# XunshanMan/Object-oriented-SLAM

Measured on AMD Instinct MI355X. Metric: LM iterations/sec (cams+ellipsoids), higher is better.
Workload: dtype f64

## Files before the change

### object-oriented-slam_amd/csrc/esl_capi.hip

```cpp
#include <algorithm>
#include <cfloat>
#include <cmath>
#include <cstdio>
#include <cstdlib>
#include <cstring>
#include <numeric>

#include "esl_graph_int.hpp"
#include "esl_graph_layout.hpp"
#include "esl_kernels_map.hpp"
#include "esl_kernels_chunk.hpp"
#include "esl_slam.hpp"
#include "esl_fixed.hpp"

namespace esl {
static thread_local std::string g_err;
void set_error(const std::string& s) { g_err = s; }
}

using namespace esl;

namespace esl {
ProfScope::ProfScope(esl_ctx* ctx, int kind) : c(ctx), slot(-1) {
  if (!c || !c->prof_on) return;
  if (c->prof_level < 2 && (kind != 0 || !c->prof_gate)) return;
  if (c->prof_used + 2 > c->prof_ev.size()) {
    if (c->prof_ev.size() >= 16384) { prof_drain(c); }
    else {
      for (int i = 0; i < 512; ++i) { hipEvent_t e; if (hipEventCreate(&e) != hipSuccess) return; c->prof_ev.push_back(e); }
      c->prof_kind.resize(c->prof_ev.size() / 2);
    }
  }
  slot = (int)c->prof_used;
  c->prof_kind[slot / 2] = kind;
  c->prof_used += 2;
  (void)hipEventRecord(c->prof_ev[slot], c->stream);
}
ProfScope::~ProfScope() {
  if (slot >= 0) (void)hipEventRecord(c->prof_ev[slot + 1], c->stream);
}
int prof_drain(esl_ctx* c) {
  if (hipStreamSynchronize(c->stream) != hipSuccess) return ESL_ERR_HIP;
  for (size_t s = 0; s + 1 < c->prof_used; s += 2) {
    float ms = 0;
    if (hipEventElapsedTime(&ms, c->prof_ev[s], c->prof_ev[s + 1]) == hipSuccess) {
      const int k = c->prof_kind[s / 2];
      c->prof_count[k]++;
      c->prof_ms[k] += ms;
    }
  }
  c->prof_used = 0;
  return ESL_OK;
}
}

struct WorkStage {
  struct Fix { void** dst; size_t off; };
  size_t total = 0;
  std::vector<Fix> fixes;
  template <class T>
  void add(T** dst, size_t n) {
    const size_t off = layout::align_up(total, 256);
    total = off + std::max<size_t>(n, 1) * sizeof(T);
    fixes.push_back({(void**)dst, off});
  }
  int commit(esl_ctx* c) {
    int rc = arena_reserve(&c->arena_work, &c->arena_work_cap, std::max<size_t>(total, 256));
    if (rc) return rc;
    for (const Fix& f : fixes) *f.dst = c->arena_work + f.off;
    return ESL_OK;
  }
};
int esl::work_buffers(esl_ctx* c, size_t cap_objs, size_t cap_cams, size_t cap_chunks) {
  WorkStage wk;
  wk.add(&c->chunk_out, cap_chunks * kChunkOut); wk.add(&c->chunk_out2, cap_chunks * kChunkOut);
  wk.add(&c->chunk_chi, cap_chunks);
  wk.add(&c->blk_part, ((cap_objs + kStepWaves - 1) / kStepWaves + 2) * 2);
  wk.add(&c->solve_part, ((cap_objs + kStepWaves - 1) / kStepWaves + (cap_objs + 63) / 64 + 2) * 4 * 2);
  wk.add(&c->blk_chi, cap_chunks + 2);
  wk.add(&c->cams, cap_cams * 7); wk.add(&c->cams_trial, cap_cams * 7);
  wk.add(&c->objs, cap_objs * 10); wk.add(&c->objs_trial, cap_objs * 10);
  wk.add(&c->Hoo, cap_objs * 45); wk.add(&c->bo, cap_objs * 9); wk.add(&c->xo, cap_objs * 9); wk.add(&c->obj_part, cap_objs * 4);
  int rc = wk.commit(c);
  if (rc) return rc;
  ESL_HIP_TRY(hipMemsetAsync(c->obj_part, 0, std::max<size_t>(cap_objs, 1) * 4 * sizeof(double), c->stream));
  return ESL_OK;
}

extern "C" {

int esl_abi_version(void) { return ESL_ABI_VERSION; }
const char* esl_last_error(void) { return g_err.c_str(); }

int esl_device_count(void) {
  int n = 0;
  if (hipGetDeviceCount(&n) != hipSuccess) return 0;
  return n;
}

void esl_lm_params_default(esl_lm_params* p) {
  p->max_iters = 10;
  p->max_trials = 10;
  p->tau = 1e-5;
  p->jacobian_mode = ESL_JAC_NUMERIC;
  p->numeric_delta = 1e-9;
  p->linear_solver = ESL_SOLVER_AUTO;
  p->drop_nan_bbox = 1;
  p->bbox_residual = ESL_BBOX_REPROJECTION;
  p->e3d_half_turn = 0;
}

int esl_ctx_create(int device_id, esl_ctx** out) {
  if (!out) return ESL_ERR_INVALID;
  *out = nullptr;
  int n = 0;
  if (hipGetDeviceCount(&n) != hipSuccess || n <= 0) {
    set_error("no HIP device visible: libesl_hip has no CPU fallback");
    return ESL_ERR_NO_DEVICE;
  }
  if (device_id < 0 || device_id >= n) { set_error("device id out of range"); return ESL_ERR_INVALID; }
  ESL_HIP_TRY(hipSetDevice(device_id));
  esl_ctx* c = new esl_ctx();
  c->device = device_id;
  { const char* ov = std::getenv("ESL_CF_OVERLAP"); c->sw_cf_overlap = (ov && ov[0] >= '0' && ov[0] <= '4') ? ov[0] - '0' : 4; }
  { const char* ok = std::getenv("ESL_CF_OS_KERNEL"); c->sw_cf_os_kernel = (ok && ok[0] == '0') ? 0 : 1; }
  { const char* ol = std::getenv("ESL_CF_OS_LIST"); c->sw_cf_os_list = (ol && ol[0] == '0') ? 0 : 1; }
  { const char* fp = std::getenv("ESL_CF_FWD_PARTS"); const int v = fp ? std::atoi(fp) : 0; if (v == 2 || v == 4 || v == 8) c->sw_cf_fwd_parts = v; }
  { const char* sd = std::getenv("ESL_CF_STRIDE"); const int v = sd ? std::atoi(sd) : 0; c->sw_cf_stride = (v == 16 || v == 32 || v == 48) ? v : 0; }
  auto init = [&]() -> int {
    ESL_HIP_TRY(hipStreamCreateWithFlags(&c->stream, hipStreamNonBlocking));
    ESL_HIP_TRY(hipHostMalloc((void**)&c->host_part, 16 * sizeof(double), hipHostMallocDefault));
    ESL_HIP_TRY(hipMalloc((void**)&c->dev_part, 16 * sizeof(double)));
    ESL_HIP_TRY(hipMalloc((void**)&c->chol_info, 4 * sizeof(int)));
    ESL_HIP_TRY(hipMemset(c->chol_info, 0, 4 * sizeof(int)));
    ESL_HIP_TRY(hipMalloc((void**)&c->tickets, 4 * sizeof(unsigned int)));
    ESL_HIP_TRY(hipMemset(c->tickets, 0, 4 * sizeof(unsigned int)));
    ESL_HIP_TRY(hipMalloc((void**)&c->dev_scal, 8 * sizeof(double)));
    ESL_HIP_TRY(hipEventCreateWithFlags(&c->ev_try, hipEventDisableTiming));
    ESL_HIP_TRY(hipHostMalloc(&c->host_scal, sizeof(LmScalars), hipHostMallocMapped));
    ESL_HIP_TRY(hipHostGetDevicePointer(&c->host_scal_dev, c->host_scal, 0));
    std::memset(c->host_scal, 0, sizeof(LmScalars));
    ESL_HIP_TRY(hipMalloc(&c->lm_dev, 2 * sizeof(LmCore)));
    ESL_HIP_TRY(hipMemset(c->lm_dev, 0, 2 * sizeof(LmCore)));
    ESL_HIP_TRY(hipHostMalloc(&c->lm_host, sizeof(LmHostView), hipHostMallocMapped));
    ESL_HIP_TRY(hipHostGetDevicePointer(&c->lm_host_dev, c->lm_host, 0));
    std::memset(c->lm_host, 0, sizeof(LmHostView));
    return ESL_OK;
  };
  const int rc = init();
  if (rc) { const std::string msg = g_err; esl_ctx_destroy(c); set_error(msg); return rc; }
  *out = c;
  return ESL_OK;
}

int esl_ctx_destroy(esl_ctx* c) {
  if (!c) return ESL_OK;
  (void)hipSetDevice(c->device);
  if (c->stream) (void)hipStreamSynchronize(c->stream);
  slam_sync_side(c);
  free_graph(c);
  slam_release(c);
  if (c->arena_graph) (void)hipFree(c->arena_graph);
  if (c->arena_work) (void)hipFree(c->arena_work);
  if (c->stage_host) (void)hipHostFree(c->stage_host);
  if (c->append_dev) (void)hipFree(c->append_dev);
  if (c->slam_tab_dev) (void)hipFree(c->slam_tab_dev);
  c->eq_buf.release();
  if (c->fx_blob) (void)hipFree(c->fx_blob);
  c->chain_ws.release();
  fit_release(c);
  plane_release(c);
  reloc_release(c);
  assoc_release(c);
  merge_release(c);
  render_release(c);
  dense_release(c);
  init_batch_release(c);
  for (hipEvent_t e : c->prof_ev) (void)hipEventDestroy(e);
  if (c->host_part) (void)hipHostFree(c->host_part);
  dev_free(&c->dev_part);
  dev_free(&c->chol_info);
  dev_free(&c->tickets); dev_free(&c->dev_scal);
  if (c->host_scal) (void)hipHostFree(c->host_scal);
  if (c->lm_host) (void)hipHostFree(c->lm_host);
  if (c->lm_dev) (void)hipFree(c->lm_dev);
  if (c->ev_try) (void)hipEventDestroy(c->ev_try);
  esl_comm_destroy(c);
  slam_release_runtime(c);
  if (c->stream) (void)hipStreamDestroy(c->stream);
  delete c;
  return ESL_OK;
}

int esl_ctx_trim(esl_ctx* c) {
  if (!c) return ESL_ERR_INVALID;
  ESL_HIP_TRY(hipSetDevice(c->device));
  ESL_HIP_TRY(hipStreamSynchronize(c->stream));
  slam_trim(c, c->graph_loaded && c->g.n_free_cams > 0);
  return ESL_OK;
}

int esl_debug_scratch_allocs(esl_ctx* c, int32_t owner, int64_t* allocs_out, int64_t* bytes_out) {
  if (!c || !allocs_out || !bytes_out || owner < ESL_SCRATCH_RELOC || owner > ESL_SCRATCH_INIT_ROBUST) {
    set_error("esl_debug_scratch_allocs: null pointer or unknown owner");
    return ESL_ERR_INVALID;
  }
  *allocs_out = 0; *bytes_out = 0;
  switch (owner) {
    case ESL_SCRATCH_RELOC: reloc_scratch_stats(c, allocs_out, bytes_out); break;
    case ESL_SCRATCH_ASSOC: assoc_scratch_stats(c, allocs_out, bytes_out); break;
    case ESL_SCRATCH_MERGE: merge_scratch_stats(c, allocs_out, bytes_out); break;
    case ESL_SCRATCH_RENDER: render_scratch_stats(c, allocs_out, bytes_out); break;
    default: init_scratch_stats(c, owner == ESL_SCRATCH_INIT_ROBUST, allocs_out, bytes_out);
  }
  return ESL_OK;
}

int esl_ctx_synchronize(esl_ctx* c) {
  if (!c) return ESL_ERR_INVALID;
  ESL_HIP_TRY(hipStreamSynchronize(c->stream));
  return ESL_OK;
}

static ChunkTable chunk_table(const esl_ctx* c) {
  ChunkTable t;
  t.n_chunks = c->n_chunks; t.obj = c->ck_obj; t.type = c->ck_type; t.begin = c->ck_begin; t.end = c->ck_end; t.ostart = c->ck_ostart;
  return t;
}
static int map_launch_linearize(esl_ctx* c, bool finalize, const double* src_objs = nullptr, double* dst_chunk = nullptr,
                                const LmCore* st = nullptr, bool validate = false) {
  const DevGraph& g = c->g;
  if (!src_objs) src_objs = c->objs;
  if (!dst_chunk) dst_chunk = c->chunk_out;
  const double* objs_b = st ? c->objs_trial : nullptr;
  double* chunk_b = st ? c->chunk_out2 : nullptr;
  if (st) { src_objs = c->objs; dst_chunk = c->chunk_out; }
  const ChunkTable ct = chunk_table(c);
  const bool an = c->lm.p.jacobian_mode == ESL_JAC_ANALYTIC;
  const int nb_e3 = (c->n_ids_e3 + 2 * kLinWaves - 1) / (2 * kLinWaves);
  const int nb_bb = (c->n_ids_bb + kLinWaves - 1) / kLinWaves;
  robust_dispatch(c->robust_on, [&](auto robust) {
    constexpr bool R = decltype(robust)::value;
    if (ct.n_chunks > 0) {
      ProfScope ps(c, 0);
      const dim3 block(64 * kLinWaves);
      int* cnt = c->chol_info + 2;
      if (an && g.bbox_mode) {
        if (validate && g.check_vis)
          hipLaunchKernelGGL((k_chunk_linearize_both<ESL_JAC_ANALYTIC, 2, true, R>), dim3(nb_e3 + nb_bb), block, 0, c->stream, g, ct, c->ck_ids_e3,
                             c->n_ids_e3, nb_e3, c->ck_ids_bb, c->n_ids_bb, c->cams, src_objs, objs_b, c->lm.p.numeric_delta, dst_chunk,
                             chunk_b, c->blk_chi, st, cnt);
        else if (validate)
          hipLaunchKernelGGL((k_chunk_linearize_both<ESL_JAC_ANALYTIC, 1, true, R>), dim3(nb_e3 + nb_bb), block, 0, c->stream, g, ct, c->ck_ids_e3,
                             c->n_ids_e3, nb_e3, c->ck_ids_bb, c->n_ids_bb, c->cams, src_objs, objs_b, c->lm.p.numeric_delta, dst_chunk,
                             chunk_b, c->blk_chi, st, cnt);
        else
          hipLaunchKernelGGL((k_chunk_linearize_both<ESL_JAC_ANALYTIC, 0, true, R>), dim3(nb_e3 + nb_bb), block, 0, c->stream, g, ct, c->ck_ids_e3,
                             c->n_ids_e3, nb_e3, c->ck_ids_bb, c->n_ids_bb, c->cams, src_objs, objs_b, c->lm.p.numeric_delta, dst_chunk,
                             chunk_b, c->blk_chi, st, cnt);
      } else if (an) {
        if (validate && g.check_vis)
          hipLaunchKernelGGL((k_chunk_linearize_both<ESL_JAC_ANALYTIC, 2, false, R>), dim3(nb_e3 + nb_bb), block, 0, c->stream, g, ct, c->ck_ids_e3,
                             c->n_ids_e3, nb_e3, c->ck_ids_bb, c->n_ids_bb, c->cams, src_objs, objs_b, c->lm.p.numeric_delta, dst_chunk,
                             chunk_b, c->blk_chi, st, cnt);
        else if (validate)
          hipLaunchKernelGGL((k_chunk_linearize_both<ESL_JAC_ANALYTIC, 1, false, R>), dim3(nb_e3 + nb_bb), block, 0, c->stream, g, ct, c->ck_ids_e3,
                             c->n_ids_e3, nb_e3, c->ck_ids_bb, c->n_ids_bb, c->cams, src_objs, objs_b, c->lm.p.numeric_delta, dst_chunk,
                             chunk_b, c->blk_chi, st, cnt);
        else
          hipLaunchKernelGGL((k_chunk_linearize_both<ESL_JAC_ANALYTIC, 0, false, R>), dim3(nb_e3 + nb_bb), block, 0, c->stream, g, ct, c->ck_ids_e3,
                             c->n_ids_e3, nb_e3, c->ck_ids_bb, c->n_ids_bb, c->cams, src_objs, objs_b, c->lm.p.numeric_delta, dst_chunk,
                             chunk_b, c->blk_chi, st, cnt);
      } else {
        if (nb_e3 > 0)
          hipLaunchKernelGGL((k_chunk_linearize<ESL_JAC_NUMERIC, 1, 0, false, R>), dim3(nb_e3), block, 0, c->stream, g, ct, c->ck_ids_e3,
                             c->n_ids_e3, c->cams, src_objs, objs_b, c->lm.p.numeric_delta, dst_chunk, chunk_b, c->blk_chi, 0, st, cnt);
        if (nb_bb > 0) {
          auto launch_bb = [&](auto kern) {
            hipLaunchKernelGGL(kern, dim3(nb_bb), block, 0, c->stream, g, ct, c->ck_ids_bb, c->n_ids_bb, c->cams, src_objs, objs_b,
// ... 643 lines not shown
```

### object-oriented-slam_amd/csrc/esl_cf.hpp

```cpp
#pragma once
#include "esl_cf_plan.hpp"
#include "esl_kernels_map.hpp"

namespace esl {

__device__ __forceinline__ double cf_readlane(double v, int src) {
  const int lo = __builtin_amdgcn_readlane(__double2loint(v), src), hi = __builtin_amdgcn_readlane(__double2hiint(v), src);
  return __hiloint2double(hi, lo);
}

static __global__ __launch_bounds__(256) void k_cf_gather_B(int nf, const double* __restrict__ Aod, const int* __restrict__ od_start,
                                                            const int* __restrict__ od_edge, double* __restrict__ B) {
  const long t = (long)blockIdx.x * 256 + threadIdx.x;
  const long i = t / 36;
  if (i >= nf) return;
  const int e = (int)(t - i * 36), r = e / 6, c = e - 6 * r;
  double s = 0;
  if (i + 1 < nf)
    for (int q = od_start[i]; q < od_start[i + 1]; ++q) {
      const int es = od_edge[q];
      const double* Hij = Aod + (size_t)(es >> 1) * 90 + 54;
      s += (es & 1) ? Hij[c * 6 + r] : Hij[r * 6 + c];
    }
  B[t] = s;
// ... 263 lines not shown
          for (int q = 0; q < CH * 6; ++q) sv[q * 64 + lane] = (q < hl * 6) ? svy[h0 * 6 + q] : 0.0;
        } else if (col) {
          const int ka = cst[ch], kb = cst[ch + 1];
          for (int k = ka; k < kb; k += 4) {
            int sl[4];
            double rec[4][6];
#pragma unroll
            for (int e = 0; e < 4; ++e) {
              const int kk = (k + e < kb) ? k + e : ka;
              sl[e] = oe_slot[kk];
              const double* src = V + ((size_t)kk * 9 + b) * 6;
#pragma unroll
              for (int a = 0; a < 6; ++a) rec[e][a] = src[a];
            }
#pragma unroll
            for (int e = 0; e < 4; ++e)
              if (k + e < kb && sl[e] - i0 >= h0 && sl[e] - i0 - h0 < hl) {
#pragma unroll
                for (int a = 0; a < 6; ++a) sv[((sl[e] - i0 - h0) * 6 + a) * 64 + lane] += rec[e][a];
              }
          }
        }
        __builtin_amdgcn_wave_barrier();
      }
      for (int ii = 0; ii < hl; ++ii) {
        const double* M = sM + (h0 + ii) * 36;
        double xn[6];
#pragma unroll
        for (int a = 0; a < 6; ++a) {
          double t = sv[(ii * 6 + a) * 64 + lane];
#pragma unroll
          for (int q = 0; q < 6; ++q) t -= M[a * 6 + q] * x[q];
          xn[a] = t;
        }
#pragma unroll
        for (int a = 0; a < 6; ++a) { x[a] = xn[a]; sv[(ii * 6 + a) * 64 + lane] = xn[a]; }
        if (use_z) {
          const double* Z = sZ + (h0 + ii) * 36;
#pragma unroll
          for (int a = 0; a < 6; ++a)
#pragma unroll
            for (int q = 0; q < 6; ++q) acc[a] += Z[q * 6 + a] * xn[q];
        }
      }
      if (on) {
#pragma unroll
        for (int q0 = 0; q0 < CH * 6; q0 += 8) {
          double t[8];
#pragma unroll
          for (int e = 0; e < 8; ++e) t[e] = sv[((q0 + e < hl * 6) ? q0 + e : 0) * 64 + lane];
#pragma unroll
          for (int e = 0; e < 8; ++e)
            if (q0 + e < hl * 6) {
              const int q = q0 + e;
              if (MODE == 2) {
                Xt[(size_t)sg.xoff[seg] + (size_t)(6 * (i0 - beg + h0) + q) * (size_t)sg.xld[seg] + (size_t)j] = t[e];
              } else {
                const size_t row = (SEP && sep_stride > 0) ? (size_t)(6 * ((i0 + q / 6) * sep_stride + sep_stride - 1) + q % 6) : (size_t)(6 * i0 + q);
                Xt[(size_t)j + row * (size_t)ldx] = t[e];
              }
            }
        }
      }
      __builtin_amdgcn_wave_barrier();
    }
  }
  if (use_z && on) {
#pragma unroll
    for (int a = 0; a < 6; ++a) R[(size_t)tcol + (size_t)(6 * (seg - 1) + a) * (size_t)ldx] = acc[a];
  }
}

static __global__ __launch_bounds__(64) void k_cf_zt(int nf, int stride, const double* __restrict__ Linv, const double* __restrict__ Mm,
                                                     const double* __restrict__ B, double* __restrict__ Zt) {
  __shared__ double sM[kCfMaxStride * 36];
  const int p = blockIdx.x + 1, lane = threadIdx.x;
  const int beg = p * stride, end = (beg + stride - 1 < nf) ? beg + stride - 1 : nf;
  if (beg >= end) return;
  const int len = end - beg;
  {
    constexpr int kQ = kCfMaxStride * 36 / 64;
    double t[kQ];
#pragma unroll
    for (int q = 0; q < kQ; ++q) { const int idx = q * 64 + lane; t[q] = Mm[(size_t)beg * 36 + (idx < len * 36 ? idx : 0)]; }
#pragma unroll
    for (int q = 0; q < kQ; ++q) sM[q * 64 + lane] = t[q];
  }
  __builtin_amdgcn_wave_barrier();
  const int c = lane < 6 ? lane : 5;
  double z[6];
  {
    const double* Li = Linv + (size_t)beg * 36;
    const double* Bs = B + (size_t)(beg - 1) * 36;
#pragma unroll
    for (int r = 0; r < 6; ++r) {
      double v = 0;
#pragma unroll
      for (int k = 0; k <= r; ++k) v += Li[r * 6 + k] * Bs[k * 6 + c];
      z[r] = v;
    }
  }
  for (int ii = 0; ii < len; ++ii) {
    if (ii > 0) {
      const double* M = sM + ii * 36;
      double zn[6];
#pragma unroll
      for (int r = 0; r < 6; ++r) {
        double v = 0;
#pragma unroll
        for (int k = 0; k < 6; ++k) v -= M[r * 6 + k] * z[k];
        zn[r] = v;
      }
#pragma unroll
      for (int r = 0; r < 6; ++r) z[r] = zn[r];
    }
    if (lane < 6) {
#pragma unroll
      for (int r = 0; r < 6; ++r) Zt[(size_t)(beg + ii) * 36 + r * 6 + lane] = z[r];
    }
  }
}

static __global__ __launch_bounds__(256) void k_cf_sep_assemble(int nf, int stride, int n_sep, const double* __restrict__ Hcc, double lambda,
                                                                const double* __restrict__ Gfac, const double* __restrict__ Zt,
                                                                double* __restrict__ Hs, double* __restrict__ Bs) {
  const int t = blockIdx.x * 256 + threadIdx.x;
  const int k = t / 36;
  if (k >= n_sep) return;
  const int e = t - k * 36, r = e / 6, c = e - 6 * r;
  const int s = k * stride + stride - 1, l = s - 1;
  double v = Hcc[(size_t)s * 36 + e] + ((r == c) ? lambda : 0.0);
#pragma unroll
  for (int q = 0; q < 6; ++q) v -= Gfac[(size_t)l * 36 + q * 6 + r] * Gfac[(size_t)l * 36 + q * 6 + c];
  const int beg = (k + 1) * stride, end = (beg + stride - 1 < nf) ? beg + stride - 1 : nf;
  for (int j = beg; j < end; ++j) {
#pragma unroll
    for (int q = 0; q < 6; ++q) v -= Zt[(size_t)j * 36 + q * 6 + r] * Zt[(size_t)j * 36 + q * 6 + c];
  }
  Hs[t] = v;
  double w = 0;
  if (k + 1 < n_sep) {
    const int le = end - 1;
#pragma unroll
    for (int q = 0; q < 6; ++q) w -= Gfac[(size_t)le * 36 + q * 6 + r] * Zt[(size_t)le * 36 + q * 6 + c];
  }
  Bs[t] = w;
}

static __global__ __launch_bounds__(64) void k_cf_sep_rhs(int nf, int n_o, int stride, int n_chunks, const int* __restrict__ oe_cst,
                                                          const int* __restrict__ oe_slot, const double* __restrict__ V,
                                                          const double* __restrict__ vy, const double* __restrict__ Gfac,
                                                          const double* __restrict__ LiS, const double* __restrict__ Xt, long ldx,
                                                          double* __restrict__ R, const int* __restrict__ cmap ,
                                                          CfSegs sg) {
  const int j = blockIdx.x * 64 + threadIdx.x, k = blockIdx.y;
  if (j > n_o) return;
  const bool rhs = j == n_o;
  const int N1 = n_o / 9 + 1;
  const int s = k * stride + stride - 1, l = s - 1;
  double vs[6] = {0, 0, 0, 0, 0, 0};
  if (rhs) {
#pragma unroll
    for (int a = 0; a < 6; ++a) vs[a] = vy[(size_t)s * 6 + a];
  } else {
    const int tb = j / 9, b = j - 9 * tb;
    const int o = sg.unrank ? sg.unrank[tb] : tb;
    const int* cst = oe_cst + (size_t)o * (n_chunks + 1);
    const int ch = s / kCfFwdCh;
    for (int q = cst[ch]; q < cst[ch + 1]; ++q)
      if (oe_slot[q] == s) {
        const double* src = V + ((size_t)q * 9 + b) * 6;
#pragma unroll
        for (int a = 0; a < 6; ++a) vs[a] += src[a];
      }
  }
  bool has_acc = (k + 1) * stride < nf;
  double xl[6] = {0, 0, 0, 0, 0, 0};
  if (cmap) {
    const int tb2 = j / 9, bb = rhs ? 0 : j - 9 * tb2;
    const int ob = rhs ? N1 - 1 : (sg.unrank ? sg.unrank[tb2] : tb2);
    has_acc = has_acc && cmap[(size_t)(k + 1) * N1 + ob] >= 0;
    const int e = cmap[(size_t)k * N1 + ob];
    if (e >= 0) {
      const double* src = Xt + (size_t)sg.xoff[k] + (size_t)(9 * (e & 0xFFFFFF) + bb);
      const size_t ld = (size_t)sg.xld[k];
#pragma unroll
      for (int r = 0; r < 6; ++r) xl[r] = src[(size_t)(6 * (stride - 2) + r) * ld];
    }
  } else {
#pragma unroll
    for (int r = 0; r < 6; ++r) xl[r] = Xt[(size_t)j + (size_t)(6 * l + r) * (size_t)ldx];
  }
  double t[6];
#pragma unroll
  for (int a = 0; a < 6; ++a) t[a] = has_acc ? R[(size_t)j + (size_t)(6 * k + a) * (size_t)ldx] : 0.0;
#pragma unroll
  for (int a = 0; a < 6; ++a)
#pragma unroll
    for (int r = 0; r < 6; ++r) t[a] += Gfac[(size_t)l * 36 + r * 6 + a] * xl[r];
#pragma unroll
  for (int a = 0; a < 6; ++a) {
    double v = vs[a];
#pragma unroll
    for (int q = 0; q <= a; ++q) v -= LiS[(size_t)k * 36 + a * 6 + q] * t[q];
    R[(size_t)j + (size_t)(6 * k + a) * (size_t)ldx] = v;
  }
}

static __global__ __launch_bounds__(256) void k_cf_back_prep(int nf, int stride, int n_sep, const double* __restrict__ Zt, const double* __restrict__ Gfac,
                                                             const double* __restrict__ xc, double* __restrict__ z) {
  const int t = blockIdx.x * 256 + threadIdx.x;
  const int i = t / 6, a = t - 6 * i;
  if (i >= nf) return;
  const int p = i / stride, pos = i - p * stride;
  if (pos == stride - 1) return;
  double v = 0;
  if (p >= 1) {
    const double* xs = xc + (size_t)(p * stride - 1) * 6;
#pragma unroll
    for (int q = 0; q < 6; ++q) v += Zt[(size_t)i * 36 + a * 6 + q] * xs[q];
  }
  if ((pos == stride - 2 || i == nf - 1) && p < n_sep) {
    const double* xs = xc + (size_t)(p * stride + stride - 1) * 6;
#pragma unroll
    for (int q = 0; q < 6; ++q) v += Gfac[(size_t)i * 36 + a * 6 + q] * xs[q];
  }
  z[t] -= v;
}

__device__ __forceinline__ void cf_T_init_full_one(const double* __restrict__ Hoo, const double* __restrict__ bo, double lambda,
                                                   double* __restrict__ T, long ldt, long n_o, long t) {
  const long col = t / ldt, row = t - col * ldt;
  if (col >= n_o) return;
  double v = 0;
  const long o = col / 9;
  const int c = (int)(col - 9 * o);
  if (row == n_o) v = bo[(size_t)o * 9 + c];
  else if (row < n_o && row / 9 == o && row >= col) {
    const int r = (int)(row - 9 * o);
    v = Hoo[(size_t)o * 45 + c * 9 - (c * (c - 1)) / 2 + (r - c)] + ((r == c) ? lambda : 0.0);
  }
  T[t] = v;
}
static __global__ __launch_bounds__(256) void k_cf_edge_scale_T(DevGraph g, int nb_es, int n_list, const int* __restrict__ oe_u, const int* __restrict__ oe_slot,
                                                                const double* __restrict__ W, const double* __restrict__ Linv,
                                                                const double* __restrict__ bc, double* __restrict__ V, double* __restrict__ vy,
                                                                const double* __restrict__ Hoo, const double* __restrict__ bo, double lambda,
                                                                double* __restrict__ T, long ldt, long n_o) {
  if ((int)blockIdx.x < nb_es) cf_edge_scale_one(g, n_list, oe_u, oe_slot, W, Linv, bc, V, vy, (long)blockIdx.x * 256 + threadIdx.x);
  else cf_T_init_full_one(Hoo, bo, lambda, T, ldt, n_o, (long)(blockIdx.x - nb_es) * 256 + threadIdx.x);
}

static __global__ __launch_bounds__(256) void k_cf_z(const double* __restrict__ Xt, long ldx, int n_o, const double* __restrict__ xo,
                                                     double* __restrict__ z) {
  __shared__ double red[4];
  const double* row = Xt + (size_t)blockIdx.x * (size_t)ldx;
  double s = 0;
  for (int o = threadIdx.x; o < n_o; o += 256) s += row[o] * xo[o];
  s = wave_sum(s);
  if ((threadIdx.x & 63) == 0) red[threadIdx.x >> 6] = s;
  __syncthreads();
  if (threadIdx.x == 0) z[blockIdx.x] = row[n_o] - (((red[0] + red[1]) + red[2]) + red[3]);
}

constexpr int kCfBackCh = 32;
static __global__ __launch_bounds__(64) void k_cf_tridiag_back(int nf_all, const double* __restrict__ Linv, const double* __restrict__ Nn,
                                                               const double* __restrict__ z, double* __restrict__ xc, int stride, int seglen,
                                                               int map_stride) {
  __shared__ double sLi[kCfBackCh * 36], sN[kCfBackCh * 36], sz[kCfBackCh * 6];
  const int lane = threadIdx.x;
  const int a = lane < 6 ? lane : 5;
  const int beg = (int)blockIdx.x * stride;
  const int nf = (beg + seglen < nf_all) ? beg + seglen : nf_all;
  if (beg >= nf) return;
  double xa = 0;
  for (int hi = nf; hi > beg; hi -= kCfBackCh) {
    const int i0 = (hi - kCfBackCh > beg) ? hi - kCfBackCh : beg, len = hi - i0;
    __builtin_amdgcn_wave_barrier();
    {
      constexpr int kQ = kCfBackCh * 36 / 64, kZ = (kCfBackCh * 6 + 63) / 64;
      double tl[kQ], tn[kQ], tz[kZ];
#pragma unroll
      for (int q = 0; q < kQ; ++q) {
        const int idx = q * 64 + lane, cl = idx < len * 36 ? idx : 0;
        tl[q] = Linv[(size_t)i0 * 36 + cl]; tn[q] = Nn[(size_t)i0 * 36 + cl];
      }
#pragma unroll
      for (int q = 0; q < kZ; ++q) {
        const int idx = q * 64 + lane, cl = idx < len * 6 ? idx : 0;
        const size_t src = map_stride > 0 ? (size_t)((i0 + cl / 6) * map_stride + map_stride - 1) * 6 + cl % 6 : (size_t)i0 * 6 + cl;
        tz[q] = z[src];
      }
#pragma unroll
      for (int q = 0; q < kQ; ++q) { sLi[q * 64 + lane] = tl[q]; sN[q * 64 + lane] = tn[q]; }
#pragma unroll
      for (int q = 0; q < kZ; ++q) if (q * 64 + lane < kCfBackCh * 6) sz[q * 64 + lane] = tz[q];
    }
    __builtin_amdgcn_wave_barrier();
    for (int ii = len - 1; ii >= 0; --ii) {
      double xn[6];
#pragma unroll
      for (int k = 0; k < 6; ++k) xn[k] = cf_readlane(xa, k);
      double s = 0;
#pragma unroll
      for (int k = 0; k < 6; ++k) s += sLi[ii * 36 + k * 6 + a] * sz[ii * 6 + k] - sN[ii * 36 + a * 6 + k] * xn[k];
      xa = s;
      const size_t dst = map_stride > 0 ? (size_t)((i0 + ii) * map_stride + map_stride - 1) * 6 : (size_t)(i0 + ii) * 6;
      if (lane < 6) xc[dst + lane] = s;
    }
  }
}

__device__ __forceinline__ void cf_obj_update_one(const DevGraph& g, double lambda, const double* __restrict__ objs, const double* __restrict__ bo,
                                                  const double* __restrict__ xo, double* __restrict__ objs_trial, double* __restrict__ part, int o) {
  if (o >= g.n_objs) return;
  const Ell e = ell_load(objs + 10 * o);
  const bool active = (g.bb_start[o + 1] > g.bb_start[o]) || (g.e3_start[o + 1] > g.e3_start[o]) || g.gr_cnt[o] > 0;
  part[o * 4 + 3] = 1;
  if (!active) {
    ell_store(e, objs_trial + 10 * o);
    part[o * 4 + 2] = 0;
    return;
  }
  double x[9], scale = 0;
#pragma unroll
  for (int i = 0; i < 9; ++i) { x[i] = xo[(size_t)o * 9 + i]; scale += x[i] * (lambda * x[i] + bo[(size_t)o * 9 + i]); }
  ell_store(ell_oplus(e, x), objs_trial + 10 * o);
  part[o * 4 + 2] = scale;
}

typedef double cf_d4 __attribute__((ext_vector_type(4)));
constexpr int kCfTPer = 16;
constexpr int kCfTBatch = 8;
static __global__ __launch_bounds__(256) void k_cf_T_sparse(int N, int nw, const unsigned long long* __restrict__ mask, const int* __restrict__ cmap,
                                                            const long long* __restrict__ xoff, const int* __restrict__ xld,
                                                            const double* __restrict__ Xc, const double* __restrict__ Hoo,
                                                            const double* __restrict__ bo, double lambda, double* __restrict__ T, long ldt,
                                                            int o2_begin, int o2_end, const int* __restrict__ unrank) {
  const int lane = threadIdx.x & 63, wave = __builtin_amdgcn_readfirstlane(threadIdx.x >> 6);
  const int t1 = blockIdx.x;
  const int o1 = (t1 == N || !unrank) ? t1 : unrank[t1];
  const int r = lane & 15, kq = lane >> 4;
  const int N1 = N + 1;
  const long n_o = 9L * N;
  for (int q = wave; q < kCfTPer; q += 4) {
    const int t2 = o2_begin + (int)blockIdx.y * kCfTPer + q;
    if (t2 >= o2_end || t2 > t1 || t2 >= N) continue;
    const int o2 = unrank ? unrank[t2] : t2;
    cf_d4 acc = {0, 0, 0, 0};
    for (int wd = 0; wd < nw; ++wd) {
      unsigned long long m = mask[(size_t)o1 * nw + wd] & mask[(size_t)o2 * nw + wd];
      if (!m) continue;
      const int pl = wd * 64 + lane;
      const bool mine = (m >> lane) & 1ull;
      const int e1l = mine ? cmap[(size_t)pl * N1 + o1] : 0, e2l = mine ? cmap[(size_t)pl * N1 + o2] : 0;
      const long long xol = mine ? xoff[pl] : 0;
      const int ldl = mine ? xld[pl] : 0;
      while (m) {
        const int bit = __builtin_ctzll(m);
        m &= m - 1;
        const int e1 = __builtin_amdgcn_readlane(e1l, bit), e2 = __builtin_amdgcn_readlane(e2l, bit);
        const int ld = __builtin_amdgcn_readlane(ldl, bit);
        const long long xo = ((long long)__builtin_amdgcn_readlane((int)(xol >> 32), bit) << 32) | (unsigned)__builtin_amdgcn_readlane((int)xol, bit);
        const int f1 = e1 >> 24, f2 = e2 >> 24, f = f1 > f2 ? f1 : f2;
        const double* pa = Xc + xo + 9 * (e1 & 0xFFFFFF) + r;
        const double* pb = Xc + xo + 9 * (e2 & 0xFFFFFF) + r;
        for (int k = (6 * f) & ~3; k < 6 * (kCfFwdCh - 1); k += 4 * kCfTBatch) {
          double av[kCfTBatch], bv[kCfTBatch];
#pragma unroll
          for (int u = 0; u < kCfTBatch; ++u) {
            int row = k + 4 * u + kq;
            row = row < kCfSegRows ? row : kCfSegRows - 1;
            av[u] = pa[(long)row * ld];
            bv[u] = pb[(long)row * ld];
          }
#pragma unroll
          for (int u = 0; u < kCfTBatch; ++u) acc = __builtin_amdgcn_mfma_f64_16x16x4f64(av[u], bv[u], acc, 0, 0, 0);
        }
      }
    }
    if (r < 9) {
#pragma unroll
      for (int g = 0; g < 4; ++g) {
        const int i = kq + 4 * g;
        if (o1 == N) {
          if (i == 0) T[n_o + (9L * t2 + r) * ldt] = bo[(size_t)o2 * 9 + r] - acc[g];
        } else if (i < 9) {
          double base = 0;
          if (o1 == o2) {
            const int lo = i < r ? i : r, hi = i < r ? r : i;
            base = Hoo[(size_t)o1 * 45 + lo * 9 - (lo * (lo - 1)) / 2 + (hi - lo)] + ((i == r) ? lambda : 0.0);
          }
          T[(9L * t1 + i) + (9L * t2 + r) * ldt] = base - acc[g];
        }
      }
    }
  }
}

static __global__ __launch_bounds__(256) void k_cf_z_sparse(int n_o, const double* __restrict__ Xs, long ldx, CfSegs sg, const double* __restrict__ Xc,
                                                            const double* __restrict__ xo, const double* __restrict__ xo_t, double* __restrict__ z,
                                                            int stride) {
  __shared__ double red[4];
  const int t = blockIdx.x, i = t / 6, a = t - 6 * i;
  const int p = i / stride, pos = i - p * stride;
  double s = 0, y;
  if (pos == stride - 1) {
    const double* row = Xs + (size_t)(6 * p + a) * (size_t)ldx;
    for (int o = threadIdx.x; o < n_o; o += 256) s += row[o] * xo_t[o];
    y = row[n_o];
  } else {
    const int ob = sg.seg_start[p], m = 9 * (sg.seg_start[p + 1] - ob);
    const double* row = Xc + (size_t)sg.xoff[p] + (size_t)(6 * pos + a) * (size_t)sg.xld[p];
    for (int cc = threadIdx.x; cc < m; cc += 256) {
      const int ci = cc / 9;
      s += row[cc] * xo[(size_t)9 * sg.seg_obj[ob + ci] + (cc - 9 * ci)];
    }
    y = row[m];
  }
  s = wave_sum(s);
  if ((threadIdx.x & 63) == 0) red[threadIdx.x >> 6] = s;
  __syncthreads();
  if (threadIdx.x == 0) z[t] = y - (((red[0] + red[1]) + red[2]) + red[3]);
}

static __global__ __launch_bounds__(256) void k_cf_seg_syrk(const int* __restrict__ twork, const int* __restrict__ seg_start,
                                                            const int* __restrict__ seg_first, const long long* __restrict__ xoff,
                                                            const int* __restrict__ xld, const double* __restrict__ Xc,
                                                            const long long* __restrict__ boff, double* __restrict__ P) {
  const int p = twork[3 * blockIdx.x], ti = twork[3 * blockIdx.x + 1], tj = twork[3 * blockIdx.x + 2];
  const int lane = threadIdx.x & 63, wave = __builtin_amdgcn_readfirstlane(threadIdx.x >> 6);
  const int r = lane & 15, kq = lane >> 4;
  const int ob = seg_start[p], m = 9 * (seg_start[p + 1] - ob);
  const int c1b = ti * kCfSyT + (wave >> 1) * 64, c2b = tj * kCfSyT + (wave & 1) * 64;
  if (c1b + 63 < c2b || c1b >= m || c2b >= m) return;
  const long ld = xld[p];
  const double* X = Xc + xoff[p];
  cf_d4 acc[4][4];
#pragma unroll
  for (int mi = 0; mi < 4; ++mi)
#pragma unroll
    for (int nj = 0; nj < 4; ++nj) acc[mi][nj] = cf_d4{0, 0, 0, 0};
  const double* pa = X + c1b + r;
  const double* pb = X + c2b + r;
  constexpr int kB = 3;
  constexpr int kNBatch = kCfSegRows / (4 * kB);
  static_assert(kNBatch * 4 * kB == kCfSegRows, "slab rows = whole batches");
  double a0[kB][4], b0[kB][4], a1[kB][4], b1[kB][4];
  auto load = [&](double (&a)[kB][4], double (&b)[kB][4], int it) {
    const int k = it * 4 * kB;
#pragma unroll
    for (int u = 0; u < kB; ++u)
#pragma unroll
      for (int q = 0; q < 4; ++q) {
        a[u][q] = pa[(long)(k + 4 * u + kq) * ld + 16 * q];
        b[u][q] = pb[(long)(k + 4 * u + kq) * ld + 16 * q];
      }
  };
  auto mac = [&](double (&a)[kB][4], double (&b)[kB][4]) {
#pragma unroll
    for (int u = 0; u < kB; ++u)
#pragma unroll
      for (int mi = 0; mi < 4; ++mi)
#pragma unroll
        for (int nj = 0; nj < 4; ++nj) acc[mi][nj] = __builtin_amdgcn_mfma_f64_16x16x4f64(b[u][nj], a[u][mi], acc[mi][nj], 0, 0, 0);
  };
  const int it0 = (6 * seg_first[ob + c1b / 9]) / (4 * kB);
  load(a0, b0, it0);
  for (int it = it0; it < kNBatch; it += 2) {
    if (it + 1 < kNBatch) load(a1, b1, it + 1);
    mac(a0, b0);
    if (it + 1 < kNBatch) {
      if (it + 2 < kNBatch) load(a0, b0, it + 2);
      mac(a1, b1);
    }
  }
  double* Pp = P + (size_t)boff[p] * 81;
#pragma unroll
  for (int mi = 0; mi < 4; ++mi) {
    const int c1 = c1b + 16 * mi + r;
    if (c1 >= m) continue;
    const int i1 = c1 / 9, i = c1 - 9 * i1;
    const size_t row_off = (size_t)i1 * (i1 + 1) / 2;
#pragma unroll
    for (int nj = 0; nj < 4; ++nj)
#pragma unroll
      for (int g = 0; g < 4; ++g) {
        const int c2 = c2b + 16 * nj + kq + 4 * g;
        if (c2 > c1) continue;
        const int i2 = c2 / 9, j = c2 - 9 * i2;
        Pp[(row_off + i2) * 81 + j * 9 + i] = acc[mi][nj][g];
      }
  }
}

static __global__ __launch_bounds__(64) void k_cf_seg_rhs(const int* __restrict__ fwork, const int* __restrict__ seg_start,
                                                          const long long* __restrict__ xoff, const int* __restrict__ xld,
                                                          const double* __restrict__ Xc, const long long* __restrict__ roff,
                                                          double* __restrict__ Prhs) {
  const int p = fwork[2 * blockIdx.x], c = fwork[2 * blockIdx.x + 1] * 64 + (int)threadIdx.x;
  const int m = 9 * (seg_start[p + 1] - seg_start[p]);
  const long ld = xld[p];
  const double* X = Xc + xoff[p];
  const int cc = c < m ? c : 0;
  double s = 0;
#pragma unroll 6
  for (int row = 0; row < 6 * (kCfFwdCh - 1); ++row) s += X[(long)row * ld + cc] * X[(long)row * ld + m];
  if (c < m) Prhs[roff[p] + c] = s;
}

static __global__ __launch_bounds__(256) void k_cf_T_gather(int N, int nw, const unsigned long long* __restrict__ mask, const int* __restrict__ cmap,
                                                            const long long* __restrict__ boff, const long long* __restrict__ roff,
                                                            const double* __restrict__ P, const double* __restrict__ Prhs,
                                                            const double* __restrict__ Hoo, const double* __restrict__ bo, double lambda,
                                                            double* __restrict__ T, long ldt, int o2_begin, int o2_end, const int* __restrict__ unrank,
                                                            int accumulate = 0) {
  const int lane = threadIdx.x & 63, wave = __builtin_amdgcn_readfirstlane(threadIdx.x >> 6);
  const int t1 = blockIdx.x;
  const int o1 = (t1 == N || !unrank) ? t1 : unrank[t1];
  const int N1 = N + 1;
  const long n_o = 9L * N;
  const bool rhs = o1 == N;
  for (int q = wave; q < kCfTPer; q += 4) {
    const int t2 = o2_begin + (int)blockIdx.y * kCfTPer + q;
    if (t2 >= o2_end || t2 > t1 || t2 >= N) continue;
    const int o2 = unrank ? unrank[t2] : t2;
    double s0 = 0, s1 = 0;
    const int eT0 = (lane % 9) * 9 + lane / 9, eT1 = lane < 17 ? ((64 + lane) % 9) * 9 + (64 + lane) / 9 : 0;
    for (int wd = 0; wd < nw; ++wd) {
      unsigned long long mk = mask[(size_t)o1 * nw + wd] & mask[(size_t)o2 * nw + wd];
      if (!mk) continue;
      const int pl = wd * 64 + lane;
      long long offl = 0;
      int swl = 0;
      if ((mk >> lane) & 1ull) {
        const long long i2 = cmap[(size_t)pl * N1 + o2] & 0xFFFFFF;
        if (rhs) offl = roff[pl] + 9 * i2;
        else {
          const long long i1 = cmap[(size_t)pl * N1 + o1] & 0xFFFFFF;
          swl = i2 > i1;
          offl = (boff[pl] + (swl ? i2 * (i2 + 1) / 2 + i1 : i1 * (i1 + 1) / 2 + i2)) * 81;
        }
      }
      while (mk) {
        long long off[4];
        bool have[4], sw[4];
#pragma unroll
        for (int u = 0; u < 4; ++u) {
          have[u] = mk != 0;
          const int bit = have[u] ? __builtin_ctzll(mk) : 0;
          if (have[u]) mk &= mk - 1;
          off[u] = ((long long)__builtin_amdgcn_readlane((int)(offl >> 32), bit) << 32) | (unsigned)__builtin_amdgcn_readlane((int)offl, bit);
          sw[u] = __builtin_amdgcn_readlane(swl, bit) != 0;
        }
        double v0[4], v1[4];
#pragma unroll
        for (int u = 0; u < 4; ++u) {
// ... 472 lines not shown
```

### object-oriented-slam_amd/csrc/esl_cf_plan.hpp

```cpp
#pragma once
#include <algorithm>
#include <array>
#include <cmath>
#include <cstddef>
#include <cstdint>
#include <utility>
#include <vector>

namespace esl {

constexpr int kCfFwdCh = 16;
constexpr int kCfSyT = 128;
constexpr int kCfSegRows = 96;
constexpr int kCfMaxStride = 128;
constexpr int kCfKC = 16;
constexpr int kCfSparseMinCams = 256;

constexpr double kCfUpdFlopsPerMs = 0.83 * 79.0e9;
constexpr double kCfPairMs = (7.82 - 4.21) / (77.35e6 - 31.05e6);
constexpr double kCfSlabMs = 1.30 / 1.35e8;
constexpr double kCfStrideMargin = 0.05;
inline double cf_stride_cost(double upd_flops, double pairs, double slab) {
  return upd_flops / kCfUpdFlopsPerMs + pairs * kCfPairMs + slab * kCfSlabMs;
}
inline int cf_stride_choose(long n_o, const double* upd_flops, const double* pairs, const double* slab) {
  if (n_o < 8192) return kCfFwdCh;
  const double base = cf_stride_cost(upd_flops[0], pairs[0], slab[0]);
  int best = 1;
  double best_ms = base * (1.0 - kCfStrideMargin);
  for (int m = 2; m <= 3; ++m) {
    const double ms = cf_stride_cost(upd_flops[m - 1], pairs[m - 1], slab[m - 1]);
    if (ms < best_ms) { best = m; best_ms = ms; }
  }
  return best * kCfFwdCh;
}

struct CfSwitches {
  int sparse = -1;
  bool tperm_off = false;
  bool no_nd = false;
  int nd_min = 48;
  int stride = 0;
  int os_kernel = 1;
  int os_list = 1;
};

struct CfSegTables {
  int S = kCfFwdCh, nseg = 0, nw = 0;
  std::vector<int> p, o, first;
  std::vector<int> seg_start, xld, fw_off;
  std::vector<long long> xoff, boff, roff, tw_off;
  int n_fwork = 0, n_twork = 0;
  size_t xc_len = 0, p_blocks = 0, prhs_len = 0;
  double sp_flops = 0;
};
struct CfPlan : CfSegTables {
  int n_list = 0, n_chunks = 0;
  int64_t ldx = 0, ldt = 0, kpad = 0, kpad_s = 0;
  bool nd = false;
  int stride = 0, n_sep = 0, n_seg = 1;
  bool sparse = false;
  int form = 0;
  std::vector<int> os, ou;
  size_t y_len = 0;
  size_t os_npairs = 0;
  bool os_offsets = false;
  double os_flops = 0;
  bool os_list = false;
  std::vector<int> os_run, os_heads;
  size_t osm_npairs = 0, osm_row_npairs = 0, os_list_npairs = 0;
  double osm_flops = 0;
  bool tperm = false;
  std::vector<int> rank, unrank, kfirst;
  double upd_flops = 0;
};

inline void cf_entry_lists(int N, int nf, const std::vector<int>& start, const int* cu_start, const int* cu_obj, const int* cu_id,
                           std::vector<int>& os, std::vector<int>& ou) {
  std::vector<int> cur(start.begin(), start.end() - 1);
  os.assign((size_t)start[(size_t)N], 0); ou.assign((size_t)start[(size_t)N], 0);
  for (int sl = 0; sl < nf; ++sl)
    for (int q = cu_start[sl]; q < cu_start[sl + 1]; ++q) { const int at = cur[cu_obj[q]]++; os[(size_t)at] = sl; ou[(size_t)at] = cu_id[q]; }
}
inline CfSegTables cf_walk(int S, int N, int nf, const int* cu_start, const int* cu_obj) {
  CfSegTables t;
  const int nseg = (nf + S - 1) / S;
  t.S = S; t.nseg = nseg; t.nw = (nseg + 63) / 64;
  std::vector<int> last_seg((size_t)N, -1);
  for (int sl = 0; sl < nf; ++sl) {
    const int p = sl / S, pos = sl - p * S;
    if (pos == S - 1) continue;
    for (int q = cu_start[sl]; q < cu_start[sl + 1]; ++q) {
      const int o = cu_obj[q];
      if (last_seg[(size_t)o] != p) { last_seg[(size_t)o] = p; t.p.push_back(p); t.o.push_back(o); t.first.push_back(pos); }
    }
  }
  const size_t n_inc = t.p.size();
  const long long rows = S == kCfFwdCh ? kCfSegRows : 6 * (S - 1);
  t.seg_start.assign((size_t)nseg + 1, 0); t.xld.assign((size_t)nseg, 0); t.fw_off.assign((size_t)nseg + 1, 0);
  t.xoff.assign((size_t)nseg + 1, 0); t.boff.assign((size_t)nseg + 1, 0); t.roff.assign((size_t)nseg + 1, 0); t.tw_off.assign((size_t)nseg + 1, 0);
  for (size_t q = 0; q < n_inc; ++q) ++t.seg_start[(size_t)t.p[q] + 1];
  for (int p = 0; p < nseg; ++p) t.seg_start[(size_t)p + 1] += t.seg_start[(size_t)p];
  for (size_t q = 0; q < n_inc; ++q)
    t.sp_flops += 81.0 * (double)(q - (size_t)t.seg_start[(size_t)t.p[q]] + 1) * (6.0 * (S - 1 - t.first[q]));
  for (int p = 0; p < nseg; ++p) {
    const int cnt = t.seg_start[(size_t)p + 1] - t.seg_start[(size_t)p];
    const int m = 9 * cnt + 1;
    t.xld[(size_t)p] = (m + 15) / 16 * 16 + 16;
    t.xoff[(size_t)p + 1] = t.xoff[(size_t)p] + rows * t.xld[(size_t)p];
    t.fw_off[(size_t)p + 1] = t.fw_off[(size_t)p] + (m + 63) / 64;
    t.boff[(size_t)p + 1] = t.boff[(size_t)p] + (long long)cnt * (cnt + 1) / 2;
    t.roff[(size_t)p + 1] = t.roff[(size_t)p] + 9LL * cnt;
    const long long nt = (9 * cnt + kCfSyT - 1) / kCfSyT;
    t.tw_off[(size_t)p + 1] = t.tw_off[(size_t)p] + nt * (nt + 1) / 2;
  }
  t.n_fwork = t.fw_off[(size_t)nseg]; t.n_twork = (int)t.tw_off[(size_t)nseg];
  t.xc_len = (size_t)t.xoff[(size_t)nseg] + 2 * kCfSyT;
  t.p_blocks = (size_t)t.boff[(size_t)nseg]; t.prhs_len = (size_t)t.roff[(size_t)nseg];
  return t;
}
inline double cf_staircase(int S, int N, int nf, const std::vector<int>& unrank, const std::vector<int>& first_cam, std::vector<int>& kfirst) {
  const size_t n_o = (size_t)9 * N;
  double upd_flops = 0;
  const int Ks = (int)((6 * ((size_t)nf / (size_t)S) + kCfKC - 1) / kCfKC * kCfKC);
  kfirst.assign((n_o + 1 + 256) / 64 + 8, Ks);
  for (size_t col = 0; col < n_o; ++col) {
    const int k0 = std::max(0, first_cam[(size_t)unrank[col / 9]] / S - 1);
    kfirst[col / 64] = std::min(kfirst[col / 64], std::min(6 * k0, Ks));
  }
  kfirst[n_o / 64] = 0;
  const long nti = ((long)n_o + 1 + 127) / 128;
  for (long ti = 0; ti < nti; ++ti) {
    const int ka = std::min(kfirst[(size_t)(ti * 2)], kfirst[(size_t)(ti * 2 + 1)]);
    for (long tj = 0; tj <= ti && tj * 128 < (long)n_o; ++tj) {
      const int kb = std::min(kfirst[(size_t)(tj * 2)], kfirst[(size_t)(tj * 2 + 1)]);
      int ks = std::min(std::max(ka, kb), Ks) & ~(kCfKC - 1);
      if (((Ks - ks) & kCfKC) != 0 && ks >= kCfKC) ks -= kCfKC;
      const double rows_t = (double)std::min<long>(128, (long)n_o + 1 - ti * 128), cols_t = (double)std::min<long>(128, (long)n_o - tj * 128);
      const double in_triangle = tj < ti ? 1.0 : 0.5 * (cols_t + 1.0) / cols_t;
      upd_flops += 2.0 * rows_t * cols_t * (double)(Ks - ks) * in_triangle;
    }
  }
  return upd_flops;
}
struct CfOsCounts { double prod = 0, rhs_entries = 0; };
inline CfOsCounts cf_os_counts(int S, int N, const std::vector<int>& start, const std::vector<int>& os, const std::vector<int>& rank) {
  std::vector<std::array<int, 3>> inc3;
  CfOsCounts n;
  for (int o = 0; o < N; ++o) {
    int last_p = -1;
    for (int k = start[(size_t)o]; k < start[(size_t)o + 1]; ++k) {
      const int sl = os[(size_t)k];
      if (sl % S == S - 1) continue;
      const int p = sl / S;
      if (p != last_p) { inc3.push_back({p, rank.empty() ? o : rank[(size_t)o], 0}); last_p = p; }
      ++inc3.back()[2]; n.rhs_entries += 1;
    }
  }
  std::sort(inc3.begin(), inc3.end());
  for (size_t q = 0, q0 = 0; q < inc3.size(); ++q) {
    if (inc3[q][0] != inc3[q0][0]) q0 = q;
    n.prod += (double)inc3[q][2] * (double)(q - q0 + 1);
  }
  return n;
}

inline void cf_os_sides(CfPlan& pl, const std::vector<int>& start) {
  const int S = pl.S;
  const size_t n_inc = pl.p.size();
  pl.os_run.assign(pl.os.size(), 0); pl.os_heads.assign(n_inc, 0);
  std::vector<int> cur(start.begin(), start.end() - 1);
  for (size_t q = 0; q < n_inc; ++q) {
    const int o = pl.o[q], p = pl.p[q], end = start[(size_t)o + 1];
    int k = cur[(size_t)o];
    while (k < end && pl.os[(size_t)k] / S < p) ++k;
    for (int head = -1; k < end && pl.os[(size_t)k] / S == p; ++k) {
      const int sl = pl.os[(size_t)k];
      if (sl % S == S - 1) continue;
      if (head < 0 || pl.os[(size_t)head] != sl) { head = k; ++pl.os_heads[q]; }
      ++pl.os_run[(size_t)head];
    }
    cur[(size_t)o] = k;
  }
  double both = 0, row = 0, brow = 0;
  std::vector<int> v;
  std::vector<std::pair<int, int>> byrank;
  for (int p = 0; p < pl.nseg; ++p) {
    const int q0 = pl.seg_start[(size_t)p], n = pl.seg_start[(size_t)p + 1] - q0;
    v.assign(pl.os_heads.begin() + q0, pl.os_heads.begin() + q0 + n);
    std::sort(v.begin(), v.end());
    for (int i = 0; i < n; ++i) { both += (double)v[(size_t)i] * (double)(n - i); brow += v[(size_t)i]; }
    byrank.clear();
    for (int i = 0; i < n; ++i) { const int o = pl.o[(size_t)(q0 + i)]; byrank.push_back({pl.rank.empty() ? o : pl.rank[(size_t)o], pl.os_heads[(size_t)(q0 + i)]}); }
    std::sort(byrank.begin(), byrank.end());
    for (int i = 0; i < n; ++i) row += (double)byrank[(size_t)i].second * (double)(i + 1);
  }
  pl.osm_npairs = (size_t)(both + brow); pl.osm_row_npairs = (size_t)(row + brow);
  pl.osm_flops = 2.0 * 6.0 * (81.0 * both + 9.0 * brow);
}

inline bool cf_plan_build(int N, int nf, size_t EU, const std::vector<int>& start, const int* cu_start, const int* cu_obj, const int* cu_id, bool chain_ok,
                          bool comm, size_t total_mem, const CfSwitches& sw, CfPlan& pl) {
  pl = CfPlan{};
  const size_t nfz = (size_t)nf, n_o = (size_t)9 * N;
  const int nch = (nf + kCfFwdCh - 1) / kCfFwdCh;
  pl.ldx = (int64_t)((n_o + 1 + 127) / 128 * 128);
  pl.kpad = (int64_t)((6 * nfz + kCfKC - 1) / kCfKC * kCfKC);
  pl.ldt = pl.ldx;
  pl.n_list = start[(size_t)N]; pl.n_chunks = nch;
  pl.nseg = nch; pl.nw = (nch + 63) / 64;
  if ((size_t)std::max(N, 1) * (size_t)(nch + 1) > ((size_t)1 << 28)) return false;
  cf_entry_lists(N, nf, start, cu_start, cu_obj, cu_id, pl.os, pl.ou);
  CfSegTables& seg = pl;
  if (chain_ok && nf >= kCfSparseMinCams && N > 0 && (size_t)nch * (size_t)(N + 1) <= ((size_t)1 << 28) && !sw.no_nd) {
    seg = cf_walk(kCfFwdCh, N, nf, cu_start, cu_obj);
    const double dense = (double)n_o * (double)n_o * 6.0 * (double)nfz;
    const double sparse = (double)n_o * (double)n_o * 6.0 * (double)(nfz / kCfFwdCh) + 24.0 * pl.sp_flops;
    pl.sparse = sw.sparse >= 0 ? sw.sparse != '0' : (n_o >= 2048 && sparse < 0.5 * dense);
    const double need = 8.0 * (81.0 * (double)pl.p_blocks + (double)pl.xc_len + 2.0 * (double)pl.ldt * (double)n_o +
                               2.0 * 6.0 * (double)(nfz / kCfFwdCh) * (double)pl.ldx  + 54.0 * (double)EU );
    pl.form = sw.sparse == '2' || need > 0.4 * (double)total_mem ? 2 : 1;
    if ((sw.sparse < 0 || sw.sparse == '3') && !comm) pl.form = 3;
  }
  const bool sp = pl.sparse;
  std::vector<int> first_cam;
  pl.tperm = sp && N > 0 && !sw.tperm_off;
  if (pl.tperm) {
    std::vector<int> cnt(nfz + 2, 0);
    first_cam.assign((size_t)N, nf);
    for (int o = 0; o < N; ++o) if (start[(size_t)o + 1] > start[(size_t)o]) first_cam[(size_t)o] = pl.os[(size_t)start[(size_t)o]];
    for (int o = 0; o < N; ++o) ++cnt[(size_t)first_cam[(size_t)o] + 1];
    for (int s = 0; s <= nf; ++s) cnt[(size_t)s + 1] += cnt[(size_t)s];
    pl.rank.assign((size_t)N, 0); pl.unrank.assign((size_t)N, 0);
    for (int o = 0; o < N; ++o) { const int t = cnt[(size_t)first_cam[(size_t)o]]++; pl.rank[(size_t)o] = t; pl.unrank[(size_t)t] = o; }
  }
  if (sp && pl.form == 3 && !comm) {
    int want = sw.stride;
    CfSegTables cand[3];
    if (!want && pl.tperm && n_o >= 8192) {
      double upd[3], pairs[3], slab[3];
      for (int m = 1; m <= 3; ++m) {
        const int S = m * kCfFwdCh;
        cand[m - 1] = cf_walk(S, N, nf, cu_start, cu_obj);
        const CfOsCounts n = cf_os_counts(S, N, start, pl.os, pl.rank);
        long long cols = 0;
        for (int x : cand[m - 1].xld) cols += x;
        upd[m - 1] = cf_staircase(S, N, nf, pl.unrank, first_cam, pl.kfirst); pairs[m - 1] = n.prod + n.rhs_entries; slab[m - 1] = 6.0 * (S - 1) * (double)cols;
      }
      want = cf_stride_choose((long)n_o, upd, pairs, slab);
      seg = std::move(cand[want / kCfFwdCh - 1]);
    }
    if (!want) want = kCfFwdCh;
    if (want != pl.S) seg = cf_walk(want, N, nf, cu_start, cu_obj);
  }
  pl.nd = nfz >= (size_t)std::max(sw.nd_min, 2 * kCfFwdCh) && !sw.no_nd;
  if (pl.nd) {
    int sd = 16 * (int)std::max(1.0, std::floor(std::sqrt((double)nfz) / 16.0 + 0.5));
    sd = std::min(sd, kCfMaxStride);
    if (sp) sd = pl.S;
    pl.stride = sd; pl.n_sep = nf / sd; pl.n_seg = (nf + sd - 1) / sd;
  }
  if (sp) pl.kpad_s = (int64_t)((6 * (size_t)pl.n_sep + kCfKC - 1) / kCfKC * kCfKC);
  if (pl.tperm) pl.upd_flops = cf_staircase(pl.S, N, nf, pl.unrank, first_cam, pl.kfirst);
  if (sp && pl.form == 3) {
    const CfOsCounts n = cf_os_counts(pl.S, N, start, pl.os, pl.rank);
    const size_t y_recs = std::max<size_t>(pl.p.size(), 1) * (size_t)(pl.S - 1);
    pl.os_flops = 2.0 * 6.0 * (81.0 * n.prod + 9.0 * n.rhs_entries);
    pl.os_npairs = (size_t)(n.prod + n.rhs_entries);
    pl.y_len = y_recs * 54 + std::max<size_t>(nfz, 1) * 6;
    pl.os_offsets = sw.os_kernel != 0 && 54 * std::max(EU, y_recs) <= (size_t)INT32_MAX;
    cf_os_sides(pl, start);
    pl.os_list = sw.os_list != 0;
    pl.os_list_npairs = pl.os_list ? pl.osm_npairs : pl.os_npairs;
  }
  return true;
}

}
```

### object-oriented-slam_amd/csrc/esl_chol.hpp

```cpp
#pragma once
#include <hip/hip_runtime.h>

#include <algorithm>
#include <cstdint>
#include <cstdio>
#include <cstdlib>
#include <vector>

#include "esl_chol_kernels.hpp"
#include "esl_chol_plan.hpp"
#include "esl_chol_persist.hpp"

namespace esl {

struct CholDist {
  int rank = 0, n_ranks = 1;
  void* user = nullptr;
  int (*bcast)(void* user, double* dev, size_t count, int root) = nullptr;
  double* pack = nullptr;
  double* pack2 = nullptr;
  int (*bcast_on)(void* user, double* dev, size_t count, int root, hipStream_t stream) = nullptr;
};
inline int chol_outer_panels(int n);
inline size_t chol_pack_len(int n) { const size_t w = (size_t)chol_outer_panels(n) * kNB; return ((size_t)n + 1) * w + w * kNB; }
inline int chol_outer_panels(int n) { return (n >= 8192) ? 4 : 2; }

struct CholSwitches {
  int persistent = 2;
  bool small = true;
  bool backsub_launches = false;
  bool upd_v = true;
  bool fuse = true;
  int merge = 0;
  bool strips = false;
  int special = 2;
  int W = 0;
  int filler = 128;
  int timeout_ms = 0;
  bool timing = false;
  bool debug = false;
  bool upd_v_cap = false;
};
inline CholSwitches chol_switches_from_env() {
  CholSwitches s;
  auto clamp = [](int v, int lo, int hi) { return v < lo ? lo : (v > hi ? hi : v); };
  if (const char* e = std::getenv("ESL_CHOL_PERSISTENT")) s.persistent = e[0] == '1' ? 1 : 0;
  if (const char* e = std::getenv("ESL_CHOL_SMALL")) s.small = e[0] != '0';
  if (const char* e = std::getenv("ESL_CHOL_BACKSUB_LAUNCHES")) s.backsub_launches = e[0] == '1';
  if (const char* e = std::getenv("ESL_UPD_V")) s.upd_v = std::atoi(e) != 0;
  if (const char* e = std::getenv("ESL_CHOL_FUSE")) s.fuse = e[0] != '0';
  if (const char* e = std::getenv("ESL_CHOL_MERGE")) s.merge = clamp(std::atoi(e), 1, 16);
  if (const char* e = std::getenv("ESL_CHOL_STRIPS")) s.strips = e[0] == '1';
  if (const char* e = std::getenv("ESL_CHOL_SPECIAL")) s.special = clamp(std::atoi(e), 1, 8);
  if (const char* e = std::getenv("ESL_CHOL_W")) s.W = std::max(1, std::atoi(e));
  if (const char* e = std::getenv("ESL_CHOL_FILLER")) s.filler = std::max(1, std::atoi(e));
  if (const char* e = std::getenv("ESL_CHOL_TIMEOUT_MS")) s.timeout_ms = std::max(1, std::atoi(e));
  s.timing = std::getenv("ESL_CHOL_TIMING") != nullptr;
  s.debug = std::getenv("ESL_CHOL_DEBUG") != nullptr;
  if (const char* e = std::getenv("ESL_UPD_V_CAP")) s.upd_v_cap = e[0] == '1';
  return s;
}

inline bool chol_update_v_applies(const CholSwitches& sw, long lda, long rows, long base, long col_limit, bool ext, long ldp) {
  const long nrows = rows - base, nc = col_limit - base;
  if (nrows <= 0 || nc <= 0) return false;
  const bool whole = (nc >= nrows - 1);
  const long big_tiles = ((nrows + 255) / 256) * ((nc + 127) / 128) / (whole ? 2 : 1);
  return big_tiles >= 1024 && sw.upd_v && (lda & 1) == 0 && (base & 1) == 0 && (!ext || (ldp & 1) == 0);
}
constexpr size_t kCholLdsVCap = 84 * 1024;
static_assert(2 * kCholLdsVCap > 160 * 1024 && kCholLdsVCap >= kCholLdsV, "one capped workgroup per CU");
inline void chol_launch_update(const CholSwitches& sw, double* M, long lda, long rows, hipStream_t stream, int kcol0, int K, long base, long col_limit,
                               const double* Pext = nullptr, long ldp = 0, double* part = nullptr, const int* kfirst = nullptr, bool assign = false,
                               bool cap = false) {
  const long nrows = rows - base, nc = col_limit - base;
  if (nrows <= 0 || nc <= 0) return;
  const bool whole = (nc >= nrows - 1);
  const long big_tiles = ((nrows + 255) / 256) * ((nc + 127) / 128) / (whole ? 2 : 1);
  if (big_tiles >= 1024) {
    const long ntI = (nrows + 255) / 256, ntJ = (nc + 127) / 128;
    const long nblk = whole ? ntI * (ntI + 1) : ntI * ntJ;
    if (chol_update_v_applies(sw, lda, rows, base, col_limit, Pext != nullptr, ldp)) {
      const long vI = (nrows + kVT - 1) / kVT, vJ = (nc + kVT - 1) / kVT;
      const long vblk = whole ? chol_v_grid(vI) : vI * vJ;
      hipLaunchKernelGGL(k_chol_update_v, dim3((unsigned)vblk), dim3(256), (cap || sw.upd_v_cap) ? kCholLdsVCap : kCholLdsV, stream, M, lda, rows, col_limit, kcol0, K, base, (int)vJ, whole ? 0 : 1, Pext, ldp,
                         Pext ? kfirst : nullptr, assign ? 1 : 0);
      return;
    }
    hipLaunchKernelGGL((k_chol_update_lds<256, 128>), dim3((unsigned)nblk), dim3(512), kCholLdsBig, stream, M, lda, rows, col_limit, kcol0, K,
                       base, (int)ntJ, whole ? 0 : 1, Pext, ldp, (double*)nullptr, 0, Pext ? kfirst : nullptr);
  } else {
    const long ntI = (nrows + 127) / 128, ntJ = (nc + 63) / 64;
    const long nblk = whole ? ntI * (ntI + 1) : ntI * ntJ;
    int nsplit = 1, kper = K;
    if (part && Pext && base == 0 && nblk < 128 && K >= 16 * kKC) {
      nsplit = (int)std::min<long>(kCholMaxSplit, std::max<long>(1, 512 / nblk));
      kper = ((K + nsplit - 1) / nsplit + kKC - 1) / kKC * kKC;
      nsplit = (K + kper - 1) / kper;
    }
    if (nsplit > 1) {
      hipLaunchKernelGGL((k_chol_update_lds<128, 64>), dim3((unsigned)nblk, (unsigned)nsplit), dim3(512), kCholLdsSmall, stream, M, lda, rows, col_limit,
                         kcol0, K, base, (int)ntJ, whole ? 0 : 1, Pext, ldp, part, kper);
      hipLaunchKernelGGL(k_chol_splitk_reduce, dim3((unsigned)((rows * col_limit + 255) / 256)), dim3(256), 0, stream, M, lda, rows, col_limit, part, nsplit);
    } else {
      hipLaunchKernelGGL((k_chol_update_lds<128, 64>), dim3((unsigned)nblk), dim3(512), kCholLdsSmall, stream, M, lda, rows, col_limit, kcol0, K,
                         base, (int)ntJ, whole ? 0 : 1, Pext, ldp, (double*)nullptr, 0, Pext ? kfirst : nullptr);
    }
  }
}

struct CholRuntime {
  hipStream_t side = nullptr;
  std::vector<hipEvent_t> ev_panel, ev_trail;
  hipStream_t comm = nullptr;
  hipEvent_t ev_begin = nullptr;
  std::vector<hipEvent_t> ev_packed, ev_recv, ev_unpacked;
  bool attr_set = false;
  int* bs_flags = nullptr; int bs_flags_cap = 0;
  CholPlan plan;
  CholTask* d_tasks = nullptr; int* d_ns = nullptr; int* d_sync = nullptr;
  size_t d_tasks_cap = 0, d_ns_cap = 0, d_sync_cap = 0;
  CholSwitches sw;
  int n_cu = 0;
  int fallbacks = 0;
  void (*prof_mark)(void* user, int begin) = nullptr;
  void* prof_user = nullptr;
  hipStream_t cf_side = nullptr;
  hipEvent_t cf_ev_x = nullptr, cf_ev_p = nullptr, cf_ev_a = nullptr, cf_ev_s = nullptr;
  hipError_t cf_overlap_init() {
    if (cf_side && cf_ev_x && cf_ev_p && cf_ev_a && cf_ev_s) return hipSuccess;
    if (cf_side) return hipErrorNotReady;
    hipError_t e = hipStreamCreateWithFlags(&cf_side, hipStreamNonBlocking); if (e != hipSuccess) return e;
    for (hipEvent_t* ev : {&cf_ev_x, &cf_ev_p, &cf_ev_a, &cf_ev_s}) {
      e = hipEventCreateWithFlags(ev, hipEventDisableTiming); if (e != hipSuccess) return e;
    }
    return hipSuccess;
  }
  void release() {
    if (cf_side) { (void)hipStreamSynchronize(cf_side); (void)hipStreamDestroy(cf_side); cf_side = nullptr; }
    for (hipEvent_t* ev : {&cf_ev_x, &cf_ev_p, &cf_ev_a, &cf_ev_s})
      if (*ev) { (void)hipEventDestroy(*ev); *ev = nullptr; }
    if (bs_flags) { (void)hipFree(bs_flags); bs_flags = nullptr; bs_flags_cap = 0; }
    if (d_tasks) { (void)hipFree(d_tasks); d_tasks = nullptr; d_tasks_cap = 0; }
    if (d_ns) { (void)hipFree(d_ns); d_ns = nullptr; d_ns_cap = 0; }
    if (d_sync) { (void)hipFree(d_sync); d_sync = nullptr; d_sync_cap = 0; }
    plan = CholPlan();
    for (std::vector<hipEvent_t>* v : {&ev_panel, &ev_trail, &ev_packed, &ev_recv, &ev_unpacked}) {
      for (hipEvent_t e : *v) (void)hipEventDestroy(e);
      v->clear();
    }
    if (side) { (void)hipStreamDestroy(side); side = nullptr; }
    if (comm) { (void)hipStreamDestroy(comm); comm = nullptr; }
    if (ev_begin) { (void)hipEventDestroy(ev_begin); ev_begin = nullptr; }
    attr_set = false;
  }
};

inline hipError_t chol_set_attributes(CholRuntime& rt) {
  if (rt.attr_set) return hipSuccess;
  rt.sw = chol_switches_from_env();
  hipError_t e = hipFuncSetAttribute((const void*)k_chol_potrf2, hipFuncAttributeMaxDynamicSharedMemorySize, (int)kP2Lds); if (e != hipSuccess) return e;
  e = hipFuncSetAttribute((const void*)k_chol_update_lds<256, 128>, hipFuncAttributeMaxDynamicSharedMemorySize, (int)kCholLdsBig); if (e != hipSuccess) return e;
  e = hipFuncSetAttribute((const void*)k_chol_update_v, hipFuncAttributeMaxDynamicSharedMemorySize, (int)kCholLdsVCap); if (e != hipSuccess) return e;
  e = hipFuncSetAttribute((const void*)k_chol_backsub, hipFuncAttributeMaxDynamicSharedMemorySize, (int)kBsLds); if (e != hipSuccess) return e;
  e = hipFuncSetAttribute((const void*)k_chol_persist, hipFuncAttributeMaxDynamicSharedMemorySize, (int)kPwLds); if (e != hipSuccess) return e;
  const int on = rt.sw.timing ? 1 : 0;
  e = hipMemcpyToSymbol(HIP_SYMBOL(g_chol_stats_on), &on, sizeof(on)); if (e != hipSuccess) return e;
  if (rt.sw.timeout_ms > 0) {
    const long long ticks = 100000LL * rt.sw.timeout_ms;
    e = hipMemcpyToSymbol(HIP_SYMBOL(g_chol_timeout_ticks), &ticks, sizeof(ticks)); if (e != hipSuccess) return e;
  }
  int dev = 0;
  hipDeviceProp_t prop;
  e = hipGetDevice(&dev); if (e != hipSuccess) return e;
  e = hipGetDeviceProperties(&prop, dev); if (e != hipSuccess) return e;
  rt.n_cu = prop.multiProcessorCount > 0 ? prop.multiProcessorCount : kPwGrid;
  rt.attr_set = true;
  return hipSuccess;
}

inline int chol_merge_for(const CholSwitches& sw, int n) { return sw.merge > 0 ? sw.merge : (n >= 16384 ? 3 : 2); }
inline void chol_plan_from_switches(const CholSwitches& sw, int n, int W, int filler, CholPlan& pl) {
  chol_plan_build(n, W, filler, pl, sw.fuse, chol_merge_for(sw, n), sw.strips, std::min(sw.special, W));
}
inline hipError_t chol_factor_persistent(double* M, long lda, int n, double* Linv_ws, int* info, hipStream_t st, CholRuntime& rt) {
  const CholSwitches& sw = rt.sw;
  const int W = sw.W > 0 ? sw.W : chol_outer_panels(n);
  const int merge = chol_merge_for(sw, n), spc = std::min(sw.special, W);
  if (rt.plan.n != n || rt.plan.W != W || rt.plan.fuse != (sw.fuse ? 1 : 0) || rt.plan.merge != merge || rt.plan.strip_merge != (sw.strips ? 1 : 0) || rt.plan.sp != spc) {
    { hipError_t e0 = hipStreamSynchronize(st); if (e0 != hipSuccess) return e0; }
    chol_plan_from_switches(sw, n, W, sw.filler, rt.plan);
    auto grow = [](void** p, size_t* cap, size_t need) -> hipError_t {
      if (*cap >= need) return hipSuccess;
      if (*p) { (void)hipFree(*p); *p = nullptr; *cap = 0; }
      hipError_t e = hipMalloc(p, need); if (e == hipSuccess) *cap = need;
      return e;
    };
    hipError_t e = grow((void**)&rt.d_tasks, &rt.d_tasks_cap, std::max<size_t>(rt.plan.tasks.size(), 1) * sizeof(CholTask)); if (e != hipSuccess) return e;
    e = grow((void**)&rt.d_ns, &rt.d_ns_cap, std::max<size_t>(rt.plan.ns.size(), 1) * sizeof(int)); if (e != hipSuccess) return e;
    {
      const size_t need = chol_sync_words(rt.plan.np, rt.plan.nR) * sizeof(int);
      if (rt.d_sync_cap < need) {
        if (rt.d_sync) { (void)hipFree(rt.d_sync); rt.d_sync = nullptr; rt.d_sync_cap = 0; }
        e = hipMalloc((void**)&rt.d_sync, need); if (e != hipSuccess) return e;
        rt.d_sync_cap = need;
      }
    }
    e = hipStreamSynchronize(st); if (e != hipSuccess) return e;
    if (!rt.plan.tasks.empty()) { e = hipMemcpyAsync(rt.d_tasks, rt.plan.tasks.data(), rt.plan.tasks.size() * sizeof(CholTask), hipMemcpyHostToDevice, st); if (e != hipSuccess) return e; }
    e = hipMemcpyAsync(rt.d_ns, rt.plan.ns.data(), rt.plan.ns.size() * sizeof(int), hipMemcpyHostToDevice, st); if (e != hipSuccess) return e;
  }
  const CholPlan& pl = rt.plan;
  hipError_t e = hipMemsetAsync(rt.d_sync, 0, chol_sync_words(pl.np, pl.nR) * sizeof(int), st); if (e != hipSuccess) return e;
  const int grid = std::max(2, std::min(rt.n_cu > 0 ? rt.n_cu : kPwGrid, kPwGrid));
  hipLaunchKernelGGL(k_chol_persist, dim3((unsigned)grid), dim3(kPwThreads), kPwLds, st, M, lda, n, pl.np, pl.W, pl.nR, Linv_ws, (const CholTask*)rt.d_tasks,
                     (int)pl.tasks.size(), (const int*)rt.d_ns, rt.d_sync, info, pl.fuse, pl.sp);
  return hipGetLastError();
}

struct CholOuter { int p0, p1, c_begin, c_end; long h, w; size_t n_inv; };
inline CholOuter chol_outer_geo(int n, int o) {
  const int W = chol_outer_panels(n), np = (n + kNB - 1) / kNB;
  CholOuter g;
  g.p0 = o * W; g.p1 = (g.p0 + W < np) ? g.p0 + W : np;
  g.c_begin = g.p0 * kNB; g.c_end = (g.p1 * kNB < n) ? g.p1 * kNB : n;
  g.h = (long)n + 1 - g.c_begin; g.w = g.c_end - g.c_begin; g.n_inv = (size_t)(g.p1 - g.p0) * kNB * kNB;
  return g;
}
inline int chol_n_outer(int n) { const int W = chol_outer_panels(n); return ((n + kNB - 1) / kNB + W - 1) / W; }
inline void chol_factor_outer(const CholSwitches& sw, double* M, long lda, int n, double* Linv_ws, int* info, hipStream_t st, const CholOuter& g) {
  const long rows = (long)n + 1;
  for (int p = g.p0; p < g.p1; ++p) {
    const int k0 = p * kNB, nb = (n - k0 < kNB) ? (n - k0) : kNB;
    double* Linv = Linv_ws + (size_t)p * kNB * kNB;
    hipLaunchKernelGGL(k_chol_potrf2, dim3(1), dim3(kP2Threads), kP2Lds, st, M, lda, k0, nb, Linv, info);
    const long below = rows - (k0 + nb);
    if (below > 0) hipLaunchKernelGGL(k_chol_panel, dim3((unsigned)((below + 63) / 64)), dim3(512), 0, st, M, lda, rows, k0, nb, Linv);
    if (p + 1 < g.p1) chol_launch_update(sw, M, lda, rows, st, k0, nb, (long)k0 + nb, (long)g.c_end);
  }
}
inline hipError_t chol_stage_panel(double* M, long lda, int n, double* Linv_ws, hipStream_t st, const CholOuter& g, double* buf) {
  hipLaunchKernelGGL(k_chol_pack, dim3((unsigned)((g.h + 255) / 256), (unsigned)g.w), dim3(256), 0, st, M, lda, (long)n + 1, (long)g.c_begin, (long)g.c_begin, buf, 0);
  return hipMemcpyAsync(buf + (size_t)g.h * g.w, Linv_ws + (size_t)g.p0 * kNB * kNB, g.n_inv * sizeof(double), hipMemcpyDeviceToDevice, st);
}
inline hipError_t chol_unpack_panel(double* M, long lda, int n, double* Linv_ws, hipStream_t st, const CholOuter& g, double* buf) {
  hipLaunchKernelGGL(k_chol_pack, dim3((unsigned)((g.h + 255) / 256), (unsigned)g.w), dim3(256), 0, st, M, lda, (long)n + 1, (long)g.c_begin, (long)g.c_begin, buf, 1);
  return hipMemcpyAsync(Linv_ws + (size_t)g.p0 * kNB * kNB, buf + (size_t)g.h * g.w, g.n_inv * sizeof(double), hipMemcpyDeviceToDevice, st);
}
inline hipError_t chol_grow_events(std::vector<hipEvent_t>& v, int count) {
  while ((int)v.size() < count) {
    hipEvent_t ev;
    hipError_t e = hipEventCreateWithFlags(&ev, hipEventDisableTiming); if (e != hipSuccess) return e;
    v.push_back(ev);
  }
  return hipSuccess;
}

inline hipError_t chol_solve_small(const double* M, long lda, int n, double* x, int* info, hipStream_t st) {
  hipLaunchKernelGGL(k_chol_small, dim3(1), dim3(kCsThreads), 0, st, M, lda, n, x, info);
  return hipGetLastError();
}

inline hipError_t chol_factor_dist_overlap(double* M, long lda, int n, double* Linv_ws, int* info, hipStream_t st, CholRuntime& rt, const CholDist& dist) {
  const long rows = (long)n + 1;
  const int n_outer = chol_n_outer(n), R = dist.n_ranks, me = dist.rank;
  if (!rt.comm) { hipError_t e = hipStreamCreateWithFlags(&rt.comm, hipStreamNonBlocking); if (e != hipSuccess) return e; }
  if (!rt.ev_begin) { hipError_t e = hipEventCreateWithFlags(&rt.ev_begin, hipEventDisableTiming); if (e != hipSuccess) return e; }
  {
    hipError_t e = hipEventRecord(rt.ev_begin, st); if (e != hipSuccess) return e;
    e = hipStreamWaitEvent(rt.comm, rt.ev_begin, 0); if (e != hipSuccess) return e;
  }
  for (std::vector<hipEvent_t>* v : {&rt.ev_packed, &rt.ev_recv, &rt.ev_unpacked}) { hipError_t e = chol_grow_events(*v, n_outer); if (e != hipSuccess) return e; }
  auto buf_of = [&](int o) { return (o & 1) ? dist.pack2 : dist.pack; };
  auto factor_and_stage = [&](int o) -> hipError_t {
    const CholOuter g = chol_outer_geo(n, o);
    chol_factor_outer(rt.sw, M, lda, n, Linv_ws, info, st, g);
    hipError_t e = chol_stage_panel(M, lda, n, Linv_ws, st, g, buf_of(o)); if (e != hipSuccess) return e;
    e = hipGetLastError(); if (e != hipSuccess) return e;
    return hipEventRecord(rt.ev_packed[o], st);
  };
  auto update_with = [&](int o, int o2) {
    const CholOuter g = chol_outer_geo(n, o), q = chol_outer_geo(n, o2);
    chol_launch_update(rt.sw, M, lda, rows, st, g.c_begin, g.c_end - g.c_begin, (long)q.c_begin, (long)q.c_end);
  };
  if (0 % R == me) { hipError_t e = factor_and_stage(0); if (e != hipSuccess) return e; }
  for (int o = 0; o < n_outer; ++o) {
    const int owner = o % R;
    const CholOuter g = chol_outer_geo(n, o);
    hipError_t e;
    if (owner == me) e = hipStreamWaitEvent(rt.comm, rt.ev_packed[o], 0);
    else e = (o >= 2) ? hipStreamWaitEvent(rt.comm, rt.ev_unpacked[o - 2], 0) : hipSuccess;
    if (e != hipSuccess) return e;
    if (dist.bcast_on(dist.user, buf_of(o), (size_t)g.h * g.w + g.n_inv, owner, rt.comm)) return hipErrorUnknown;
// ... 187 lines not shown
```

### object-oriented-slam_amd/csrc/esl_ctx.hpp

```cpp
#pragma once
#include <hip/hip_runtime.h>

#include <cstdint>
#include <string>
#include <type_traits>
#include <vector>

#include "../../include/esl.h"
#include "esl_cf_plan.hpp"
#include "esl_math.hpp"

namespace esl {

void set_error(const std::string& s);
#define ESL_HIP_TRY(expr)                                                                         \
  do {                                                                                            \
    hipError_t _e = (expr);                                                                       \
    if (_e != hipSuccess) {                                                                       \
      esl::set_error(std::string(#expr) + ": " + hipGetErrorString(_e));                          \
      return ESL_ERR_HIP;                                                                         \
    }                                                                                             \
  } while (0)

struct DevGraph {
// ... 70 lines not shown
  esl_lm_params p;
  bool slam = false;
  double lambda_used = 0;
  bool have_trial = false;
};

}

#include "esl_scratch.hpp"

struct BlobArena { char* dev = nullptr; size_t cap = 0; char* host = nullptr; size_t host_cap = 0; hipEvent_t ev = nullptr; };
struct esl_ctx;
namespace esl {
struct ProfScope {
  esl_ctx* c; int slot;
  ProfScope(esl_ctx* ctx, int kind);
  ~ProfScope();
};
int prof_drain(esl_ctx* c);
void fit_graphs_clear(esl_ctx* c);
void fit_release(esl_ctx* c);
void plane_release(esl_ctx* c);
void reloc_release(esl_ctx* c);
void assoc_release(esl_ctx* c);
void merge_release(esl_ctx* c);
void render_release(esl_ctx* c);
void dense_release(esl_ctx* c);
void init_batch_release(esl_ctx* c);
void reloc_scratch_stats(const esl_ctx* c, int64_t* allocs, int64_t* bytes);
void assoc_scratch_stats(const esl_ctx* c, int64_t* allocs, int64_t* bytes);
void merge_scratch_stats(const esl_ctx* c, int64_t* allocs, int64_t* bytes);
void render_scratch_stats(const esl_ctx* c, int64_t* allocs, int64_t* bytes);
void init_scratch_stats(const esl_ctx* c, bool robust, int64_t* allocs, int64_t* bytes);
void dense_scratch_stats(const esl_ctx* c, int64_t* allocs, int64_t* bytes);
int comm_gather_scalars_device(esl_ctx* c);
int comm_allreduce_sum(esl_ctx* c, double* dev_buf, size_t count, hipStream_t st = nullptr);
int comm_reduce_sum_root(esl_ctx* c, double* dev_buf, size_t count, int root);
int comm_bcast(esl_ctx* c, double* dev_buf, size_t count, int root, hipStream_t st = nullptr);
int comm_check_replicated(esl_ctx* c);
int comm_reduce4(esl_ctx* c, const double* dev_src4, double out[4]);
}

struct esl_ctx {
  int device = 0;
  hipStream_t stream = nullptr;
  esl::DevGraph g;
  bool graph_loaded = false;
  bool states_loaded = false;
  double* cams = nullptr; double* cams_trial = nullptr;
  double* objs = nullptr; double* objs_trial = nullptr;
  double* Hoo = nullptr;
  double* bo = nullptr;
  double* xo = nullptr;
  double* obj_part = nullptr;
  double* Hcc = nullptr;
  double* bc = nullptr;
  double* xc = nullptr;
  double* Wbb = nullptr;
  double* Abb = nullptr;
  double* Aod = nullptr;
  double* Dinv = nullptr;
  double* Yb = nullptr;
  double* Wt = nullptr;
  double* Tb = nullptr;
  double* S = nullptr;
  int64_t S_n = 0;
  double* cam_part = nullptr;
  double* od_part = nullptr;
  int* chol_info = nullptr;
  double* host_part = nullptr;
  double* dev_part = nullptr;
  esl::LmState lm;
  esl_robust_params robust = {{0, 0, 0, 0}, {1, 1, 1, 1}};
  bool robust_on = false;
  std::vector<int> h_bb_slot_of, h_e3_slot_of, h_grav_obj;
  esl::Scratch eq_buf;
  double* cams_snap = nullptr; double* objs_snap = nullptr;
  bool prof_on = false;
  int prof_level = 0;
  unsigned prof_runs = 0;
  bool prof_gate = true;
  std::vector<hipEvent_t> prof_ev;
  std::vector<int> prof_kind;
  size_t prof_used = 0;
  int64_t prof_count[ESL_PROF_KINDS] = {0};
  double prof_ms[ESL_PROF_KINDS] = {0};
  std::vector<int> h_bb_cam, h_bb_obj, h_e3_cam, h_e3_obj, h_cam_slot, h_od_i, h_od_j;
  int n_chunks = 0;
  int *ck_obj = nullptr, *ck_type = nullptr, *ck_begin = nullptr, *ck_end = nullptr, *ck_ostart = nullptr;
  int *ck_ids_bb = nullptr, *ck_ids_e3 = nullptr; int n_ids_bb = 0, n_ids_e3 = 0;
  double* chunk_out = nullptr;
  double* chunk_out2 = nullptr;
  hipEvent_t ev_try = nullptr;
  double* chunk_chi = nullptr;
  double* blk_part = nullptr;
  double* solve_part = nullptr;
  double* blk_chi = nullptr;
  unsigned int* tickets = nullptr;
  double* dev_scal = nullptr;
  esl::HostImage* append_img = nullptr;
  char* append_dev = nullptr; size_t append_dev_cap = 0;
  char* slam_tab_dev = nullptr; size_t slam_tab_cap = 0;
  char* arena_graph = nullptr; size_t arena_graph_cap = 0;
  char* arena_work = nullptr;  size_t arena_work_cap = 0;
  char* stage_host = nullptr;  size_t stage_host_cap = 0;
  BlobArena arena_slam, arena_solve, arena_S;
  const int *h_cu_start = nullptr, *h_cu_obj = nullptr, *h_cu_id = nullptr;
  std::vector<int> h_ue_start, h_ue_id, h_ue_slot;
  char* fit_slab = nullptr; size_t fit_slab_cap = 0;
  char* fit_in = nullptr;  size_t fit_in_cap = 0;
  char* fit_out = nullptr; size_t fit_out_cap = 0;
  esl::Scratch plane_slab;
  esl::RelocState* reloc = nullptr;
  esl::AssocState* assoc = nullptr;
  esl::MergeState* merge = nullptr;
  esl::RenderState* render = nullptr;
  esl::DenseState* dense = nullptr;
  esl::InitBatchState* init_batch = nullptr;
  void* fit_graph_cache = nullptr;
  bool parts_fresh = false;
  bool cams_match_snap = false;
  int n_grav_edges = 0;
  void* lm_dev = nullptr;
  void* lm_host = nullptr;
  void* lm_host_dev = nullptr;
  void* host_scal = nullptr;
  void* host_scal_dev = nullptr;
  bool sys_combined = false;
  void* comm = nullptr;
  int comm_ranks = 1, comm_rank = 0;
  bool comm_replicated = false;
  esl_host_allreduce_fn host_allreduce = nullptr;
  void* host_user = nullptr;
  double* host_stage = nullptr;
  double* dev_gather = nullptr;
  double* host_gather = nullptr;
  double* Linv_ws = nullptr;
  double* z_ws = nullptr;
  int64_t S_lda = 0;
  bool cf_chain_ok = false;
  bool cf_ready = false;
  bool cf_unavailable = false;
  esl::CfPlan cf_plan;
  int *cf_oe_start = nullptr, *cf_oe_u = nullptr, *cf_oe_slot = nullptr, *cf_od_start = nullptr, *cf_od_edge = nullptr, *cf_oe_cst = nullptr;
  double *cf_Linv = nullptr, *cf_M = nullptr, *cf_N = nullptr, *cf_V = nullptr, *cf_vy = nullptr, *cf_z = nullptr;
  double *cf_B = nullptr, *cf_Lfac = nullptr, *cf_G = nullptr;
  double *cf_Zt = nullptr, *cf_Hs = nullptr, *cf_Bs = nullptr, *cf_LfacS = nullptr, *cf_GS = nullptr, *cf_LiS = nullptr, *cf_MS = nullptr,
         *cf_NS = nullptr, *cf_R = nullptr;
  double *cf_Xt = nullptr, *cf_T = nullptr, *cf_Linv_ws = nullptr, *cf_part = nullptr;
  int *cf_seg_start = nullptr, *cf_seg_obj = nullptr, *cf_seg_first = nullptr, *cf_cmap = nullptr, *cf_xld = nullptr, *cf_fwork = nullptr, *cf_twork = nullptr;
  unsigned long long* cf_mask = nullptr;
  long long *cf_xoff = nullptr, *cf_boff = nullptr, *cf_roff = nullptr;
  double *cf_Xc = nullptr, *cf_Xs = nullptr, *cf_P = nullptr, *cf_Prhs = nullptr, *cf_Y = nullptr, *cf_Yr = nullptr;
  long long* cf_os_start = nullptr;
  int *cf_os_cnt = nullptr, *cf_os_pairs = nullptr;
  int *cf_os_run = nullptr, *cf_os_heads = nullptr;
  double* cf_Vm = nullptr;
  int *cf_rank = nullptr, *cf_unrank = nullptr, *cf_kfirst = nullptr;
  double* cf_xo_t = nullptr;
  int lm_solver_used = 0;
  bool fx_on = false;
  std::vector<uint8_t> fx_flags;
  esl::AnchGraph fx;
  char* fx_blob = nullptr; size_t fx_blob_cap = 0;
  double* fx_A = nullptr; double* fx_chi = nullptr;
  std::vector<int> fx_bb_map, fx_e3_map;
  std::vector<int> fx_grav_obj;
  bool chain_ok = false;
  esl::Scratch chain_ws;
  esl_pcg_params pcg = {1000, 8, 1e-10};
  esl_pcg_params pcg_run = {1000, 8, 1e-10};
  double* pcg_ws = nullptr; size_t pcg_ws_cap = 0;
  double* pcg_st = nullptr; double* pcg_M = nullptr;
  double* pcg_host = nullptr;
  bool pcg_ran = false;
  bool pcg_reset = true;
  void* chol_rt = nullptr;
  void* chol_prof_scope = nullptr;
  unsigned long long graph_fp = 0;
  bool repl_checked = false;
  double *chol_pack = nullptr, *chol_pack2 = nullptr;
  size_t chol_pack_len = 0;
  bool schur_attr_set = false;
  int sw_chol_dist = -1;
  bool sw_chol_overlap = true;
  int sw_cf_overlap = 4;
  int sw_cf_os_kernel = 1;
  int sw_cf_os_list = 1;
  int sw_cf_fwd_parts = 8;
  int sw_cf_stride = 0;
};
```

### object-oriented-slam_amd/csrc/esl_slam.hip

```cpp
#include "esl_slam.hpp"

#include <algorithm>
#include <array>
#include <chrono>
#include <cmath>
#include <cstdio>
#include <cstdlib>
#include <cstring>

#include "esl_cf.hpp"
#include "esl_chol.hpp"
#include "esl_fixed.hpp"
#include "esl_kernels_slam.hpp"
#include "esl_pcg.hpp"

namespace esl {

static __global__ __launch_bounds__(256) void k_cf_updates(DevGraph g, int nb_obj, double lambda, const double* __restrict__ objs, const double* __restrict__ bo,
                                                           const double* __restrict__ xo, double* __restrict__ objs_trial, double* __restrict__ obj_part,
                                                           const double* __restrict__ cams, const double* __restrict__ xc, const double* __restrict__ bc,
                                                           double* __restrict__ cams_trial, double* __restrict__ cam_part) {
  if ((int)blockIdx.x < nb_obj) cf_obj_update_one(g, lambda, objs, bo, xo, objs_trial, obj_part, blockIdx.x * 256 + threadIdx.x);
  else slam_cam_update_one(g, lambda, cams, xc, bc, cams_trial, cam_part, ((int)blockIdx.x - nb_obj) * 256 + threadIdx.x);
}

template <class T>
static int al(T** dst, size_t n) {
  if (*dst) { (void)hipFree(*dst); *dst = nullptr; }
  ESL_HIP_TRY(hipMalloc((void**)dst, std::max<size_t>(n, 1) * sizeof(T)));
  return ESL_OK;
}

namespace {
struct BlobStage {
  struct Item { void** dst; size_t bytes, off; bool upload; };
  std::vector<Item> items;
  size_t total = 0, up_end = 0;
  BlobArena* a = nullptr;
  template <class T> int up(T** dst, size_t n) { return add((void**)dst, n * sizeof(T), true); }
  template <class T> int work(T** dst, size_t n) { return add((void**)dst, n * sizeof(T), false); }
  int add(void** dst, size_t bytes, bool upload) {
    const size_t off = (total + 255) / 256 * 256;
    items.push_back({dst, bytes, off, upload});
    total = off + std::max<size_t>(bytes, 8);
    if (upload) up_end = total;
    return (int)items.size() - 1;
  }
  int reserve(BlobArena& arena) {
    a = &arena;
    if (a->ev) ESL_HIP_TRY(hipEventSynchronize(a->ev));
    else ESL_HIP_TRY(hipEventCreateWithFlags(&a->ev, hipEventDisableTiming));
    if (up_end > a->host_cap) {
      if (a->host) { (void)hipHostFree(a->host); a->host = nullptr; a->host_cap = 0; }
      const size_t want = up_end + up_end / 2 + 4096;
      ESL_HIP_TRY(hipHostMalloc((void**)&a->host, want, hipHostMallocDefault));
      a->host_cap = want;
    }
    if (total > a->cap) {
      if (a->dev) { (void)hipFree(a->dev); a->dev = nullptr; a->cap = 0; }
      const size_t want = total + (total < ((size_t)1 << 30) ? total / 8 : 0) + 4096;
      ESL_HIP_TRY(hipMalloc((void**)&a->dev, want));
      a->cap = want;
    }
    for (const Item& it : items) *it.dst = a->dev + it.off;
    return ESL_OK;
  }
  template <class T> T* host(int i) const { return (T*)(a->host + items[(size_t)i].off); }
  int ship(hipStream_t st) {
    if (up_end) ESL_HIP_TRY(hipMemcpyAsync(a->dev, a->host, up_end, hipMemcpyHostToDevice, st));
    ESL_HIP_TRY(hipEventRecord(a->ev, st));
    return ESL_OK;
  }
};
double now_us() { return std::chrono::duration<double, std::micro>(std::chrono::steady_clock::now().time_since_epoch()).count(); }
}

static void cf_forget(esl_ctx* c);
void slam_forget(esl_ctx* c) {
  DevGraph& g = c->g;
  g.ue_start = g.ue_id = g.ue_slot = g.cu_start = g.cu_obj = g.cu_id = nullptr;
  c->Hcc = c->bc = c->xc = c->Wbb = c->Abb = c->Aod = c->Dinv = c->Yb = c->Wt = c->Tb = c->cam_part = c->od_part = c->z_ws = nullptr;
  c->cf_od_start = c->cf_od_edge = nullptr;
  c->S = c->Linv_ws = nullptr;
  c->pcg_M = nullptr;
  cf_forget(c);
  c->cf_chain_ok = false; c->cf_unavailable = false; c->chain_ok = false;
  c->h_ue_start.clear(); c->h_ue_id.clear(); c->h_ue_slot.clear();
  c->h_cu_start = c->h_cu_obj = c->h_cu_id = nullptr;
}
static void blob_release(BlobArena& a) {
  if (a.dev) (void)hipFree(a.dev);
  if (a.host) (void)hipHostFree(a.host);
  if (a.ev) (void)hipEventDestroy(a.ev);
  a = BlobArena{};
}
static void pcg_release(esl_ctx* c) {
  if (c->pcg_ws) (void)hipFree(c->pcg_ws);
  if (c->pcg_host) (void)hipHostFree(c->pcg_host);
  c->pcg_ws = c->pcg_st = c->pcg_M = c->pcg_host = nullptr; c->pcg_ws_cap = 0; c->pcg_ran = false;
}
void slam_release(esl_ctx* c) { slam_forget(c); blob_release(c->arena_slam); blob_release(c->arena_solve); blob_release(c->arena_S); pcg_release(c); }
void slam_trim(esl_ctx* c, bool keep_lists) {
  slam_sync_side(c);
  cf_forget(c);
  c->S = c->Linv_ws = nullptr;
  c->cf_unavailable = false;
  blob_release(c->arena_solve); blob_release(c->arena_S);
  if (!keep_lists) { slam_forget(c); blob_release(c->arena_slam); }
}

int slam_alloc(esl_ctx* c) {
  DevGraph& g = c->g;
  const int N = g.n_objs, F = g.n_cams, nf = g.n_free_cams;
  const bool timing = std::getenv("ESL_UPLOAD_HOST_TIMING") != nullptr;
  const double t0 = timing ? now_us() : 0;
  std::vector<int>& start = c->h_ue_start;
  std::vector<int>& id = c->h_ue_id;
  std::vector<int>& slot = c->h_ue_slot;
  start.assign((size_t)N + 1, 0);
  for (int i = 0; i < g.n_bbox; ++i) if (c->h_bb_obj[i] >= 0 && c->h_cam_slot[c->h_bb_cam[i]] >= 0) ++start[(size_t)c->h_bb_obj[i] + 1];
  for (int i = 0; i < g.n_e3d; ++i) if (c->h_e3_obj[i] >= 0 && c->h_cam_slot[c->h_e3_cam[i]] >= 0) ++start[(size_t)c->h_e3_obj[i] + 1];
  for (int o = 0; o < N; ++o) start[(size_t)o + 1] += start[o];
  const size_t nue = (size_t)start[N];
  id.resize(nue); slot.resize(nue);
  {
    std::vector<int> cur(start.begin(), start.end() - 1);
    for (int i = 0; i < g.n_bbox; ++i) {
      if (c->h_bb_obj[i] < 0) continue;
      const int s = c->h_cam_slot[c->h_bb_cam[i]];
      if (s >= 0) { const int at = cur[c->h_bb_obj[i]]++; id[at] = i; slot[at] = s; }
    }
    for (int i = 0; i < g.n_e3d; ++i) {
      if (c->h_e3_obj[i] < 0) continue;
      const int s = c->h_cam_slot[c->h_e3_cam[i]];
      if (s >= 0) { const int at = cur[c->h_e3_obj[i]]++; id[at] = g.n_bbox + i; slot[at] = s; }
    }
  }
  g.n_ue = (int)nue;
  std::vector<int> ods((size_t)std::max(nf, 1) + 1, 0), ode;
  bool chain = true;
  {
    std::vector<std::pair<int, int>> pe;
    for (int e = 0; e < g.n_odom; ++e) {
      const int si = c->h_cam_slot[c->h_od_i[e]], sj = c->h_cam_slot[c->h_od_j[e]];
      if (si < 0 || sj < 0) continue;
      if (si == sj + 1) pe.push_back({sj, e * 2});
      else if (sj == si + 1) pe.push_back({si, e * 2 + 1});
      else chain = false;
    }
    for (auto& p : pe) ++ods[(size_t)p.first + 1];
    for (int k = 0; k < nf; ++k) ods[(size_t)k + 1] += ods[k];
    ode.resize(pe.size());
    std::vector<int> cur(ods.begin(), ods.end() - 1);
    for (auto& p : pe) ode[(size_t)cur[p.first]++] = p.second;
  }
  c->cf_chain_ok = chain && nf > 0 && N > 0;
  c->chain_ok = chain && nf > 0;
  const double t1 = timing ? now_us() : 0;
  const size_t EU = (size_t)g.n_bbox + g.n_e3d;
  const int64_t n = 6 * (int64_t)nf;
  c->S_n = n;
  c->S_lda = ((n + 1 + 127) / 128) * 128;
  BlobStage st;
  const int i_ust = st.up(&g.ue_start, start.size()), i_uid = st.up(&g.ue_id, nue), i_usl = st.up(&g.ue_slot, nue);
  const int i_cst = st.up(&g.cu_start, (size_t)nf + 1), i_cob = st.up(&g.cu_obj, nue), i_cid = st.up(&g.cu_id, nue);
  const int i_ods = st.up(&c->cf_od_start, ods.size()), i_ode = st.up(&c->cf_od_edge, ode.size());
  st.work(&c->Hcc, (size_t)nf * 36); st.work(&c->bc, (size_t)nf * 6);
  st.work(&c->Wbb, EU * 54);
  st.work(&c->Abb, EU * 27);
  st.work(&c->Yb, EU * 54);
  st.work(&c->Wt, EU * 54);
  st.work(&c->Tb, EU * 6);
  st.work(&c->Aod, (size_t)g.n_odom * 90); st.work(&c->Dinv, (size_t)N * 81);
  st.work(&c->cam_part, (size_t)F * 4); st.work(&c->od_part, (size_t)g.n_odom);
  st.work(&c->xc, (size_t)n); st.work(&c->z_ws, (size_t)kNB);
  if (int rc = st.reserve(c->arena_slam)) return rc;
  std::memcpy(st.host<int>(i_ust), start.data(), start.size() * sizeof(int));
  if (nue) { std::memcpy(st.host<int>(i_uid), id.data(), nue * sizeof(int)); std::memcpy(st.host<int>(i_usl), slot.data(), nue * sizeof(int)); }
  std::memcpy(st.host<int>(i_ods), ods.data(), ods.size() * sizeof(int));
  if (!ode.empty()) std::memcpy(st.host<int>(i_ode), ode.data(), ode.size() * sizeof(int));
  {
    int* cstart = st.host<int>(i_cst); int* cobj = st.host<int>(i_cob); int* cid = st.host<int>(i_cid);
    c->h_cu_start = cstart; c->h_cu_obj = cobj; c->h_cu_id = cid;
    std::fill(cstart, cstart + nf + 1, 0);
    for (size_t k = 0; k < nue; ++k) ++cstart[(size_t)slot[k] + 1];
    g.cu_max = 0;
    for (int s = 0; s < nf; ++s) { g.cu_max = std::max(g.cu_max, cstart[(size_t)s + 1]); cstart[(size_t)s + 1] += cstart[s]; }
    std::vector<int> cur(cstart, cstart + nf);
    for (int o = 0; o < N; ++o)
      for (int k = start[o]; k < start[(size_t)o + 1]; ++k) { const int at = cur[slot[k]]++; cobj[at] = o; cid[at] = id[k]; }
  }
  if (int rc = st.ship(c->stream)) return rc;
  ESL_HIP_TRY(hipMemsetAsync(c->Abb, 0, std::max<size_t>(EU, 1) * 27 * sizeof(double), c->stream));
  ESL_HIP_TRY(hipMemsetAsync(c->Wbb, 0, std::max<size_t>(EU, 1) * 54 * sizeof(double), c->stream));
  if (timing) {
    const double t2 = now_us();
    ESL_HIP_TRY(hipStreamSynchronize(c->stream));
    fprintf(stderr, "[slam_alloc host, us] lists %.0f  layout + per-camera lists + enqueue %.0f  wait %.0f  (blob %.1f MB uploaded, %.1f MB in all)\n",
            t1 - t0, t2 - t1, now_us() - t2, st.up_end / 1e6, st.total / 1e6);
  }
  return ESL_OK;
}

static CholRuntime& chol_rt(esl_ctx* c);
static __global__ void k_info_to_double(const int* __restrict__ info, double* __restrict__ d) { d[0] = info[0] ? 1.0 : 0.0; }
static __global__ void k_double_to_info(const double* __restrict__ d, int* __restrict__ info) { if (d[0] > 0.5) info[0] |= 1; }
static int slam_ensure_S(esl_ctx* c) {
  if (c->S) return ESL_OK;
  const size_t n = (size_t)c->S_n, np = (n + kNB - 1) / kNB;
  BlobStage st;
  st.work(&c->S, (size_t)c->S_lda * n); st.work(&c->Linv_ws, np * kNB * kNB);
  const int rc = st.reserve(c->arena_S);
  if (rc) { c->S = c->Linv_ws = nullptr; return rc; }
  return st.ship(c->stream);
}

static int chol_pack_ensure(esl_ctx* c, int n) {
  const size_t need = chol_pack_len(n);
  if (c->chol_pack && c->chol_pack2 && c->chol_pack_len >= need) return ESL_OK;
  int rc = al(&c->chol_pack, need);
  if (rc) return rc;
  if ((rc = al(&c->chol_pack2, need))) return rc;
  c->chol_pack_len = need;
  return ESL_OK;
}
static int chol_dist_fill(esl_ctx* c, int n, CholDist& d) {
  d.rank = c->comm_rank; d.n_ranks = c->comm_ranks; d.user = c;
  d.bcast = [](void* u, double* dev, size_t count, int root) { return comm_bcast((esl_ctx*)u, dev, count, root); };
  const int rc = chol_pack_ensure(c, n);
  if (rc) return rc;
  d.pack = c->chol_pack;
  if (c->sw_chol_overlap) {
    d.pack2 = c->chol_pack2;
    d.bcast_on = [](void* u, double* dev, size_t count, int root, hipStream_t st) { return comm_bcast((esl_ctx*)u, dev, count, root, st); };
  }
  return ESL_OK;
}
static bool cf_applicable(const esl_ctx* c) { return c->cf_chain_ok && (!c->comm || c->comm_replicated); }
static bool cf_dist(const esl_ctx* c) {
  if (!c->comm || !c->comm_replicated || c->comm_ranks < 2) return false;
  if (c->sw_chol_dist >= 0) return c->sw_chol_dist == 1;
  return 9L * c->g.n_objs >= 8192;
}
static bool chain_applicable(const esl_ctx* c) { return c->chain_ok && c->g.n_ue == 0 && !c->comm; }
static int slam_pick_solver(const esl_ctx* c) {
  const int want = c->lm.p.linear_solver;
  if (want == ESL_SOLVER_PCG) return c->comm ? -3 : ESL_SOLVER_PCG;
  if (want == ESL_SOLVER_CAMERA_CHAIN) return chain_applicable(c) ? ESL_SOLVER_CAMERA_CHAIN : -2;
  if (want == ESL_SOLVER_AUTO && c->fx_on && chain_applicable(c)) return ESL_SOLVER_CAMERA_CHAIN;
  if (want == ESL_SOLVER_REDUCED_CAMERA) return ESL_SOLVER_REDUCED_CAMERA;
  if (want == ESL_SOLVER_REDUCED_ELLIPSOID) return cf_applicable(c) ? ESL_SOLVER_REDUCED_ELLIPSOID : -1;
  if (!cf_applicable(c) || c->cf_unavailable) return ESL_SOLVER_REDUCED_CAMERA;
  const double nc = (double)c->S_n, no = 9.0 * c->g.n_objs;
  return (no * no * nc + no * no * no / 3.0 < nc * nc * nc / 3.0) ? ESL_SOLVER_REDUCED_ELLIPSOID : ESL_SOLVER_REDUCED_CAMERA;
}
static void cf_forget(esl_ctx* c) {
  c->cf_oe_start = c->cf_oe_u = c->cf_oe_slot = c->cf_oe_cst = nullptr;
  c->cf_seg_start = c->cf_seg_obj = c->cf_seg_first = c->cf_cmap = c->cf_xld = c->cf_fwork = c->cf_twork = nullptr;
  c->cf_mask = nullptr; c->cf_xoff = c->cf_boff = c->cf_roff = nullptr;
  c->cf_Linv = c->cf_M = c->cf_N = c->cf_V = c->cf_B = c->cf_Lfac = c->cf_G = c->cf_vy = c->cf_z = nullptr;
  c->cf_T = c->cf_Linv_ws = c->cf_part = nullptr;
  c->cf_Zt = c->cf_Hs = c->cf_Bs = c->cf_LfacS = c->cf_GS = c->cf_LiS = c->cf_MS = c->cf_NS = c->cf_R = nullptr;
  c->cf_Xc = c->cf_Xs = c->cf_P = c->cf_Prhs = c->cf_Xt = c->cf_Y = c->cf_Yr = nullptr;
  c->cf_os_start = nullptr; c->cf_os_cnt = c->cf_os_pairs = c->cf_os_run = c->cf_os_heads = nullptr; c->cf_Vm = nullptr;
  c->cf_rank = c->cf_unrank = c->cf_kfirst = nullptr; c->cf_xo_t = nullptr;
  c->cf_plan = CfPlan{};
  c->cf_ready = false;
}
static int cf_ensure_impl(esl_ctx* c);
static int cf_ensure(esl_ctx* c) {
  if (c->cf_ready) return ESL_OK;
  const int rc = cf_ensure_impl(c);
  if (rc) { cf_forget(c); (void)hipGetLastError(); return rc; }
  c->cf_ready = true;
  return ESL_OK;
}
static_assert(kCfKC == kKC, "esl_cf_plan.hpp pads K to the rank-K update's chunk");
static int cf_ensure_impl(esl_ctx* c) {
  const DevGraph& g = c->g;
  const int N = g.n_objs, nfi = g.n_free_cams;
  const size_t nf = (size_t)nfi, EU = (size_t)g.n_bbox + g.n_e3d, n_o = (size_t)9 * N;
  const bool timing = std::getenv("ESL_UPLOAD_HOST_TIMING") != nullptr;
  const double t0 = timing ? now_us() : 0;
  CfSwitches sw;
  { const char* e = std::getenv("ESL_CF_SPARSE"); sw.sparse = e ? (int)(unsigned char)e[0] : -1; }
  { const char* e = std::getenv("ESL_CF_TPERM"); sw.tperm_off = e && e[0] == '0'; }
  sw.no_nd = std::getenv("ESL_CF_NO_ND") != nullptr;
  static const int nd_min = [] { const char* e = std::getenv("ESL_CF_ND_MIN"); return e ? std::atoi(e) : 48; }();
  sw.nd_min = nd_min; sw.stride = c->sw_cf_stride; sw.os_kernel = c->sw_cf_os_kernel; sw.os_list = c->sw_cf_os_list;
  size_t free_b = 0, total_b = 0;
  if (nfi >= kCfSparseMinCams) ESL_HIP_TRY(hipMemGetInfo(&free_b, &total_b));
  CfPlan& pl = c->cf_plan;
  if (!cf_plan_build(N, nfi, EU, c->h_ue_start, c->h_cu_start, c->h_cu_obj, c->h_cu_id, c->cf_chain_ok, c->comm != nullptr, total_b, sw, pl)) {
    set_error("camera-first elimination: the (ellipsoid, camera chunk) range table of this graph exceeds 1 GB");
    return ESL_ERR_ALLOC;
  }
  const bool sp = pl.sparse, os3 = sp && pl.form == 3, osm = os3 && pl.os_list;
  const int nch = pl.n_chunks, nseg = pl.nseg, nw = pl.nw, N1 = N + 1;
  const size_t n_inc = pl.p.size();
  const size_t y_recs = std::max<size_t>(n_inc, 1) * (size_t)(pl.S - 1), nb = (size_t)N * (N + 1) / 2 + N;
  const double t1 = timing ? now_us() : 0;
  BlobStage st;
  struct Up { int item; const void* src; size_t bytes; };
  std::vector<Up> ups;
  auto ship = [&](auto** dst, const auto& v) { ups.push_back({st.up(dst, v.size()), v.data(), v.size() * sizeof(v[0])}); };
  ship(&c->cf_oe_start, c->h_ue_start); ship(&c->cf_oe_u, pl.ou); ship(&c->cf_oe_slot, pl.os);
  int* d_inc = nullptr; int* d_fw_off = nullptr; long long* d_tw_off = nullptr;
  int i_inc = -1;
  if (pl.tperm) { ship(&c->cf_rank, pl.rank); ship(&c->cf_unrank, pl.unrank); ship(&c->cf_kfirst, pl.kfirst); }
  if (sp) {
    i_inc = st.up(&d_inc, 4 * n_inc); ship(&c->cf_seg_start, pl.seg_start); ship(&c->cf_xld, pl.xld);
    ship(&c->cf_xoff, pl.xoff); ship(&c->cf_boff, pl.boff); ship(&c->cf_roff, pl.roff); ship(&d_fw_off, pl.fw_off); ship(&d_tw_off, pl.tw_off);
  }
  if (osm) { ship(&c->cf_os_run, pl.os_run); ship(&c->cf_os_heads, pl.os_heads); }
  st.work(&c->cf_oe_cst, (size_t)std::max(N, 1) * (nch + 1));
  if (sp) {
    st.work(&c->cf_cmap, (size_t)nseg * N1); st.work(&c->cf_mask, (size_t)N1 * nw); st.work(&c->cf_seg_obj, n_inc); st.work(&c->cf_seg_first, n_inc);
    st.work(&c->cf_fwork, 2 * (size_t)pl.n_fwork); st.work(&c->cf_twork, 3 * (size_t)pl.n_twork);
  }
  st.work(&c->cf_Linv, nf * 36); st.work(&c->cf_M, nf * 36); st.work(&c->cf_N, nf * 36); st.work(&c->cf_V, EU * 54);
  st.work(&c->cf_B, nf * 36); st.work(&c->cf_Lfac, nf * 21); st.work(&c->cf_G, nf * 36); st.work(&c->cf_vy, nf * 6); st.work(&c->cf_z, nf * 6);
  st.work(&c->cf_T, (size_t)pl.ldt * n_o); st.work(&c->cf_Linv_ws, ((n_o + kNB - 1) / kNB) * kNB * kNB);
  if (pl.tperm) st.work(&c->cf_xo_t, n_o);
  if (n_o <= 1024) st.work(&c->cf_part, (size_t)kCholMaxSplit * (size_t)pl.ldt * n_o);
  if (pl.nd) {
    const size_t ns = (size_t)std::max(pl.n_sep, 1);
    st.work(&c->cf_Zt, nf * 36); st.work(&c->cf_Hs, ns * 36); st.work(&c->cf_Bs, ns * 36); st.work(&c->cf_LfacS, ns * 21);
    st.work(&c->cf_GS, ns * 36); st.work(&c->cf_LiS, ns * 36); st.work(&c->cf_MS, ns * 36); st.work(&c->cf_NS, ns * 36);
    st.work(&c->cf_R, ns * 6 * (size_t)pl.ldx);
  }
  if (sp) {
    st.work(&c->cf_Xc, pl.xc_len); st.work(&c->cf_Xs, (size_t)pl.ldx * (size_t)pl.kpad_s);
    if (pl.form == 1) { st.work(&c->cf_P, pl.p_blocks * 81); st.work(&c->cf_Prhs, pl.prhs_len); }
    if (pl.form == 3) {
      st.work(&c->cf_Y, y_recs * 54); st.work(&c->cf_Yr, std::max<size_t>(nf, 1) * 6);
      st.work(&c->cf_os_start, nb + 1); st.work(&c->cf_os_cnt, nb); st.work(&c->cf_os_pairs, 2 * std::max<size_t>(pl.os_list_npairs, 1));
      if (osm) st.work(&c->cf_Vm, EU * 54);
    }
  } else {
    st.work(&c->cf_Xt, (size_t)pl.ldx * (size_t)pl.kpad);
  }
  if (int rc = st.reserve(c->arena_solve)) return rc;
  for (const Up& u : ups) if (u.bytes) std::memcpy(st.host<char>(u.item), u.src, u.bytes);
  if (sp && n_inc) {
    int* inc = st.host<int>(i_inc);
    std::memcpy(inc, pl.p.data(), n_inc * sizeof(int)); std::memcpy(inc + n_inc, pl.o.data(), n_inc * sizeof(int));
    std::memcpy(inc + 2 * n_inc, pl.first.data(), n_inc * sizeof(int));
    for (size_t q = 0; q < n_inc; ++q) inc[3 * n_inc + q] = (int)q;
  }
  if (int rc = st.ship(c->stream)) return rc;
  if (N > 0) {
    const long nt = (long)N * (nch + 1);
    hipLaunchKernelGGL(k_cf_make_cst, dim3((unsigned)((nt + 255) / 256)), dim3(256), 0, c->stream, N, nch, c->cf_oe_start, c->cf_oe_slot, c->cf_oe_cst);
  }
  if (sp) {
    ESL_HIP_TRY(hipMemsetAsync(c->cf_cmap, 0xFF, (size_t)nseg * N1 * sizeof(int), c->stream));
    ESL_HIP_TRY(hipMemsetAsync(c->cf_mask, 0, (size_t)N1 * nw * sizeof(unsigned long long), c->stream));
    if (n_inc)
      hipLaunchKernelGGL(k_cf_make_cmap, dim3((unsigned)((n_inc + 255) / 256)), dim3(256), 0, c->stream, (int)n_inc, d_inc, N1, nw, c->cf_seg_start, c->cf_cmap,
                         c->cf_mask, c->cf_seg_obj, c->cf_seg_first);
    hipLaunchKernelGGL(k_cf_make_work, dim3((unsigned)nseg), dim3(64), 0, c->stream, nseg, N, nw, c->cf_seg_start, d_fw_off, d_tw_off, c->cf_cmap, c->cf_mask,
                       c->cf_fwork, c->cf_twork);
  }
  if (os3) {
    const dim3 grid((unsigned)(N + 1), (unsigned)((N + kCfTPer - 1) / kCfTPer));
    ESL_HIP_TRY(hipMemsetAsync(c->cf_os_cnt, 0, nb * sizeof(int), c->stream));
    hipLaunchKernelGGL(k_cf_os_list<false>, grid, dim3(256), 0, c->stream, N, nw, nch, pl.S / kCfFwdCh, c->cf_mask, c->cf_cmap, c->cf_seg_start, c->cf_oe_cst, c->cf_oe_slot,
                       (const int*)c->cf_unrank, (const long long*)nullptr, c->cf_os_cnt, (int2*)nullptr, 0, (const int*)c->cf_os_run, (const int*)c->cf_os_heads);
    std::vector<int> h_cnt(nb);
    std::vector<long long> h_start(nb + 1);
    ESL_HIP_TRY(hipMemcpyAsync(h_cnt.data(), c->cf_os_cnt, nb * sizeof(int), hipMemcpyDeviceToHost, c->stream));
    ESL_HIP_TRY(hipStreamSynchronize(c->stream));
    h_start[0] = 0;
    for (size_t b = 0; b < nb; ++b) h_start[b + 1] = h_start[b] + h_cnt[b];
    if ((size_t)h_start[nb] != pl.os_list_npairs) {
      set_error("camera-first elimination: the one-sided assembly's pair list does not have the length the host counted");
      return ESL_ERR_STATE;
    }
    ESL_HIP_TRY(hipMemcpyAsync(c->cf_os_start, h_start.data(), (nb + 1) * sizeof(long long), hipMemcpyHostToDevice, c->stream));
    hipLaunchKernelGGL(k_cf_os_list<true>, grid, dim3(256), 0, c->stream, N, nw, nch, pl.S / kCfFwdCh, c->cf_mask, c->cf_cmap, c->cf_seg_start, c->cf_oe_cst, c->cf_oe_slot,
                       (const int*)c->cf_unrank, (const long long*)c->cf_os_start, c->cf_os_cnt, (int2*)c->cf_os_pairs, pl.os_offsets ? 1 : 0,
                       (const int*)c->cf_os_run, (const int*)c->cf_os_heads);
    ESL_HIP_TRY(hipStreamSynchronize(c->stream));
  }
  if (pl.nd) ESL_HIP_TRY(hipMemsetAsync(c->cf_Zt, 0, nf * 36 * sizeof(double), c->stream));
  if (sp) {
    ESL_HIP_TRY(hipMemsetAsync(c->cf_Xc, 0, std::max<size_t>(pl.xc_len, 1) * sizeof(double), c->stream));
    ESL_HIP_TRY(hipMemsetAsync(c->cf_Xs, 0, (size_t)pl.ldx * (size_t)pl.kpad_s * sizeof(double), c->stream));
    ESL_HIP_TRY(hipMemsetAsync(c->cf_T, 0, (size_t)pl.ldt * n_o * sizeof(double), c->stream));
    if (pl.form == 3) {
      ESL_HIP_TRY(hipMemsetAsync(c->cf_Y, 0, y_recs * 54 * sizeof(double), c->stream));
      ESL_HIP_TRY(hipMemsetAsync(c->cf_Yr, 0, std::max<size_t>(nf, 1) * 6 * sizeof(double), c->stream));
    }
  } else {
    ESL_HIP_TRY(hipMemsetAsync(c->cf_Xt, 0, (size_t)pl.ldx * (size_t)pl.kpad * sizeof(double), c->stream));
  }
  ESL_HIP_TRY(hipMemsetAsync(c->cf_V, 0, std::max<size_t>(EU, 1) * 54 * sizeof(double), c->stream));
  if (timing)
    fprintf(stderr, "[cf_ensure host, us] sorts + structure %.0f  layout + tables + enqueue %.0f  (blob %.1f MB uploaded, %.1f MB in all; sparse %d form %d)\n",
            t1 - t0, now_us() - t1, st.up_end / 1e6, st.total / 1e6, (int)sp, pl.form);
  return ESL_OK;
}

namespace {
struct CfSideJoin {
  CholRuntime& rt; hipStream_t main; bool armed;
  hipError_t wait(hipEvent_t ev) { const hipError_t e = hipStreamWaitEvent(main, ev, 0); armed = e != hipSuccess; return e; }
  ~CfSideJoin() {
    if (!armed) return;
    if (hipEventRecord(rt.cf_ev_p, rt.cf_side) != hipSuccess || hipStreamWaitEvent(main, rt.cf_ev_p, 0) != hipSuccess) (void)hipStreamSynchronize(rt.cf_side);
  }
};
struct CfTrial {
  esl_ctx* c; CholRuntime& rt; const CfPlan& pl; const DevGraph& g; const double lambda;
  const int N, nf, n_o; const long ldx, ldt;
  const int st, ns, nseg;
  const bool nd, dist;
  const unsigned cg;
  const hipStream_t main;
  CfSideJoin join;
  CfTrial(esl_ctx* c_, CholRuntime& rt_, double lambda_)
      : c(c_), rt(rt_), pl(c_->cf_plan), g(c_->g), lambda(lambda_), N(g.n_objs), nf(g.n_free_cams), n_o(9 * N), ldx((long)pl.ldx), ldt((long)pl.ldt),
        st(pl.stride), ns(pl.n_sep), nseg(pl.n_seg), nd(st > 0 && ns > 0), dist(cf_dist(c_)), cg((unsigned)((n_o + 1 + 63) / 64)), main(c_->stream),
        join{rt_, c_->stream, false} {}
  CfSegs segs() const { return CfSegs{c->cf_fwork, c->cf_seg_start, c->cf_seg_obj, c->cf_xoff, c->cf_xld, c->cf_rank, c->cf_unrank}; }
  int edge_blocks() const { return (int)(((long)pl.n_list * 9 + nf + 255) / 256); }
  template <class F> void my_columns(F f) const {
    if (!dist) { f(0L, (long)n_o); return; }
    const int Wp = chol_outer_panels(n_o), n_outer = ((n_o + kNB - 1) / kNB + Wp - 1) / Wp;
    for (int op = c->comm_rank; op < n_outer; op += c->comm_ranks) f((long)op * Wp * kNB, std::min<long>((long)(op + 1) * Wp * kNB, (long)n_o));
  }
  dim3 block_grid(long c_begin, long c_end, int& o2b, int& o2e) const {
    o2b = (int)(c_begin / 9); o2e = (int)((c_end + 8) / 9);
    return dim3((unsigned)(N + 1), (unsigned)((o2e - o2b + kCfTPer - 1) / kCfTPer));
  }
  void edge_scale(int cls, hipStream_t s) const {
    hipLaunchKernelGGL(k_cf_edge_scale, dim3((unsigned)edge_blocks()), dim3(256), 0, s, g, pl.n_list, c->cf_oe_u, c->cf_oe_slot, c->Wbb, c->cf_Linv, c->bc,
                       c->cf_V, c->cf_vy, cls, st);
  }
  void segment_chains() const {
    hipLaunchKernelGGL(k_cf_chain, dim3((unsigned)nseg), dim3(64), 0, main, nf, c->Hcc, c->cf_B, lambda, c->cf_Lfac, c->cf_G, c->chol_info, st, st - 1);
    hipLaunchKernelGGL(k_cf_factor_blocks, dim3((unsigned)((nf + 63) / 64)), dim3(64), 0, main, nf, c->cf_Lfac, c->cf_G, c->cf_Linv, c->cf_M, c->cf_N, st);
    if (nseg > 1) hipLaunchKernelGGL(k_cf_zt, dim3((unsigned)(nseg - 1)), dim3(64), 0, main, nf, st, c->cf_Linv, c->cf_M, c->cf_B, c->cf_Zt);
    hipLaunchKernelGGL(k_cf_sep_assemble, dim3((unsigned)((ns * 36 + 255) / 256)), dim3(256), 0, main, nf, st, ns, c->Hcc, lambda, c->cf_G, c->cf_Zt,
                       c->cf_Hs, c->cf_Bs);
  }
  void sep_chain(hipStream_t s) const {
    hipLaunchKernelGGL(k_cf_chain, dim3(1), dim3(64), 0, s, ns, c->cf_Hs, c->cf_Bs, 0.0, c->cf_LfacS, c->cf_GS, c->chol_info, ns, ns);
    hipLaunchKernelGGL(k_cf_factor_blocks, dim3((unsigned)((ns + 63) / 64)), dim3(64), 0, s, ns, c->cf_LfacS, c->cf_GS, c->cf_LiS, c->cf_MS, c->cf_NS, 0,
                       c->cf_Linv, st);
  }
  int slabs(bool beside) {
    segment_chains();
    if (beside) {
      ESL_HIP_TRY(hipEventRecord(rt.cf_ev_a, main));
      ESL_HIP_TRY(hipStreamWaitEvent(rt.cf_side, rt.cf_ev_a, 0));
      join.armed = true;
    }
    sep_chain(beside ? rt.cf_side : main);
    if (beside) ESL_HIP_TRY(hipEventRecord(rt.cf_ev_s, rt.cf_side));
    edge_scale(beside ? 1 : 0, main);
    auto forward = [&](auto parts) {
      hipLaunchKernelGGL((k_cf_forward<2, decltype(parts)::value>), dim3((unsigned)pl.n_fwork), dim3(64), 0, main, nf, n_o, pl.n_chunks, c->cf_oe_cst, c->cf_oe_slot,
                         c->cf_V, c->cf_vy, c->cf_M, c->cf_Xc, ldx, st, st - 1, (const double*)c->cf_Zt, c->cf_R, st, segs());
    };
    if (c->sw_cf_fwd_parts == 8) forward(std::integral_constant<int, 8>{});
    else if (c->sw_cf_fwd_parts == 4) forward(std::integral_constant<int, 4>{});
    else forward(std::integral_constant<int, 2>{});
    return ESL_OK;
  }
  void sep_rhs(hipStream_t s, bool sp = true) const {
    hipLaunchKernelGGL(k_cf_sep_rhs, dim3(cg, (unsigned)ns), dim3(64), 0, s, nf, n_o, st, pl.n_chunks, c->cf_oe_cst, c->cf_oe_slot, c->cf_V, c->cf_vy,
                       c->cf_G, c->cf_LiS, sp ? c->cf_Xc : c->cf_Xt, ldx, c->cf_R, sp ? (const int*)c->cf_cmap : nullptr, sp ? segs() : CfSegs{});
  }
  void sep_forward(hipStream_t s, bool sp = true) const {
    hipLaunchKernelGGL(k_cf_forward<1>, dim3(cg), dim3(64), 0, s, ns, n_o, pl.n_chunks, c->cf_oe_cst, c->cf_oe_slot, c->cf_V, c->cf_vy,
                       c->cf_MS, sp ? c->cf_Xs : c->cf_Xt, ldx, ns, ns, (const double*)nullptr, c->cf_R, sp ? 0 : st, CfSegs{});
  }
  void products(hipStream_t s) const {
    hipLaunchKernelGGL(k_cf_seg_syrk, dim3((unsigned)pl.n_twork), dim3(256), 0, s, c->cf_twork, c->cf_seg_start, c->cf_seg_first, c->cf_xoff,
                       c->cf_xld, c->cf_Xc, c->cf_boff, c->cf_P);
    hipLaunchKernelGGL(k_cf_seg_rhs, dim3((unsigned)pl.n_fwork), dim3(64), 0, s, c->cf_fwork, c->cf_seg_start, c->cf_xoff, c->cf_xld, c->cf_Xc,
                       c->cf_roff, c->cf_Prhs);
  }
  void gather_products(long c_begin, long c_end, int accumulate) const {
    int o2b, o2e;
    const dim3 grid = block_grid(c_begin, c_end, o2b, o2e);
    hipLaunchKernelGGL(k_cf_T_gather, grid, dim3(256), 0, main, N, pl.nw, c->cf_mask, c->cf_cmap, c->cf_boff, c->cf_roff, c->cf_P, c->cf_Prhs,
                       c->Hoo, c->bo, lambda, c->cf_T, ldt, o2b, o2e, (const int*)c->cf_unrank, accumulate);
  }
  void update() const {
    ProfScope pk(c, 7);
    const double* Xf = pl.sparse ? c->cf_Xs : c->cf_Xt;
    const int K = (int)(pl.sparse ? pl.kpad_s : pl.kpad);
    if (!dist && K <= 0) return;
    my_columns([&](long c_begin, long c_end) {
      chol_launch_update(rt.sw, c->cf_T, ldt, (long)n_o + 1, main, 0, K, c_begin, c_end, Xf, ldx, dist ? nullptr : c->cf_part, pl.sparse ? c->cf_kfirst : nullptr);
    });
  }

  int build_dense() {
    auto edge_scale_T = [&] {
      const int nb_es = edge_blocks();
      hipLaunchKernelGGL(k_cf_edge_scale_T, dim3((unsigned)(nb_es + (int)((ldt * (long)n_o + 255) / 256))), dim3(256), 0, main, g, nb_es, pl.n_list, c->cf_oe_u,
                         c->cf_oe_slot, c->Wbb, c->cf_Linv, c->bc, c->cf_V, c->cf_vy, c->Hoo, c->bo, lambda, c->cf_T, ldt, (long)n_o);
    };
    if (!nd) {
      hipLaunchKernelGGL(k_cf_chain, dim3(1), dim3(64), 0, main, nf, c->Hcc, c->cf_B, lambda, c->cf_Lfac, c->cf_G, c->chol_info, nf, nf);
      hipLaunchKernelGGL(k_cf_factor_blocks, dim3((unsigned)((nf + 63) / 64)), dim3(64), 0, main, nf, c->cf_Lfac, c->cf_G, c->cf_Linv, c->cf_M, c->cf_N, 0);
      edge_scale_T();
      hipLaunchKernelGGL(k_cf_forward<0>, dim3(cg), dim3(64), 0, main, nf, n_o, pl.n_chunks, c->cf_oe_cst, c->cf_oe_slot, c->cf_V, c->cf_vy,
                         c->cf_M, c->cf_Xt, ldx, nf, nf, (const double*)nullptr, (double*)nullptr, 0, CfSegs{});
    } else {
      segment_chains();
      sep_chain(main);
      edge_scale_T();
      hipLaunchKernelGGL(k_cf_forward<0>, dim3(cg, (unsigned)nseg), dim3(64), 0, main, nf, n_o, pl.n_chunks, c->cf_oe_cst, c->cf_oe_slot, c->cf_V,
                         c->cf_vy, c->cf_M, c->cf_Xt, ldx, st, st - 1, (const double*)c->cf_Zt, c->cf_R, st, CfSegs{});
      sep_rhs(main, false);
      sep_forward(main, false);
    }
    ESL_HIP_TRY(hipGetLastError());
    update();
    return ESL_OK;
  }

  int build_stored_serial() {
    if (int rc = slabs(false)) return rc;
    sep_rhs(main);
    sep_forward(main);
    {
      ProfScope pk(c, 8);
      if (pl.form == 1) products(main);
      my_columns([&](long c_begin, long c_end) {
        if (pl.form == 1) { gather_products(c_begin, c_end, 0); return; }
        int o2b, o2e;
        const dim3 grid = block_grid(c_begin, c_end, o2b, o2e);
        hipLaunchKernelGGL(k_cf_T_sparse, grid, dim3(256), 0, main, N, pl.nw, c->cf_mask, c->cf_cmap, c->cf_xoff, c->cf_xld, c->cf_Xc, c->Hoo, c->bo,
                           lambda, c->cf_T, ldt, o2b, o2e, (const int*)c->cf_unrank);
      });
    }
    ESL_HIP_TRY(hipGetLastError());
    update();
    return ESL_OK;
  }

  int build_stored_side(int ov) {
    const bool side_chain = ov != 3, early_products = ov != 2;
    if (int rc = slabs(side_chain)) return rc;
    if (side_chain) {
      ESL_HIP_TRY(join.wait(rt.cf_ev_s));
      edge_scale(2, main);
    }
    sep_rhs(main);
    if (early_products) ESL_HIP_TRY(hipEventRecord(rt.cf_ev_x, main));
    sep_forward(main);
    if (!early_products) ESL_HIP_TRY(hipEventRecord(rt.cf_ev_x, main));
    ESL_HIP_TRY(hipStreamWaitEvent(rt.cf_side, rt.cf_ev_x, 0));
    join.armed = true;
    products(rt.cf_side);
    ESL_HIP_TRY(hipEventRecord(rt.cf_ev_p, rt.cf_side));
    if (chol_update_v_applies(rt.sw, ldt, (long)n_o + 1, 0, (long)n_o, true, ldx)) {
      {
        ProfScope pk(c, 7);
        chol_launch_update(rt.sw, c->cf_T, ldt, (long)n_o + 1, main, 0, (int)pl.kpad_s, 0, (long)n_o, c->cf_Xs, ldx, nullptr, c->cf_kfirst, true, ov == 4);
      }
      ESL_HIP_TRY(join.wait(rt.cf_ev_p));
      ProfScope pk(c, 8);
      gather_products(0, (long)n_o, 1);
    } else {
      ESL_HIP_TRY(join.wait(rt.cf_ev_p));
      {
        ProfScope pk(c, 8);
        gather_products(0, (long)n_o, 0);
      }
      ESL_HIP_TRY(hipGetLastError());
      update();
    }
    return ESL_OK;
  }

  int build_onesided(bool beside) {
    const hipStream_t sst = beside ? rt.cf_side : main;
    if (int rc = slabs(beside)) return rc;
    if (beside) {
      ESL_HIP_TRY(hipEventRecord(rt.cf_ev_x, main));
      ESL_HIP_TRY(hipStreamWaitEvent(rt.cf_side, rt.cf_ev_x, 0));
      edge_scale(2, rt.cf_side);
    }
    sep_rhs(sst);
    sep_forward(sst);
    if (beside) ESL_HIP_TRY(hipEventRecord(rt.cf_ev_p, rt.cf_side));
    {
      ProfScope pk(c, 8);
      auto seg_back = [&](auto mch) {
        hipLaunchKernelGGL(k_cf_seg_back<decltype(mch)::value>, dim3((unsigned)pl.n_fwork), dim3(64), 0, main, nf, c->cf_fwork, c->cf_seg_start, c->cf_xoff,
                           c->cf_xld, c->cf_Xc, c->cf_Linv, c->cf_G, c->cf_Y, c->cf_Yr);
      };
      if (st == 3 * kCfFwdCh) seg_back(std::integral_constant<int, 3>{});
      else if (st == 2 * kCfFwdCh) seg_back(std::integral_constant<int, 2>{});
      else seg_back(std::integral_constant<int, 1>{});
      if (pl.os_list && pl.n_list > 0)
        hipLaunchKernelGGL(k_cf_v_merge, dim3((unsigned)(((long)pl.n_list * 9 + 255) / 256)), dim3(256), 0, main, pl.n_list, (const int*)c->cf_os_run, c->cf_V, c->cf_Vm);
      const dim3 grid((unsigned)(N + 1), (unsigned)((N + kCfTPer - 1) / kCfTPer));
      hipLaunchKernelGGL(pl.os_offsets ? k_cf_T_onesided_lds : k_cf_T_onesided, grid, dim3(256), 0, main, N, (const int2*)c->cf_os_pairs,
                         (const long long*)c->cf_os_start, (const int*)c->cf_os_cnt, pl.os_list ? c->cf_Vm : c->cf_V, c->cf_Y, c->cf_Yr, c->Hoo, c->bo, lambda, c->cf_T, ldt, 0, N,
                         (const int*)c->cf_unrank, 0);
    }
    ESL_HIP_TRY(hipGetLastError());
    if (beside) ESL_HIP_TRY(join.wait(rt.cf_ev_p));
    update();
    return ESL_OK;
  }

  int back_substitute() const {
    {
      ProfScope ps(c, 3);
      double* xsol = (pl.sparse && pl.tperm) ? c->cf_xo_t : c->xo;
      if (dist) {
        CholDist d;
        if (int rc = chol_dist_fill(c, n_o, d)) return rc;
        ESL_HIP_TRY(chol_factor_solve(c->cf_T, ldt, n_o, c->cf_Linv_ws, c->z_ws, xsol, c->chol_info, main, rt, &d));
      } else {
        ESL_HIP_TRY(chol_factor_solve(c->cf_T, ldt, n_o, c->cf_Linv_ws, c->z_ws, xsol, c->chol_info, main, rt));
      }
      if (xsol != c->xo) hipLaunchKernelGGL(k_cf_xo_unpermute, dim3((unsigned)((n_o + 255) / 256)), dim3(256), 0, main, N, c->cf_rank, xsol, c->xo);
      if (pl.sparse)
        hipLaunchKernelGGL(k_cf_z_sparse, dim3((unsigned)(6 * nf)), dim3(256), 0, main, n_o, c->cf_Xs, ldx, segs(), c->cf_Xc, c->xo, xsol, c->cf_z, st);
      else
        hipLaunchKernelGGL(k_cf_z, dim3((unsigned)(6 * nf)), dim3(256), 0, main, c->cf_Xt, ldx, n_o, c->xo, c->cf_z);
      if (nd) {
        hipLaunchKernelGGL(k_cf_tridiag_back, dim3(1), dim3(64), 0, main, ns, c->cf_LiS, c->cf_NS, c->cf_z, c->xc, ns, ns, st);
        hipLaunchKernelGGL(k_cf_back_prep, dim3((unsigned)((6 * nf + 255) / 256)), dim3(256), 0, main, nf, st, ns, c->cf_Zt, c->cf_G, c->xc, c->cf_z);
        hipLaunchKernelGGL(k_cf_tridiag_back, dim3((unsigned)nseg), dim3(64), 0, main, nf, c->cf_Linv, c->cf_N, c->cf_z, c->xc, st, st - 1, 0);
      } else {
        hipLaunchKernelGGL(k_cf_tridiag_back, dim3(1), dim3(64), 0, main, nf, c->cf_Linv, c->cf_N, c->cf_z, c->xc, nf, nf, 0);
      }
      ESL_HIP_TRY(hipGetLastError());
    }
    ProfScope ps(c, 1);
    const int F = g.n_cams, nb_obj = (N + 255) / 256, nb_cam = (F + 255) / 256;
    hipLaunchKernelGGL(k_cf_updates, dim3((unsigned)(nb_obj + nb_cam)), dim3(256), 0, main, g, nb_obj, lambda, c->objs, c->bo, c->xo, c->objs_trial, c->obj_part,
                       c->cams, c->xc, c->bc, c->cams_trial, c->cam_part);
    const int nb_co = (N + kWavesPerBlock - 1) / kWavesPerBlock, nb_od = (g.n_odom + kWave * kWavesPerBlock - 1) / (kWave * kWavesPerBlock);
    robust_dispatch(c->robust_on, [&](auto robust) {
      hipLaunchKernelGGL(k_slam_chi2_all<decltype(robust)::value>, dim3((unsigned)(nb_co + nb_od)), dim3(kWave * kWavesPerBlock), 0, main, g, nb_co,
                         c->cams_trial, c->objs_trial, c->obj_part, c->od_part);
    });
    ESL_HIP_TRY(hipGetLastError());
    return ESL_OK;
  }
};
}
static int slam_try_step_cf(esl_ctx* c, double lambda) {
  int rc = cf_ensure(c);
  if (rc) return rc;
  const CfPlan& pl = c->cf_plan;
  CfTrial t(c, chol_rt(c), lambda);
  {
    ProfScope ps(c, 2);
    ESL_HIP_TRY(hipMemsetAsync(c->chol_info, 0, sizeof(int), c->stream));
    hipLaunchKernelGGL(k_cf_gather_B, dim3((unsigned)(((long)t.nf * 36 + 255) / 256)), dim3(256), 0, c->stream, t.nf, c->Aod, c->cf_od_start, c->cf_od_edge, c->cf_B);
    ESL_HIP_TRY(chol_set_attributes(t.rt));
    if (!pl.sparse) rc = t.build_dense();
    else if (!t.nd) {
      set_error("camera-first elimination: sparse X needs the dissected camera chain");
      rc = ESL_ERR_STATE;
    }
    else {
      const bool side = c->sw_cf_overlap != 0 && (pl.form == 1 || pl.form == 3) && !t.dist && pl.kpad_s > 0 && t.rt.cf_overlap_init() == hipSuccess;
      rc = pl.form == 3 ? t.build_onesided(side) : side ? t.build_stored_side(c->sw_cf_overlap) : t.build_stored_serial();
    }
    if (rc) return rc;
    ESL_HIP_TRY(hipGetLastError());
  }
  return t.back_substitute();
}

static bool slam_dist_chol(esl_ctx* c) {
  if (!c->comm || c->comm_ranks < 2) return false;
  if (c->sw_chol_dist >= 0) return c->sw_chol_dist == 1;
  return c->S_n >= 8192;
}
static void chol_prof_mark(void* user, int begin) {
  esl_ctx* c = (esl_ctx*)user;
  if (begin) { if (!c->chol_prof_scope) c->chol_prof_scope = new ProfScope(c, 9); }
  else if (c->chol_prof_scope) { delete (ProfScope*)c->chol_prof_scope; c->chol_prof_scope = nullptr; }
}
static CholRuntime& chol_rt(esl_ctx* c) {
  if (!c->chol_rt) {
    CholRuntime* rt = new CholRuntime();
    rt->prof_mark = chol_prof_mark; rt->prof_user = c;
    c->chol_rt = rt;
  }
  return *(CholRuntime*)c->chol_rt;
}
void slam_sync_side(esl_ctx* c) {
  if (c->chol_rt && ((CholRuntime*)c->chol_rt)->cf_side) (void)hipStreamSynchronize(((CholRuntime*)c->chol_rt)->cf_side);
}
void slam_release_runtime(esl_ctx* c) {
  if (c->chol_prof_scope) { delete (ProfScope*)c->chol_prof_scope; c->chol_prof_scope = nullptr; }
  if (!c->chol_rt) return;
  ((CholRuntime*)c->chol_rt)->release();
  delete (CholRuntime*)c->chol_rt;
  c->chol_rt = nullptr;
  c->schur_attr_set = false;
}

static int reduce_all(esl_ctx* c, const int* info = nullptr) {
  const DevGraph& g = c->g;
  hipLaunchKernelGGL(k_slam_reduce_all, dim3(1), dim3(256), 0, c->stream, c->obj_part, g.n_objs, c->cam_part, g.n_cams, c->od_part,
                     (g.n_odom && g.shard_rank == 0) ? g.n_odom : 0, c->dev_part, info);
  ESL_HIP_TRY(hipGetLastError());
  return ESL_OK;
}

int slam_linearize(esl_ctx* c) {
  c->parts_fresh = false;
  const DevGraph& g = c->g;
  const int N = g.n_objs, F = g.n_cams;
  const bool an = c->lm.p.jacobian_mode == ESL_JAC_ANALYTIC;
  const double delta = c->lm.p.numeric_delta;
  {
    ProfScope ps(c, 0);
    if (N > 0) {
      ChunkTable ct;
      ct.n_chunks = c->n_chunks; ct.obj = c->ck_obj; ct.type = c->ck_type; ct.begin = c->ck_begin; ct.end = c->ck_end; ct.ostart = c->ck_ostart;
      const dim3 block(64 * kLinWaves);
      const int nb_e3 = (c->n_ids_e3 + kLinWaves - 1) / kLinWaves, nb_bb = (c->n_ids_bb + kLinWaves - 1) / kLinWaves;
      robust_dispatch(c->robust_on, [&](auto robust) {
        constexpr bool R = decltype(robust)::value;
        if (an) {
          if (nb_e3) hipLaunchKernelGGL((k_slam_linearize_chunks<ESL_JAC_ANALYTIC, 1, R>), dim3(nb_e3), block, 0, c->stream, g, ct, c->ck_ids_e3, c->n_ids_e3, c->cams,
                                        c->objs, delta, c->chunk_out, c->Wbb, c->Abb);
          if (nb_bb) hipLaunchKernelGGL((k_slam_linearize_chunks<ESL_JAC_ANALYTIC, 0, R>), dim3(nb_bb), block, 0, c->stream, g, ct, c->ck_ids_bb, c->n_ids_bb, c->cams,
                                        c->objs, delta, c->chunk_out, c->Wbb, c->Abb);
          hipLaunchKernelGGL((k_slam_combine<ESL_JAC_ANALYTIC, R>), dim3((N + kWavesPerBlock - 1) / kWavesPerBlock), dim3(kWave * kWavesPerBlock), 0, c->stream, g, ct,
                             c->chunk_out, c->objs, delta, c->Hoo, c->bo, c->obj_part);
        } else {
          if (nb_e3) hipLaunchKernelGGL((k_slam_linearize_chunks<ESL_JAC_NUMERIC, 1, R>), dim3(nb_e3), block, 0, c->stream, g, ct, c->ck_ids_e3, c->n_ids_e3, c->cams,
                                        c->objs, delta, c->chunk_out, c->Wbb, c->Abb);
          if (nb_bb) hipLaunchKernelGGL((k_slam_linearize_chunks<ESL_JAC_NUMERIC, 0, R>), dim3(nb_bb), block, 0, c->stream, g, ct, c->ck_ids_bb, c->n_ids_bb, c->cams,
                                        c->objs, delta, c->chunk_out, c->Wbb, c->Abb);
          hipLaunchKernelGGL((k_slam_combine<ESL_JAC_NUMERIC, R>), dim3((N + kWavesPerBlock - 1) / kWavesPerBlock), dim3(kWave * kWavesPerBlock), 0, c->stream, g, ct,
                             c->chunk_out, c->objs, delta, c->Hoo, c->bo, c->obj_part);
        }
      });
    }
    if (g.n_odom) {
      const dim3 grid((g.n_odom + 127) / 128), block(128);
      robust_dispatch(c->robust_on, [&](auto robust) {
        constexpr bool R = decltype(robust)::value;
        if (an) hipLaunchKernelGGL((k_slam_odom<ESL_JAC_ANALYTIC, R>), grid, block, 0, c->stream, g, c->cams, delta, c->Aod, c->od_part);
        else hipLaunchKernelGGL((k_slam_odom<ESL_JAC_NUMERIC, R>), grid, block, 0, c->stream, g, c->cams, delta, c->Aod, c->od_part);
      });
    }
    hipLaunchKernelGGL(k_slam_cam_gather, dim3((F + kWavesPerBlock - 1) / kWavesPerBlock), dim3(kWave * kWavesPerBlock), 0, c->stream, g, c->Abb, c->Aod,
                       c->Hcc, c->bc, c->cam_part);
    if (c->fx_on && c->fx.n_bb + c->fx.n_e3 > 0) {
      const AnchGraph& a = c->fx;
      robust_dispatch(c->robust_on, [&](auto robust) {
        constexpr bool R = decltype(robust)::value;
        const dim3 gb((a.n_bb + 63) / 64), ge((a.n_e3 + 63) / 64);
        if (an) {
          if (a.n_bb) hipLaunchKernelGGL((k_anch_linearize<ESL_JAC_ANALYTIC, 0, R>), gb, dim3(64), 0, c->stream, g, a, c->cams, c->objs, delta, c->fx_A, c->fx_chi);
          if (a.n_e3) hipLaunchKernelGGL((k_anch_linearize<ESL_JAC_ANALYTIC, 1, R>), ge, dim3(64), 0, c->stream, g, a, c->cams, c->objs, delta, c->fx_A, c->fx_chi);
        } else {
          if (a.n_bb) hipLaunchKernelGGL((k_anch_linearize<ESL_JAC_NUMERIC, 0, R>), gb, dim3(64), 0, c->stream, g, a, c->cams, c->objs, delta, c->fx_A, c->fx_chi);
          if (a.n_e3) hipLaunchKernelGGL((k_anch_linearize<ESL_JAC_NUMERIC, 1, R>), ge, dim3(64), 0, c->stream, g, a, c->cams, c->objs, delta, c->fx_A, c->fx_chi);
        }
      });
      hipLaunchKernelGGL(k_anch_gather, dim3((F + kWavesPerBlock - 1) / kWavesPerBlock), dim3(kWave * kWavesPerBlock), 0, c->stream, g, a, c->fx_A, c->fx_chi,
                         c->Hcc, c->bc, c->cam_part);
    }
    if (c->comm && !c->comm_replicated) {
      int rc2 = comm_allreduce_sum(c, c->Hcc, (size_t)g.n_free_cams * 36);
      if (!rc2) rc2 = comm_allreduce_sum(c, c->bc, (size_t)g.n_free_cams * 6);
      if (rc2) return rc2;
      hipLaunchKernelGGL(k_slam_cam_maxdiag, dim3((F + 127) / 128), dim3(128), 0, c->stream, g, c->Hcc, c->cam_part);
    }
// ... 495 lines not shown
```

Baseline: 19.19.

## Fuse segment forward and back substitution into a twisted-factorization sweep

Adds a twisted-factorization kernel that precomputes per-frame P/Q matrices from the chain factors, run on a side stream. A single sweep kernel then replaces the forward plus segment-back passes, writing only a compact last-row XL buffer instead of the full Xc. After the object solve, camera back-substitution is recomputed from V, vy and xo, and the sparse z kernel runs only on separator rows. This is meant to drop the seg_back pass and the Xc memset and traffic, at the cost of extra 6x6 algebra per frame and more numerical steps.

```diff
diff --git a/object-oriented-slam_amd/csrc/esl_capi.hip b/object-oriented-slam_amd/csrc/esl_capi.hip
--- a/object-oriented-slam_amd/csrc/esl_capi.hip
+++ b/object-oriented-slam_amd/csrc/esl_capi.hip
@@ -125,6 +125,7 @@
   { const char* ov = std::getenv("ESL_CF_OVERLAP"); c->sw_cf_overlap = (ov && ov[0] >= '0' && ov[0] <= '4') ? ov[0] - '0' : 4; }
   { const char* ok = std::getenv("ESL_CF_OS_KERNEL"); c->sw_cf_os_kernel = (ok && ok[0] == '0') ? 0 : 1; }
   { const char* ol = std::getenv("ESL_CF_OS_LIST"); c->sw_cf_os_list = (ol && ol[0] == '0') ? 0 : 1; }
+  { const char* sp = std::getenv("ESL_CF_SWEEP"); c->sw_cf_sweep = (sp && sp[0] == '0') ? 0 : 1; }
   { const char* fp = std::getenv("ESL_CF_FWD_PARTS"); const int v = fp ? std::atoi(fp) : 0; if (v == 2 || v == 4 || v == 8) c->sw_cf_fwd_parts = v; }
   { const char* sd = std::getenv("ESL_CF_STRIDE"); const int v = sd ? std::atoi(sd) : 0; c->sw_cf_stride = (v == 16 || v == 32 || v == 48) ? v : 0; }
   auto init = [&]() -> int {
diff --git a/object-oriented-slam_amd/csrc/esl_cf.hpp b/object-oriented-slam_amd/csrc/esl_cf.hpp
--- a/object-oriented-slam_amd/csrc/esl_cf.hpp
+++ b/object-oriented-slam_amd/csrc/esl_cf.hpp
@@ -439,7 +439,7 @@
                                                           const double* __restrict__ vy, const double* __restrict__ Gfac,
                                                           const double* __restrict__ LiS, const double* __restrict__ Xt, long ldx,
                                                           double* __restrict__ R, const int* __restrict__ cmap ,
-                                                          CfSegs sg) {
+                                                          CfSegs sg, const double* __restrict__ XL = nullptr, long long xl_rows = 1) {
   const int j = blockIdx.x * 64 + threadIdx.x, k = blockIdx.y;
   if (j > n_o) return;
   const bool rhs = j == n_o;
@@ -468,7 +468,12 @@
     const int ob = rhs ? N1 - 1 : (sg.unrank ? sg.unrank[tb2] : tb2);
     has_acc = has_acc && cmap[(size_t)(k + 1) * N1 + ob] >= 0;
     const int e = cmap[(size_t)k * N1 + ob];
-    if (e >= 0) {
+    if (e >= 0 && XL) {
+      const double* src = XL + (size_t)(sg.xoff[k] / xl_rows) * 6 + (size_t)(9 * (e & 0xFFFFFF) + bb);
+      const size_t ld = (size_t)sg.xld[k];
+#pragma unroll
+      for (int r = 0; r < 6; ++r) xl[r] = src[(size_t)r * ld];
+    } else if (e >= 0) {
       const double* src = Xt + (size_t)sg.xoff[k] + (size_t)(9 * (e & 0xFFFFFF) + bb);
       const size_t ld = (size_t)sg.xld[k];
 #pragma unroll
@@ -687,9 +692,9 @@
 
 static __global__ __launch_bounds__(256) void k_cf_z_sparse(int n_o, const double* __restrict__ Xs, long ldx, CfSegs sg, const double* __restrict__ Xc,
                                                             const double* __restrict__ xo, const double* __restrict__ xo_t, double* __restrict__ z,
-                                                            int stride) {
+                                                            int stride, int sep_only = 0) {
   __shared__ double red[4];
-  const int t = blockIdx.x, i = t / 6, a = t - 6 * i;
+  const int t = sep_only ? 6 * (((int)blockIdx.x / 6) * stride + stride - 1) + (int)blockIdx.x % 6 : (int)blockIdx.x, i = t / 6, a = t - 6 * i;
   const int p = i / stride, pos = i - p * stride;
   double s = 0, y;
   if (pos == stride - 1) {
diff --git a/object-oriented-slam_amd/csrc/esl_cf_plan.hpp b/object-oriented-slam_amd/csrc/esl_cf_plan.hpp
--- a/object-oriented-slam_amd/csrc/esl_cf_plan.hpp
+++ b/object-oriented-slam_amd/csrc/esl_cf_plan.hpp
@@ -43,6 +43,7 @@
   int stride = 0;
   int os_kernel = 1;
   int os_list = 1;
+  int sweep = 1;
 };
 
 struct CfSegTables {
@@ -70,6 +71,9 @@
   std::vector<int> os_run, os_heads;
   size_t osm_npairs = 0, osm_row_npairs = 0, os_list_npairs = 0;
   double osm_flops = 0;
+  bool sweep = false;
+  std::vector<int> sl_ent;
+  size_t xl_len = 0;
   bool tperm = false;
   std::vector<int> rank, unrank, kfirst;
   double upd_flops = 0;
@@ -272,6 +276,16 @@
     cf_os_sides(pl, start);
     pl.os_list = sw.os_list != 0;
     pl.os_list_npairs = pl.os_list ? pl.osm_npairs : pl.os_npairs;
+    pl.sweep = sw.sweep != 0;
+    if (pl.sweep) {
+      std::vector<int> cur(start.begin(), start.end() - 1);
+      pl.sl_ent.assign((size_t)cu_start[nf], 0);
+      for (int sl = 0; sl < nf; ++sl)
+        for (int q = cu_start[sl]; q < cu_start[sl + 1]; ++q) pl.sl_ent[(size_t)q] = cur[cu_obj[q]]++;
+      long long cols = 0;
+      for (int x : pl.xld) cols += x;
+      pl.xl_len = 6 * (size_t)cols;
+    }
   }
   return true;
 }
diff --git a/object-oriented-slam_amd/csrc/esl_cf_sweep.hpp b/object-oriented-slam_amd/csrc/esl_cf_sweep.hpp
--- /dev/null
+++ b/object-oriented-slam_amd/csrc/esl_cf_sweep.hpp
@@ -0,0 +1,502 @@
+#pragma once
+#include "esl_cf.hpp"
+
+namespace esl {
+
+constexpr int kCfSweepSI = 3 * kCfFwdCh - 1;
+
+#define CF_LT(r, c) ((r) * ((r) + 1) / 2 + (c))
+__device__ __forceinline__ void cf_chol6(double (&d)[21], double (&is)[6], bool& ok) {
+#pragma unroll
+  for (int j = 0; j < 6; ++j) {
+    const double p = d[CF_LT(j, j)];
+    ok = ok && (p > 0);
+    double q = __builtin_amdgcn_rsq(p);
+    q = q * (1.5 - 0.5 * p * q * q);
+    q = q * (1.5 - 0.5 * p * q * q);
+    is[j] = q;
+    d[CF_LT(j, j)] = p * q;
+#pragma unroll
+    for (int r = j + 1; r < 6; ++r) d[CF_LT(r, j)] *= q;
+#pragma unroll
+    for (int r = j + 1; r < 6; ++r)
+#pragma unroll
+      for (int c = j + 1; c <= r; ++c) d[CF_LT(r, c)] -= d[CF_LT(r, j)] * d[CF_LT(c, j)];
+  }
+}
+
+static __global__ __launch_bounds__(64) void k_cf_twist(int nf_all, int stride, const double* __restrict__ Hcc, double lambda,
+                                                        const double* __restrict__ Lfac, const double* __restrict__ Gfac,
+                                                        double* __restrict__ Pm, double* __restrict__ Qm, int* __restrict__ info) {
+  __shared__ double sH[kCfSweepSI * 36], sG[kCfSweepSI * 36], sL[kCfSweepSI * 21];
+  const int lane = threadIdx.x;
+  const int beg = (int)blockIdx.x * stride;
+  const int len = ((beg + stride - 1 < nf_all) ? beg + stride - 1 : nf_all) - beg;
+  if (len <= 0) return;
+  {
+    constexpr int kQ = (kCfSweepSI * 36 + 63) / 64, kL = (kCfSweepSI * 21 + 63) / 64;
+    double th[kQ], tg[kQ], tl[kL];
+#pragma unroll
+    for (int q = 0; q < kQ; ++q) {
+      const int idx = q * 64 + lane, cl = idx < len * 36 ? idx : 0;
+      th[q] = Hcc[(size_t)beg * 36 + cl]; tg[q] = Gfac[(size_t)beg * 36 + cl];
+    }
+#pragma unroll
+    for (int q = 0; q < kL; ++q) { const int idx = q * 64 + lane; tl[q] = Lfac[(size_t)beg * 21 + (idx < len * 21 ? idx : 0)]; }
+#pragma unroll
+    for (int q = 0; q < kQ; ++q) if (q * 64 + lane < kCfSweepSI * 36) { sH[q * 64 + lane] = th[q]; sG[q * 64 + lane] = tg[q]; }
+#pragma unroll
+    for (int q = 0; q < kL; ++q) if (q * 64 + lane < kCfSweepSI * 21) sL[q * 64 + lane] = tl[q];
+  }
+  __builtin_amdgcn_wave_barrier();
+  bool ok = true;
+  double K[21], isk[6];
+#pragma unroll
+  for (int k = 0; k < 21; ++k) K[k] = 0;
+#pragma unroll
+  for (int k = 0; k < 6; ++k) isk[k] = 0;
+  for (int i = len - 1; i >= 0; --i) {
+    double dm[21], P[36], Q[36];
+    if (i == len - 1) {
+#pragma unroll
+      for (int r = 0; r < 6; ++r)
+#pragma unroll
+        for (int c = 0; c < 6; ++c) { P[r * 6 + c] = r == c ? 1.0 : 0.0; Q[r * 6 + c] = 0.0; }
+#pragma unroll
+      for (int r = 0; r < 6; ++r)
+#pragma unroll
+        for (int c = 0; c <= r; ++c) dm[CF_LT(r, c)] = sH[i * 36 + r * 6 + c] + ((r == c) ? lambda : 0.0);
+    } else {
+      double g[36], h[36], L[21], Ln[21];
+#pragma unroll
+      for (int k = 0; k < 36; ++k) g[k] = sG[i * 36 + k];
+#pragma unroll
+      for (int k = 0; k < 21; ++k) { L[k] = sL[i * 21 + k]; Ln[k] = sL[(i + 1) * 21 + k]; }
+#pragma unroll
+      for (int c = 0; c < 6; ++c)
+#pragma unroll
+        for (int r = 0; r < 6; ++r) {
+          double v = g[c * 6 + r];
+#pragma unroll
+          for (int k = 0; k < r; ++k) v -= K[CF_LT(r, k)] * h[k * 6 + c];
+          h[r * 6 + c] = v * isk[r];
+        }
+      double S[36];
+#pragma unroll
+      for (int a = 0; a < 6; ++a)
+#pragma unroll
+        for (int b = 0; b <= a; ++b) {
+          double v = 0;
+#pragma unroll
+          for (int r = 0; r < 6; ++r) v += h[r * 6 + a] * h[r * 6 + b];
+          S[a * 6 + b] = v; S[b * 6 + a] = v;
+        }
+      double C[21], ic[6], Ci[36];
+#pragma unroll
+      for (int a = 0; a < 6; ++a)
+#pragma unroll
+        for (int b = 0; b <= a; ++b) C[CF_LT(a, b)] = ((a == b) ? 1.0 : 0.0) - S[a * 6 + b];
+      cf_chol6(C, ic, ok);
+#pragma unroll
+      for (int c = 0; c < 6; ++c)
+#pragma unroll
+        for (int r = 0; r < 6; ++r) {
+          if (r < c) { Ci[r * 6 + c] = 0; continue; }
+          double v = (r == c) ? 1.0 : 0.0;
+#pragma unroll
+          for (int k = c; k < r; ++k) v -= C[CF_LT(r, k)] * Ci[k * 6 + c];
+          Ci[r * 6 + c] = v * ic[r];
+        }
+#pragma unroll
+      for (int a = 0; a < 6; ++a)
+#pragma unroll
+        for (int b = 0; b <= a; ++b) {
+          double v = 0;
+#pragma unroll
+          for (int k = a; k < 6; ++k) v += Ci[k * 6 + a] * Ci[k * 6 + b];
+          P[a * 6 + b] = v; P[b * 6 + a] = v;
+        }
+      double t1[36];
+#pragma unroll
+      for (int c = 0; c < 6; ++c)
+#pragma unroll
+        for (int r = 0; r < 6; ++r) {
+          if (r < c) { t1[r * 6 + c] = 0; continue; }
+          double v = Ln[CF_LT(r, c)];
+#pragma unroll
+          for (int k = c; k < r; ++k) v -= K[CF_LT(r, k)] * t1[k * 6 + c];
+          t1[r * 6 + c] = v * isk[r];
+        }
+#pragma unroll
+      for (int a = 0; a < 6; ++a)
+#pragma unroll
+        for (int b = 0; b < 6; ++b) {
+          double v = 0;
+#pragma unroll
+          for (int r = b; r < 6; ++r) v += h[r * 6 + a] * t1[r * 6 + b];
+          Q[a * 6 + b] = v;
+        }
+      double U[36];
+#pragma unroll
+      for (int r = 0; r < 6; ++r)
+#pragma unroll
+        for (int c = 0; c < 6; ++c) {
+          double v = 0;
+#pragma unroll
+          for (int k = 0; k <= r; ++k) v += L[CF_LT(r, k)] * S[k * 6 + c];
+          U[r * 6 + c] = v;
+        }
+#pragma unroll
+      for (int r = 0; r < 6; ++r)
+#pragma unroll
+        for (int c = 0; c <= r; ++c) {
+          double v = sH[i * 36 + r * 6 + c] + ((r == c) ? lambda : 0.0);
+#pragma unroll
+          for (int k = 0; k <= c; ++k) v -= U[r * 6 + k] * L[CF_LT(c, k)];
+          dm[CF_LT(r, c)] = v;
+        }
+    }
+    cf_chol6(dm, isk, ok);
+#pragma unroll
+    for (int k = 0; k < 21; ++k) K[k] = dm[k];
+    if (lane == 0) {
+#pragma unroll
+      for (int k = 0; k < 36; ++k) { sH[i * 36 + k] = P[k]; sG[i * 36 + k] = Q[k]; }
+    }
+  }
+  __builtin_amdgcn_wave_barrier();
+  for (int idx = lane; idx < len * 36; idx += 64) { Pm[(size_t)beg * 36 + idx] = sH[idx]; Qm[(size_t)beg * 36 + idx] = sG[idx]; }
+  if (!ok && lane == 0) atomicOr(info, 1);
+}
+#undef CF_LT
+
+template <int PARTS>
+static __global__ __launch_bounds__(64) void k_cf_sweep(int nf_all, int n_o, int n_chunks, const int* __restrict__ oe_cst, const int* __restrict__ oe_slot,
+                                                        const double* __restrict__ V, const double* __restrict__ vy, const double* __restrict__ Mm,
+                                                        const double* __restrict__ Zt, const double* __restrict__ Pm, const double* __restrict__ Qm,
+                                                        double* __restrict__ R, long ldx, int stride, CfSegs sg, double* __restrict__ Y,
+                                                        double* __restrict__ Yr, double* __restrict__ XL, long long xl_rows) {
+  static_assert(PARTS == 2 || PARTS == 4 || PARTS == 8, "halves, quarters or eighths of a chunk");
+  constexpr int CH = kCfFwdCh / PARTS;
+  constexpr int kQ = kCfFwdCh * 36 / 64;
+  __shared__ double sA[kCfFwdCh * 36], sB[kCfFwdCh * 36], sP[kCfFwdCh * 36];
+  __shared__ double sv[CH * 6 * 64];
+  __shared__ double svy[kCfFwdCh * 6];
+  const int lane = threadIdx.x;
+  const int seg = sg.fwork[2 * blockIdx.x];
+  const int j = sg.fwork[2 * blockIdx.x + 1] * 64 + lane;
+  const int ob = sg.seg_start[seg];
+  const int jr = 9 * (sg.seg_start[seg + 1] - ob);
+  const bool on = j <= jr, rhs = j == jr, col = on && !rhs;
+  const int oi = col ? j / 9 : 0, b = j - 9 * oi;
+  const int o = col ? sg.seg_obj[ob + oi] : 0;
+  const long tcol = rhs ? (long)n_o : 9L * (sg.rank ? sg.rank[o] : o) + b;
+  const int SI = stride - 1;
+  const int beg = seg * stride;
+  const int nf = (beg + SI < nf_all) ? beg + SI : nf_all;
+  if (beg >= nf) return;
+  const int len = nf - beg;
+  const bool use_z = Zt != nullptr && seg >= 1;
+  const int* cst = oe_cst + (size_t)o * (n_chunks + 1);
+  constexpr int kE = 4;
+  int s_first = len, s_last = -1, ecnt = 0;
+  int eslot[kE];
+  double erec[kE][6];
+#pragma unroll
+  for (int e = 0; e < kE; ++e) {
+    eslot[e] = -1;
+#pragma unroll
+    for (int a = 0; a < 6; ++a) erec[e][a] = 0.0;
+  }
+  if (rhs) { s_first = 0; s_last = len - 1; }
+  else if (col) {
+    const int c0 = beg / kCfFwdCh, c1 = (c0 + stride / kCfFwdCh < n_chunks) ? c0 + stride / kCfFwdCh : n_chunks;
+    const int ka = cst[c0], kb = cst[c1];
+    if (ka < kb) {
+      const int f = oe_slot[ka] - beg;
+      int k = kb - 1, l = oe_slot[k] - beg;
+      while (l >= len && k > ka) { --k; l = oe_slot[k] - beg; }
+      if (f < len) {
+        s_first = f; s_last = l; ecnt = k - ka + 1;
+#pragma unroll
+        for (int e = 0; e < kE; ++e) {
+          const int kk = e < ecnt ? ka + e : ka;
+          eslot[e] = oe_slot[kk] - beg;
+          const double* src = V + ((size_t)kk * 9 + b) * 6;
+#pragma unroll
+          for (int a = 0; a < 6; ++a) erec[e][a] = src[a];
+        }
+      }
+    }
+  }
+  const bool fast = !__any(ecnt > kE);
+  double* dst = rhs ? Yr + (size_t)beg * 6 : Y + ((size_t)(ob + oi) * SI) * 54 + b * 6;
+  const int dstep = rhs ? 6 : 54;
+  auto gather = [&](int ch, int h0, int p0, int hl) {
+#pragma unroll
+    for (int q = 0; q < CH * 6; ++q) sv[q * 64 + lane] = 0.0;
+    __builtin_amdgcn_wave_barrier();
+    if (rhs) {
+#pragma unroll
+      for (int q = 0; q < CH * 6; ++q) sv[q * 64 + lane] = (q < hl * 6) ? svy[h0 * 6 + q] : 0.0;
+    } else if (col && fast) {
+#pragma unroll
+      for (int e = 0; e < kE; ++e) {
+        const int at = eslot[e] - p0;
+        if (e < ecnt && at >= 0 && at < hl) {
+#pragma unroll
+          for (int a = 0; a < 6; ++a) sv[(at * 6 + a) * 64 + lane] += erec[e][a];
+        }
+      }
+    } else if (col) {
+      const int ka = cst[ch], kb = cst[ch + 1];
+      for (int k = ka; k < kb; k += 4) {
+        int sl[4];
+        double rec[4][6];
+#pragma unroll
+        for (int e = 0; e < 4; ++e) {
+          const int kk = (k + e < kb) ? k + e : ka;
+          sl[e] = oe_slot[kk];
+          const double* src = V + ((size_t)kk * 9 + b) * 6;
+#pragma unroll
+          for (int a = 0; a < 6; ++a) rec[e][a] = src[a];
+        }
+#pragma unroll
+        for (int e = 0; e < 4; ++e) {
+          const int at = sl[e] - beg - p0;
+          if (k + e < kb && at >= 0 && at < hl) {
+#pragma unroll
+            for (int a = 0; a < 6; ++a) sv[(at * 6 + a) * 64 + lane] += rec[e][a];
+          }
+        }
+      }
+    }
+    __builtin_amdgcn_wave_barrier();
+  };
+  double x[6] = {0, 0, 0, 0, 0, 0}, acc[6] = {0, 0, 0, 0, 0, 0};
+  for (int i0 = beg; i0 < nf; i0 += kCfFwdCh) {
+    const int ch = i0 / kCfFwdCh;
+    const int clen = (nf - i0 < kCfFwdCh) ? nf - i0 : kCfFwdCh;
+    if (!__any(on && s_first < i0 - beg + clen)) continue;
+    __builtin_amdgcn_wave_barrier();
+    {
+      double tm[kQ], tz[kQ], tp[kQ], ty[2];
+#pragma unroll
+      for (int q = 0; q < kQ; ++q) {
+        const int idx = q * 64 + lane, cl = idx < clen * 36 ? idx : 0;
+        tm[q] = Mm[(size_t)i0 * 36 + cl];
+        tz[q] = use_z ? Zt[(size_t)i0 * 36 + cl] : 0.0;
+        tp[q] = Pm[(size_t)i0 * 36 + cl];
+      }
+#pragma unroll
+      for (int q = 0; q < 2; ++q) { const int idx = q * 64 + lane; ty[q] = vy[(size_t)i0 * 6 + (idx < clen * 6 ? idx : 0)]; }
+#pragma unroll
+      for (int q = 0; q < kQ; ++q) { sA[q * 64 + lane] = tm[q]; sB[q * 64 + lane] = tz[q]; sP[q * 64 + lane] = tp[q]; }
+#pragma unroll
+      for (int q = 0; q < 2; ++q) if (q * 64 + lane < kCfFwdCh * 6) svy[q * 64 + lane] = ty[q];
+    }
+    __builtin_amdgcn_wave_barrier();
+    for (int h0 = 0; h0 < clen; h0 += CH) {
+      const int hl = (clen - h0 < CH) ? clen - h0 : CH;
+      const int p0 = i0 - beg + h0;
+      if (!__any(on && s_first < p0 + hl)) continue;
+      gather(ch, h0, p0, hl);
+      for (int ii = 0; ii < hl; ++ii) {
+        const double* M = sA + (h0 + ii) * 36;
+        double xn[6];
+#pragma unroll
+        for (int a = 0; a < 6; ++a) {
+          double t = sv[(ii * 6 + a) * 64 + lane];
+#pragma unroll
+          for (int q = 0; q < 6; ++q) t -= M[a * 6 + q] * x[q];
+          xn[a] = t;
+        }
+#pragma unroll
+        for (int a = 0; a < 6; ++a) x[a] = xn[a];
+        if (use_z) {
+          const double* Z = sB + (h0 + ii) * 36;
+#pragma unroll
+          for (int a = 0; a < 6; ++a)
+#pragma unroll
+            for (int q = 0; q < 6; ++q) acc[a] += Z[q * 6 + a] * xn[q];
+        }
+        const double* P = sP + (h0 + ii) * 36;
+#pragma unroll
+        for (int a = 0; a < 6; ++a) {
+          double t = 0;
+#pragma unroll
+          for (int q = 0; q < 6; ++q) t += P[a * 6 + q] * xn[q];
+          sv[(ii * 6 + a) * 64 + lane] = t;
+        }
+      }
+      if (on) {
+#pragma unroll
+        for (int q0 = 0; q0 < CH * 6; q0 += 8) {
+          double t[8];
+#pragma unroll
+          for (int e = 0; e < 8; ++e) t[e] = sv[((q0 + e < hl * 6) ? q0 + e : 0) * 64 + lane];
+#pragma unroll
+          for (int e = 0; e < 8; ++e) {
+            const int q = q0 + e, pos = p0 + q / 6;
+            if (q < hl * 6 && pos >= s_first) dst[(size_t)pos * dstep + q % 6] = t[e];
+          }
+        }
+      }
+      __builtin_amdgcn_wave_barrier();
+    }
+  }
+  if (use_z && on) {
+#pragma unroll
+    for (int a = 0; a < 6; ++a) R[(size_t)tcol + (size_t)(6 * (seg - 1) + a) * (size_t)ldx] = acc[a];
+  }
+  if (on && len == SI) {
+    double* xl = XL + (size_t)(sg.xoff[seg] / xl_rows) * 6 + (size_t)j;
+    const size_t ld = (size_t)sg.xld[seg];
+#pragma unroll
+    for (int a = 0; a < 6; ++a) xl[(size_t)a * ld] = x[a];
+  }
+  double u[6] = {0, 0, 0, 0, 0, 0};
+  for (int i0 = beg + ((len - 1) / kCfFwdCh) * kCfFwdCh; i0 >= beg; i0 -= kCfFwdCh) {
+    const int ch = i0 / kCfFwdCh;
+    const int clen = (nf - i0 < kCfFwdCh) ? nf - i0 : kCfFwdCh;
+    if (!__any(on && s_last >= i0 - beg)) continue;
+    __builtin_amdgcn_wave_barrier();
+    {
+      double tq[kQ], tp[kQ], ty[2];
+#pragma unroll
+      for (int q = 0; q < kQ; ++q) {
+        const int idx = q * 64 + lane, cl = idx < clen * 36 ? idx : 0;
+        tq[q] = Qm[(size_t)i0 * 36 + cl];
+        tp[q] = Pm[(size_t)i0 * 36 + cl];
+      }
+#pragma unroll
+      for (int q = 0; q < 2; ++q) { const int idx = q * 64 + lane; ty[q] = vy[(size_t)i0 * 6 + (idx < clen * 6 ? idx : 0)]; }
+#pragma unroll
+      for (int q = 0; q < kQ; ++q) { sA[q * 64 + lane] = tq[q]; sP[q * 64 + lane] = tp[q]; }
+#pragma unroll
+      for (int q = 0; q < 2; ++q) if (q * 64 + lane < kCfFwdCh * 6) svy[q * 64 + lane] = ty[q];
+    }
+    __builtin_amdgcn_wave_barrier();
+    for (int h0 = ((clen - 1) / CH) * CH; h0 >= 0; h0 -= CH) {
+      const int hl = (clen - h0 < CH) ? clen - h0 : CH;
+      const int p0 = i0 - beg + h0;
+      if (!__any(on && s_last >= p0)) continue;
+      gather(ch, h0, p0, hl);
+      for (int ii = hl - 1; ii >= 0; --ii) {
+        const double* Qi = sA + (h0 + ii) * 36;
+        const bool both = p0 + ii >= s_first;
+        double un[6], d[6];
+#pragma unroll
+        for (int a = 0; a < 6; ++a) {
+          const double v = sv[(ii * 6 + a) * 64 + lane];
+          double t = v;
+#pragma unroll
+          for (int q = 0; q < 6; ++q) t -= Qi[a * 6 + q] * u[q];
+          un[a] = t;
+          d[a] = both ? t - v : t;
+        }
+#pragma unroll
+        for (int a = 0; a < 6; ++a) u[a] = un[a];
+        const double* P = sP + (h0 + ii) * 36;
+#pragma unroll
+        for (int a = 0; a < 6; ++a) {
+          double t = 0;
+#pragma unroll
+          for (int q = 0; q < 6; ++q) t += P[a * 6 + q] * d[q];
+          sv[(ii * 6 + a) * 64 + lane] = t;
+        }
+      }
+      if (on) {
+        const bool rmw = __any(s_first < s_last && s_first < p0 + hl && p0 < s_last) != 0;
+#pragma unroll
+        for (int q0 = 0; q0 < CH * 6; q0 += 8) {
+          double t[8], old[8];
+#pragma unroll
+          for (int e = 0; e < 8; ++e) t[e] = sv[((q0 + e < hl * 6) ? q0 + e : 0) * 64 + lane];
+          if (rmw) {
+#pragma unroll
+            for (int e = 0; e < 8; ++e) {
+              const int q = q0 + e, pos = p0 + q / 6;
+              old[e] = (q < hl * 6 && pos >= s_first && pos < s_last) ? dst[(size_t)pos * dstep + q % 6] : 0.0;
+            }
+          } else {
+#pragma unroll
+            for (int e = 0; e < 8; ++e) old[e] = 0.0;
+          }
+#pragma unroll
+          for (int e = 0; e < 8; ++e) {
+            const int q = q0 + e, pos = p0 + q / 6;
+            if (q < hl * 6 && pos < s_last) dst[(size_t)pos * dstep + q % 6] = (pos >= s_first) ? old[e] + t[e] : t[e];
+          }
+        }
+      }
+      __builtin_amdgcn_wave_barrier();
+    }
+  }
+}
+
+static __global__ __launch_bounds__(64) void k_cf_wxo(int stride, const int* __restrict__ sl_start, const int* __restrict__ sl_ent,
+                                                      const int* __restrict__ sl_obj, const double* __restrict__ V, const double* __restrict__ vy,
+                                                      const double* __restrict__ xo, double* __restrict__ z) {
+  __shared__ double red[64];
+  const int i = blockIdx.x, lane = threadIdx.x;
+  if (i % stride == stride - 1) return;
+  const int l = lane < 54 ? lane : 0, b = l / 6;
+  const int qa = sl_start[i], qb = sl_start[i + 1];
+  double s = 0;
+  for (int q = qa; q < qb; q += 4) {
+    double v[4], w[4];
+#pragma unroll
+    for (int e = 0; e < 4; ++e) {
+      const int qq = (q + e < qb) ? q + e : qa;
+      v[e] = V[(size_t)sl_ent[qq] * 54 + l];
+      w[e] = xo[(size_t)9 * sl_obj[qq] + b];
+    }
+#pragma unroll
+    for (int e = 0; e < 4; ++e) if (q + e < qb) s += v[e] * w[e];
+  }
+  red[lane] = s;
+  __builtin_amdgcn_wave_barrier();
+  if (lane < 6) {
+    double t = 0;
+#pragma unroll
+    for (int bb = 0; bb < 9; ++bb) t += red[6 * bb + lane];
+    z[(size_t)i * 6 + lane] = vy[(size_t)i * 6 + lane] - t;
+  }
+}
+static __global__ __launch_bounds__(64) void k_cf_z_fwd(int nf_all, int stride, const double* __restrict__ Mm, double* __restrict__ z) {
+  __shared__ double sM[kCfSweepSI * 36], sz[kCfSweepSI * 6];
+  const int lane = threadIdx.x;
+  const int beg = (int)blockIdx.x * stride;
+  const int len = ((beg + stride - 1 < nf_all) ? beg + stride - 1 : nf_all) - beg;
+  if (len <= 0) return;
+  {
+    constexpr int kQ = (kCfSweepSI * 36 + 63) / 64, kZ = (kCfSweepSI * 6 + 63) / 64;
+    double tm[kQ], tz[kZ];
+#pragma unroll
+    for (int q = 0; q < kQ; ++q) { const int idx = q * 64 + lane; tm[q] = Mm[(size_t)beg * 36 + (idx < len * 36 ? idx : 0)]; }
+#pragma unroll
+    for (int q = 0; q < kZ; ++q) { const int idx = q * 64 + lane; tz[q] = z[(size_t)beg * 6 + (idx < len * 6 ? idx : 0)]; }
+#pragma unroll
+    for (int q = 0; q < kQ; ++q) if (q * 64 + lane < kCfSweepSI * 36) sM[q * 64 + lane] = tm[q];
+#pragma unroll
+    for (int q = 0; q < kZ; ++q) if (q * 64 + lane < kCfSweepSI * 6) sz[q * 64 + lane] = tz[q];
+  }
+  __builtin_amdgcn_wave_barrier();
+  const int a = lane < 6 ? lane : 5;
+  double za = 0;
+  for (int ii = 0; ii < len; ++ii) {
+    double zp[6];
+#pragma unroll
+    for (int k = 0; k < 6; ++k) zp[k] = cf_readlane(za, k);
+    double t = sz[ii * 6 + a];
+#pragma unroll
+    for (int k = 0; k < 6; ++k) t -= sM[ii * 36 + a * 6 + k] * zp[k];
+    za = t;
+    if (lane < 6) sz[ii * 6 + lane] = t;
+  }
+  __builtin_amdgcn_wave_barrier();
+  for (int idx = lane; idx < len * 6; idx += 64) z[(size_t)beg * 6 + idx] = sz[idx];
+}
+
+}
diff --git a/object-oriented-slam_amd/csrc/esl_chol.hpp b/object-oriented-slam_amd/csrc/esl_chol.hpp
--- a/object-oriented-slam_amd/csrc/esl_chol.hpp
+++ b/object-oriented-slam_amd/csrc/esl_chol.hpp
@@ -126,19 +126,19 @@
   void (*prof_mark)(void* user, int begin) = nullptr;
   void* prof_user = nullptr;
   hipStream_t cf_side = nullptr;
-  hipEvent_t cf_ev_x = nullptr, cf_ev_p = nullptr, cf_ev_a = nullptr, cf_ev_s = nullptr;
+  hipEvent_t cf_ev_x = nullptr, cf_ev_p = nullptr, cf_ev_a = nullptr, cf_ev_s = nullptr, cf_ev_c = nullptr, cf_ev_t = nullptr;
   hipError_t cf_overlap_init() {
-    if (cf_side && cf_ev_x && cf_ev_p && cf_ev_a && cf_ev_s) return hipSuccess;
+    if (cf_side && cf_ev_x && cf_ev_p && cf_ev_a && cf_ev_s && cf_ev_c && cf_ev_t) return hipSuccess;
     if (cf_side) return hipErrorNotReady;
     hipError_t e = hipStreamCreateWithFlags(&cf_side, hipStreamNonBlocking); if (e != hipSuccess) return e;
-    for (hipEvent_t* ev : {&cf_ev_x, &cf_ev_p, &cf_ev_a, &cf_ev_s}) {
+    for (hipEvent_t* ev : {&cf_ev_x, &cf_ev_p, &cf_ev_a, &cf_ev_s, &cf_ev_c, &cf_ev_t}) {
       e = hipEventCreateWithFlags(ev, hipEventDisableTiming); if (e != hipSuccess) return e;
     }
     return hipSuccess;
   }
   void release() {
     if (cf_side) { (void)hipStreamSynchronize(cf_side); (void)hipStreamDestroy(cf_side); cf_side = nullptr; }
-    for (hipEvent_t* ev : {&cf_ev_x, &cf_ev_p, &cf_ev_a, &cf_ev_s})
+    for (hipEvent_t* ev : {&cf_ev_x, &cf_ev_p, &cf_ev_a, &cf_ev_s, &cf_ev_c, &cf_ev_t})
       if (*ev) { (void)hipEventDestroy(*ev); *ev = nullptr; }
     if (bs_flags) { (void)hipFree(bs_flags); bs_flags = nullptr; bs_flags_cap = 0; }
     if (d_tasks) { (void)hipFree(d_tasks); d_tasks = nullptr; d_tasks_cap = 0; }
diff --git a/object-oriented-slam_amd/csrc/esl_ctx.hpp b/object-oriented-slam_amd/csrc/esl_ctx.hpp
--- a/object-oriented-slam_amd/csrc/esl_ctx.hpp
+++ b/object-oriented-slam_amd/csrc/esl_ctx.hpp
@@ -246,6 +246,8 @@
   unsigned long long* cf_mask = nullptr;
   long long *cf_xoff = nullptr, *cf_boff = nullptr, *cf_roff = nullptr;
   double *cf_Xc = nullptr, *cf_Xs = nullptr, *cf_P = nullptr, *cf_Prhs = nullptr, *cf_Y = nullptr, *cf_Yr = nullptr;
+  double *cf_Pm = nullptr, *cf_Qm = nullptr, *cf_XL = nullptr;
+  int* cf_sl_ent = nullptr;
   long long* cf_os_start = nullptr;
   int *cf_os_cnt = nullptr, *cf_os_pairs = nullptr;
   int *cf_os_run = nullptr, *cf_os_heads = nullptr;
@@ -282,5 +284,6 @@
   int sw_cf_os_kernel = 1;
   int sw_cf_os_list = 1;
   int sw_cf_fwd_parts = 8;
+  int sw_cf_sweep = 1;
   int sw_cf_stride = 0;
 };
diff --git a/object-oriented-slam_amd/csrc/esl_slam.hip b/object-oriented-slam_amd/csrc/esl_slam.hip
--- a/object-oriented-slam_amd/csrc/esl_slam.hip
+++ b/object-oriented-slam_amd/csrc/esl_slam.hip
@@ -9,6 +9,7 @@
 #include <cstring>
 
 #include "esl_cf.hpp"
+#include "esl_cf_sweep.hpp"
 #include "esl_chol.hpp"
 #include "esl_fixed.hpp"
 #include "esl_kernels_slam.hpp"
@@ -263,6 +264,7 @@
   c->cf_Zt = c->cf_Hs = c->cf_Bs = c->cf_LfacS = c->cf_GS = c->cf_LiS = c->cf_MS = c->cf_NS = c->cf_R = nullptr;
   c->cf_Xc = c->cf_Xs = c->cf_P = c->cf_Prhs = c->cf_Xt = c->cf_Y = c->cf_Yr = nullptr;
   c->cf_os_start = nullptr; c->cf_os_cnt = c->cf_os_pairs = c->cf_os_run = c->cf_os_heads = nullptr; c->cf_Vm = nullptr;
+  c->cf_Pm = c->cf_Qm = c->cf_XL = nullptr; c->cf_sl_ent = nullptr;
   c->cf_rank = c->cf_unrank = c->cf_kfirst = nullptr; c->cf_xo_t = nullptr;
   c->cf_plan = CfPlan{};
   c->cf_ready = false;
@@ -288,6 +290,7 @@
   sw.no_nd = std::getenv("ESL_CF_NO_ND") != nullptr;
   static const int nd_min = [] { const char* e = std::getenv("ESL_CF_ND_MIN"); return e ? std::atoi(e) : 48; }();
   sw.nd_min = nd_min; sw.stride = c->sw_cf_stride; sw.os_kernel = c->sw_cf_os_kernel; sw.os_list = c->sw_cf_os_list;
+  sw.sweep = c->sw_cf_sweep;
   size_t free_b = 0, total_b = 0;
   if (nfi >= kCfSparseMinCams) ESL_HIP_TRY(hipMemGetInfo(&free_b, &total_b));
   CfPlan& pl = c->cf_plan;
@@ -296,6 +299,7 @@
     return ESL_ERR_ALLOC;
   }
   const bool sp = pl.sparse, os3 = sp && pl.form == 3, osm = os3 && pl.os_list;
+  const bool swp = os3 && pl.sweep;
   const int nch = pl.n_chunks, nseg = pl.nseg, nw = pl.nw, N1 = N + 1;
   const size_t n_inc = pl.p.size();
   const size_t y_recs = std::max<size_t>(n_inc, 1) * (size_t)(pl.S - 1), nb = (size_t)N * (N + 1) / 2 + N;
@@ -313,6 +317,7 @@
     ship(&c->cf_xoff, pl.xoff); ship(&c->cf_boff, pl.boff); ship(&c->cf_roff, pl.roff); ship(&d_fw_off, pl.fw_off); ship(&d_tw_off, pl.tw_off);
   }
   if (osm) { ship(&c->cf_os_run, pl.os_run); ship(&c->cf_os_heads, pl.os_heads); }
+  if (swp) ship(&c->cf_sl_ent, pl.sl_ent);
   st.work(&c->cf_oe_cst, (size_t)std::max(N, 1) * (nch + 1));
   if (sp) {
     st.work(&c->cf_cmap, (size_t)nseg * N1); st.work(&c->cf_mask, (size_t)N1 * nw); st.work(&c->cf_seg_obj, n_inc); st.work(&c->cf_seg_first, n_inc);
@@ -330,12 +335,14 @@
     st.work(&c->cf_R, ns * 6 * (size_t)pl.ldx);
   }
   if (sp) {
-    st.work(&c->cf_Xc, pl.xc_len); st.work(&c->cf_Xs, (size_t)pl.ldx * (size_t)pl.kpad_s);
+    if (!swp) st.work(&c->cf_Xc, pl.xc_len);
+    st.work(&c->cf_Xs, (size_t)pl.ldx * (size_t)pl.kpad_s);
     if (pl.form == 1) { st.work(&c->cf_P, pl.p_blocks * 81); st.work(&c->cf_Prhs, pl.prhs_len); }
     if (pl.form == 3) {
       st.work(&c->cf_Y, y_recs * 54); st.work(&c->cf_Yr, std::max<size_t>(nf, 1) * 6);
       st.work(&c->cf_os_start, nb + 1); st.work(&c->cf_os_cnt, nb); st.work(&c->cf_os_pairs, 2 * std::max<size_t>(pl.os_list_npairs, 1));
       if (osm) st.work(&c->cf_Vm, EU * 54);
+      if (swp) { st.work(&c->cf_Pm, nf * 36); st.work(&c->cf_Qm, nf * 36); st.work(&c->cf_XL, std::max<size_t>(pl.xl_len, 1)); }
     }
   } else {
     st.work(&c->cf_Xt, (size_t)pl.ldx * (size_t)pl.kpad);
@@ -385,7 +392,7 @@
   }
   if (pl.nd) ESL_HIP_TRY(hipMemsetAsync(c->cf_Zt, 0, nf * 36 * sizeof(double), c->stream));
   if (sp) {
-    ESL_HIP_TRY(hipMemsetAsync(c->cf_Xc, 0, std::max<size_t>(pl.xc_len, 1) * sizeof(double), c->stream));
+    if (!swp) ESL_HIP_TRY(hipMemsetAsync(c->cf_Xc, 0, std::max<size_t>(pl.xc_len, 1) * sizeof(double), c->stream));
     ESL_HIP_TRY(hipMemsetAsync(c->cf_Xs, 0, (size_t)pl.ldx * (size_t)pl.kpad_s * sizeof(double), c->stream));
     ESL_HIP_TRY(hipMemsetAsync(c->cf_T, 0, (size_t)pl.ldt * n_o * sizeof(double), c->stream));
     if (pl.form == 3) {
@@ -417,11 +424,12 @@
   const int st, ns, nseg;
   const bool nd, dist;
   const unsigned cg;
+  const bool swp;
   const hipStream_t main;
   CfSideJoin join;
   CfTrial(esl_ctx* c_, CholRuntime& rt_, double lambda_)
       : c(c_), rt(rt_), pl(c_->cf_plan), g(c_->g), lambda(lambda_), N(g.n_objs), nf(g.n_free_cams), n_o(9 * N), ldx((long)pl.ldx), ldt((long)pl.ldt),
-        st(pl.stride), ns(pl.n_sep), nseg(pl.n_seg), nd(st > 0 && ns > 0), dist(cf_dist(c_)), cg((unsigned)((n_o + 1 + 63) / 64)), main(c_->stream),
+        st(pl.stride), ns(pl.n_sep), nseg(pl.n_seg), nd(st > 0 && ns > 0), dist(cf_dist(c_)), cg((unsigned)((n_o + 1 + 63) / 64)), swp(pl.sparse && pl.form == 3 && pl.sweep), main(c_->stream),
         join{rt_, c_->stream, false} {}
   CfSegs segs() const { return CfSegs{c->cf_fwork, c->cf_seg_start, c->cf_seg_obj, c->cf_xoff, c->cf_xld, c->cf_rank, c->cf_unrank}; }
   int edge_blocks() const { return (int)(((long)pl.n_list * 9 + nf + 255) / 256); }
@@ -438,8 +446,9 @@
     hipLaunchKernelGGL(k_cf_edge_scale, dim3((unsigned)edge_blocks()), dim3(256), 0, s, g, pl.n_list, c->cf_oe_u, c->cf_oe_slot, c->Wbb, c->cf_Linv, c->bc,
                        c->cf_V, c->cf_vy, cls, st);
   }
-  void segment_chains() const {
+  template <class F> void segment_chains(F after_chain) const {
     hipLaunchKernelGGL(k_cf_chain, dim3((unsigned)nseg), dim3(64), 0, main, nf, c->Hcc, c->cf_B, lambda, c->cf_Lfac, c->cf_G, c->chol_info, st, st - 1);
+    after_chain();
     hipLaunchKernelGGL(k_cf_factor_blocks, dim3((unsigned)((nf + 63) / 64)), dim3(64), 0, main, nf, c->cf_Lfac, c->cf_G, c->cf_Linv, c->cf_M, c->cf_N, st);
     if (nseg > 1) hipLaunchKernelGGL(k_cf_zt, dim3((unsigned)(nseg - 1)), dim3(64), 0, main, nf, st, c->cf_Linv, c->cf_M, c->cf_B, c->cf_Zt);
     hipLaunchKernelGGL(k_cf_sep_assemble, dim3((unsigned)((ns * 36 + 255) / 256)), dim3(256), 0, main, nf, st, ns, c->Hcc, lambda, c->cf_G, c->cf_Zt,
@@ -451,7 +460,21 @@
                        c->cf_Linv, st);
   }
   int slabs(bool beside) {
-    segment_chains();
+    auto twist = [&](hipStream_t s) {
+      hipLaunchKernelGGL(k_cf_twist, dim3((unsigned)nseg), dim3(64), 0, s, nf, st, c->Hcc, lambda, c->cf_Lfac, c->cf_G, c->cf_Pm, c->cf_Qm, c->chol_info);
+    };
+    hipError_t e_tw = hipSuccess;
+    segment_chains([&] {
+      if (!swp) return;
+      if (!beside) { twist(main); return; }
+      e_tw = hipEventRecord(rt.cf_ev_c, main);
+      if (e_tw == hipSuccess) e_tw = hipStreamWaitEvent(rt.cf_side, rt.cf_ev_c, 0);
+      if (e_tw != hipSuccess) return;
+      join.armed = true;
+      twist(rt.cf_side);
+      e_tw = hipEventRecord(rt.cf_ev_t, rt.cf_side);
+    });
+    ESL_HIP_TRY(e_tw);
     if (beside) {
       ESL_HIP_TRY(hipEventRecord(rt.cf_ev_a, main));
       ESL_HIP_TRY(hipStreamWaitEvent(rt.cf_side, rt.cf_ev_a, 0));
@@ -459,6 +482,19 @@
     }
     sep_chain(beside ? rt.cf_side : main);
     if (beside) ESL_HIP_TRY(hipEventRecord(rt.cf_ev_s, rt.cf_side));
+    if (swp) {
+      edge_scale(beside ? 1 : 0, main);
+      if (beside) ESL_HIP_TRY(hipStreamWaitEvent(main, rt.cf_ev_t, 0));
+      auto sweep = [&](auto parts) {
+        hipLaunchKernelGGL((k_cf_sweep<decltype(parts)::value>), dim3((unsigned)pl.n_fwork), dim3(64), 0, main, nf, n_o, pl.n_chunks, c->cf_oe_cst, c->cf_oe_slot,
+                           c->cf_V, c->cf_vy, c->cf_M, (const double*)c->cf_Zt, c->cf_Pm, c->cf_Qm, c->cf_R, ldx, st, segs(), c->cf_Y, c->cf_Yr, c->cf_XL,
+                           (long long)(st == kCfFwdCh ? kCfSegRows : 6 * (st - 1)));
+      };
+      if (c->sw_cf_fwd_parts == 8) sweep(std::integral_constant<int, 8>{});
+      else if (c->sw_cf_fwd_parts == 4) sweep(std::integral_constant<int, 4>{});
+      else sweep(std::integral_constant<int, 2>{});
+      return ESL_OK;
+    }
     edge_scale(beside ? 1 : 0, main);
     auto forward = [&](auto parts) {
       hipLaunchKernelGGL((k_cf_forward<2, decltype(parts)::value>), dim3((unsigned)pl.n_fwork), dim3(64), 0, main, nf, n_o, pl.n_chunks, c->cf_oe_cst, c->cf_oe_slot,
@@ -471,7 +507,8 @@
   }
   void sep_rhs(hipStream_t s, bool sp = true) const {
     hipLaunchKernelGGL(k_cf_sep_rhs, dim3(cg, (unsigned)ns), dim3(64), 0, s, nf, n_o, st, pl.n_chunks, c->cf_oe_cst, c->cf_oe_slot, c->cf_V, c->cf_vy,
-                       c->cf_G, c->cf_LiS, sp ? c->cf_Xc : c->cf_Xt, ldx, c->cf_R, sp ? (const int*)c->cf_cmap : nullptr, sp ? segs() : CfSegs{});
+                       c->cf_G, c->cf_LiS, sp ? c->cf_Xc : c->cf_Xt, ldx, c->cf_R, sp ? (const int*)c->cf_cmap : nullptr, sp ? segs() : CfSegs{},
+                       (const double*)(sp && swp ? c->cf_XL : nullptr), (long long)(st == kCfFwdCh ? kCfSegRows : 6 * (st - 1)));
   }
   void sep_forward(hipStream_t s, bool sp = true) const {
     hipLaunchKernelGGL(k_cf_forward<1>, dim3(cg), dim3(64), 0, s, ns, n_o, pl.n_chunks, c->cf_oe_cst, c->cf_oe_slot, c->cf_V, c->cf_vy,
@@ -512,7 +549,7 @@
       hipLaunchKernelGGL(k_cf_forward<0>, dim3(cg), dim3(64), 0, main, nf, n_o, pl.n_chunks, c->cf_oe_cst, c->cf_oe_slot, c->cf_V, c->cf_vy,
                          c->cf_M, c->cf_Xt, ldx, nf, nf, (const double*)nullptr, (double*)nullptr, 0, CfSegs{});
     } else {
-      segment_chains();
+      segment_chains([] {});
       sep_chain(main);
       edge_scale_T();
       hipLaunchKernelGGL(k_cf_forward<0>, dim3(cg, (unsigned)nseg), dim3(64), 0, main, nf, n_o, pl.n_chunks, c->cf_oe_cst, c->cf_oe_slot, c->cf_V,
@@ -597,9 +634,11 @@
         hipLaunchKernelGGL(k_cf_seg_back<decltype(mch)::value>, dim3((unsigned)pl.n_fwork), dim3(64), 0, main, nf, c->cf_fwork, c->cf_seg_start, c->cf_xoff,
                            c->cf_xld, c->cf_Xc, c->cf_Linv, c->cf_G, c->cf_Y, c->cf_Yr);
       };
-      if (st == 3 * kCfFwdCh) seg_back(std::integral_constant<int, 3>{});
-      else if (st == 2 * kCfFwdCh) seg_back(std::integral_constant<int, 2>{});
-      else seg_back(std::integral_constant<int, 1>{});
+      if (!swp) {
+        if (st == 3 * kCfFwdCh) seg_back(std::integral_constant<int, 3>{});
+        else if (st == 2 * kCfFwdCh) seg_back(std::integral_constant<int, 2>{});
+        else seg_back(std::integral_constant<int, 1>{});
+      }
       if (pl.os_list && pl.n_list > 0)
         hipLaunchKernelGGL(k_cf_v_merge, dim3((unsigned)(((long)pl.n_list * 9 + 255) / 256)), dim3(256), 0, main, pl.n_list, (const int*)c->cf_os_run, c->cf_V, c->cf_Vm);
       const dim3 grid((unsigned)(N + 1), (unsigned)((N + kCfTPer - 1) / kCfTPer));
@@ -625,7 +664,12 @@
         ESL_HIP_TRY(chol_factor_solve(c->cf_T, ldt, n_o, c->cf_Linv_ws, c->z_ws, xsol, c->chol_info, main, rt));
       }
       if (xsol != c->xo) hipLaunchKernelGGL(k_cf_xo_unpermute, dim3((unsigned)((n_o + 255) / 256)), dim3(256), 0, main, N, c->cf_rank, xsol, c->xo);
-      if (pl.sparse)
+      if (swp) {
+        hipLaunchKernelGGL(k_cf_wxo, dim3((unsigned)nf), dim3(64), 0, main, st, g.cu_start, (const int*)c->cf_sl_ent, g.cu_obj, c->cf_V, c->cf_vy, c->xo, c->cf_z);
+        hipLaunchKernelGGL(k_cf_z_fwd, dim3((unsigned)nseg), dim3(64), 0, main, nf, st, c->cf_M, c->cf_z);
+        if (ns > 0)
+          hipLaunchKernelGGL(k_cf_z_sparse, dim3((unsigned)(6 * ns)), dim3(256), 0, main, n_o, c->cf_Xs, ldx, segs(), (const double*)nullptr, c->xo, xsol, c->cf_z, st, 1);
+      } else if (pl.sparse)
         hipLaunchKernelGGL(k_cf_z_sparse, dim3((unsigned)(6 * nf)), dim3(256), 0, main, n_o, c->cf_Xs, ldx, segs(), c->cf_Xc, c->xo, xsol, c->cf_z, st);
       else
         hipLaunchKernelGGL(k_cf_z, dim3((unsigned)(6 * nf)), dim3(256), 0, main, c->cf_Xt, ldx, n_o, c->xo, c->cf_z);
```

Measured after the change: 19.72 (median of 6 runs). 1.03x the previous value.
